# r4dl/LAENeRF

Hardware: AMD Instinct MI355X
Metric: Mrays/s, lego 800x800 train-step (4096 rays/step) (higher is better)
Workload: dtype f16 (table, MLP) / f32 (march, composite); 1 GPU; configs[1]: lego-like 800x800 pinhole rays, 4096 random pixels of one view per step, L=16 T=2^19 F=2 hash grid + 2x64 / 3x64 ffmlp, cascade 1, analytic occupancy (13% occupied), steady-state train step incl. backward + Adam; hip_graph_replay=True, march_pipelined_on_side_stream=True, steps_per_graph_replay=4, parallelism=1 independent ray-batch replicas (no data-path collective)

## Files before the change

### include/laenerf.h

```cpp
#ifndef LAENERF_H
#define LAENERF_H

#include <stdint.h>

#ifdef __cplusplus
extern "C" {
#endif

#if defined(__GNUC__) || defined(__clang__)
#define LAE_API __attribute__((visibility("default")))
#else
#define LAE_API
#endif

#define LAE_OK 0
#define LAE_EINVAL (-1)
#define LAE_ELAUNCH (-2)
#define LAE_ENULL (-3)

#define LAE_F32 0
#define LAE_F16 1

#define LAE_GRID_HASH 0
#define LAE_GRID_TILED 1
#define LAE_INTERP_LINEAR 0
#define LAE_INTERP_SMOOTHSTEP 1

#define LAE_ACT_RELU 0
#define LAE_ACT_EXPONENTIAL 1
#define LAE_ACT_SINE 2
#define LAE_ACT_SIGMOID 3
#define LAE_ACT_SQUAREPLUS 4
#define LAE_ACT_SOFTPLUS 5
#define LAE_ACT_NONE 6

#define LAE_ABI_TAG "abi14"
LAE_API const char* lae_version(void);
LAE_API const char* lae_last_error(void);


LAE_API int lae_near_far_from_aabb(const float* rays_o, const float* rays_d, const float* aabb,
                           uint32_t N, float min_near, float* nears, float* fars, void* stream);

LAE_API int lae_get_rays(const float* poses, uint32_t B, float fx, float fy, float cx, float cy, uint32_t H, uint32_t W,
                 const int64_t* inds, uint64_t inds_batch_stride, uint32_t N, int perturb, float off_x, float off_y,
                 float* rays_o, float* rays_d, const float* aabb, float min_near, float* nears, float* fars, void* stream);

#define LAE_IMG_U8 0
#define LAE_IMG_F16 1
#define LAE_IMG_F32 2
#define LAE_BATCH_IMAGE 0
#define LAE_BATCH_ALL 1
#define LAE_BG_WHITE 0
#define LAE_BG_RANDOM 1
LAE_API int lae_sample_train_batch(const void* images, int dtype, uint32_t n_img, uint32_t H, uint32_t W, uint32_t C,
                           const float* poses, float fx, float fy, float cx, float cy, uint32_t N,
                           const float* aabb, float min_near, uint64_t seed, int64_t* step_counter, int mode, int bg_mode,
                           int srgb_to_linear, float* rays_o, float* rays_d, float* nears, float* fars, float* gt,
                           float* bg_out, int64_t* inds, void* stream);

LAE_API int lae_sample_train_batch_weighted(const void* images, int dtype, uint32_t n_img, uint32_t H, uint32_t W, uint32_t C,
                                    const float* poses, float fx, float fy, float cx, float cy, uint32_t N,
                                    const float* aabb, float min_near, uint64_t seed, int64_t* step_counter, int bg_mode,
                                    int srgb_to_linear, const float* error_map, int32_t* cells_out, float* rays_o, float* rays_d,
                                    float* nears, float* fars, float* gt, float* bg_out, int64_t* inds, void* stream);

LAE_API int lae_error_map_update(float* error_map, uint32_t n_img, uint32_t H, uint32_t W, const int64_t* inds, const int32_t* cells,
                                 const float* pred, const float* gt, uint32_t N, void* stream);

// ... 94 lines not shown
                     uint32_t C, uint32_t H, const void* table_f16, const int32_t* offsets, const int32_t* offsets_host,
                     uint32_t L, float S,
                     uint32_t base_resolution, uint32_t gridtype, int align_corners, uint32_t interp,
                     const void* sigma_weights, const void* color_weights, float density_scale, float T_thresh,
                     uint32_t max_n_step, uint64_t row_budget, const float* noises, const float* bg_rays, float bg_r, float bg_g,
                     float bg_b, int blend_bg, int scale_depth, float* weights_sum, float* depth, float* image,
                     float* weights_edit, float* depth_edit, void* workspace, uint64_t workspace_bytes, uint32_t* stats_out,
                     void* stream);

LAE_API uint64_t lae_compact_scratch_bytes(uint32_t n_alive);
LAE_API int lae_compact_rays_alive(const int32_t* rays_alive, uint32_t n_alive, int32_t* out_alive,
                           int32_t* n_out_dev, void* scratch, void* stream);


LAE_API int lae_grid_encode_forward(const float* inputs, const void* embeddings, const int32_t* offsets,
                            void* outputs, uint32_t B, uint32_t D, uint32_t C, uint32_t L,
                            float S, uint32_t H, void* dy_dx, uint32_t gridtype,
                            int align_corners, uint32_t interp, int dtype, void* stream);

LAE_API int lae_grid_encode_backward(const void* grad, const float* inputs, const void* embeddings,
                             const int32_t* offsets, void* grad_embeddings, uint32_t B,
                             uint32_t D, uint32_t C, uint32_t L, float S, uint32_t H,
                             const void* dy_dx, void* grad_inputs, uint32_t gridtype,
                             int align_corners, uint32_t interp, int dtype, void* stream);

LAE_API int lae_grid_encode_forward_ex(const float* inputs, const void* embeddings, const int32_t* offsets, void* outputs,
                               uint32_t B, uint32_t D, uint32_t C, uint32_t L, float S, uint32_t H, void* dy_dx,
                               uint32_t gridtype, int align_corners, uint32_t interp, int dtype, int blc, float in_shift,
                               float in_scale, const int32_t* offsets_host, void* stream);
LAE_API int lae_grid_encode_backward_ex(const void* grad, const float* inputs, const void* embeddings, const int32_t* offsets,
                                void* grad_embeddings, uint32_t B, uint32_t D, uint32_t C, uint32_t L, float S,
                                uint32_t H, const void* dy_dx, void* grad_inputs, uint32_t gridtype,
                                int align_corners, uint32_t interp, int dtype, int blc, float in_shift, float in_scale,
                                const int32_t* offsets_host, int32_t* nonfinite_flag, uint32_t* touched_lines, void* stream);

LAE_API uint64_t lae_grid_backward_plan_bytes(uint32_t B, uint32_t L);
LAE_API uint64_t lae_grid_touched_lines_words(uint64_t n_entries);
LAE_API int lae_grid_encode_backward_plan(const float* inputs, const int32_t* offsets, uint32_t B, uint32_t D, uint32_t C, uint32_t L,
                                  float S, uint32_t H, uint32_t gridtype, int align_corners, uint32_t interp, int dtype,
                                  float in_shift, float in_scale, const int32_t* offsets_host, void* plan,
                                  uint32_t* touched_lines, void* stream);
LAE_API int lae_grid_encode_backward_planned(const void* grad, const float* inputs, const int32_t* offsets, void* grad_embeddings,
                                     uint32_t B, uint32_t D, uint32_t C, uint32_t L, float S, uint32_t H, uint32_t gridtype,
                                     int align_corners, uint32_t interp, int dtype, float in_shift, float in_scale,
                                     const int32_t* offsets_host, const void* plan, int32_t* nonfinite_flag, void* stream);

LAE_API uint64_t lae_grid_backward_workspace_bytes(uint32_t B, uint32_t L, int dtype);

LAE_API int lae_grid_forward_schedule(const int32_t* offsets_host, uint32_t L, float S, uint32_t H, uint32_t n_chunks,
                              uint32_t* nseg_out, uint32_t* segs_out);

LAE_API int lae_grid_set_forward_mode(int mode);

LAE_API int lae_grid_set_backward_mode(int mode);

LAE_API int lae_grad_total_variation(const void* inputs, const void* embeddings, void* grad,
                             const int32_t* offsets, float weight, uint32_t B, uint32_t D,
                             uint32_t C, uint32_t L, float S, uint32_t H, uint32_t gridtype,
                             int align_corners, int dtype, void* stream);


LAE_API int lae_sh_encode_forward(const float* inputs, float* outputs, uint32_t B, uint32_t D,
                          uint32_t C, float* dy_dx, void* stream);

LAE_API int lae_sh_encode_backward(const float* grad, const float* inputs, uint32_t B, uint32_t D,
                           uint32_t C, const float* dy_dx, float* grad_inputs, void* stream);


LAE_API int lae_ffmlp_forward(const void* inputs, const void* weights, uint32_t B, uint32_t input_dim,
                      uint32_t output_dim, uint32_t hidden_dim, uint32_t num_layers,
                      uint32_t activation, uint32_t output_activation, void* forward_buffer,
                      void* outputs, void* stream);

LAE_API int lae_ffmlp_inference(const void* inputs, const void* weights, uint32_t B, uint32_t input_dim,
                        uint32_t output_dim, uint32_t hidden_dim, uint32_t num_layers,
                        uint32_t activation, uint32_t output_activation, void* inference_buffer,
                        void* outputs, void* stream);

LAE_API int lae_ffmlp_backward(const void* grad, const void* inputs, const void* weights,
                       const void* forward_buffer, uint32_t B, uint32_t input_dim,
                       uint32_t output_dim, uint32_t hidden_dim, uint32_t num_layers,
                       uint32_t activation, uint32_t output_activation, int calc_grad_inputs,
                       void* backward_buffer, void* grad_inputs, void* grad_weights,
                       void* stream);
LAE_API int lae_ffmlp_backward_ex(const void* grad, const void* inputs, const void* weights,
                          const void* forward_buffer, uint32_t B, uint32_t input_dim,
                          uint32_t output_dim, uint32_t hidden_dim, uint32_t num_layers,
                          uint32_t activation, uint32_t output_activation, int calc_grad_inputs,
                          void* backward_buffer, void* grad_inputs, void* grad_weights,
                          int accumulate, int32_t* nonfinite_flag, void* stream);

LAE_API int lae_nerf_head_forward(const void* enc, const float* dirs, const void* sigma_weights, const void* color_weights,
                          uint32_t M, float density_scale, void* h_out, float* sigmas, float* rgbs, int enc_level_major,
                          void* stream);

LAE_API int lae_nerf_density_forward(const void* enc, const void* sigma_weights, uint32_t M, float density_scale, void* h_out,
                             float* sigmas, int enc_level_major, void* stream);

LAE_API int lae_nerf_head_backward(const float* grad_sigmas, const float* grad_rgbs, const void* enc, const float* dirs, const void* h,
                           const float* rgbs, const void* sigma_weights, const void* color_weights, uint32_t M,
                           float density_scale, void* grad_h, void* grad_enc, void* grad_sigma_weights,
                           void* grad_color_weights, int accumulate_weight_grads, int enc_level_major,
                           int32_t* nonfinite_flag, const float* loss_partials, uint32_t loss_n_part, uint32_t loss_n_elem,
                           const float* loss_scale, float* loss_out, void* stream);

LAE_API int lae_freq_encode_forward(const float* inputs, uint32_t B, uint32_t D, uint32_t deg, uint32_t C, float* outputs,
                            void* stream);
LAE_API int lae_freq_encode_backward(const float* grad, const float* outputs, uint32_t B, uint32_t D, uint32_t deg, uint32_t C,
                             float* grad_inputs, void* stream);

LAE_API int lae_palette_forward(const void* w_logits, const void* o_raw, const float* palette, uint32_t P, uint32_t active_mask,
                        uint32_t M, void* pred, float* w_hat, void* o_hat, void* stream);
LAE_API uint64_t lae_palette_backward_scratch_bytes(uint32_t M);
LAE_API int lae_palette_backward(const void* w_logits, const void* o_raw, const float* palette, uint32_t P, uint32_t active_mask,
                         uint32_t M, const void* g_pred, const float* g_w, const void* g_o, void* g_w_logits, void* g_o_raw,
                         float* g_palette, void* scratch, void* stream);

#define LAE_RECOLOR_PREVIEW 0
#define LAE_RECOLOR_WEIGHTS 1
#define LAE_RECOLOR_OFFSETS 2
#define LAE_RECOLOR_EVAL 3
#define LAE_RECOLOR_NO_OFFSETS 1
#define LAE_RECOLOR_TANH 2
LAE_API uint64_t lae_recolor_compact_scratch_bytes(uint32_t N);
LAE_API int lae_recolor_compact(const float* depth, const float* weights_sum, const float* rays_o, const float* rays_d, uint32_t N,
                                int32_t* indices, int32_t* slot_map, float* x_term, float* dirs, float* alpha, int32_t* count,
                                void* scratch, void* stream);
LAE_API int lae_recolor_compose(const int32_t* slot_map, uint32_t N, const void* w_logits, uint32_t w_stride, const void* o_raw,
                                uint32_t o_stride, uint32_t P, uint32_t active_mask, const float* palette, const float* p_weights,
                                const float* p_bias, const float* alpha, const float* base, const float* bg, int mode, uint32_t k,
                                int flags, float* out, uint8_t* out_u8, void* stream);

#define LAE_DISTILL_NO_BG 1
LAE_API int lae_distill_compose(uint32_t R, const int32_t* img_idx, const int32_t* pix, const float* w, const float* pred,
                                const float* dist, const void* w_logits, uint32_t w_stride, const void* o_raw, uint32_t o_stride,
                                uint32_t P, uint32_t active_mask, const float* palette_mod, const float* palette_og,
                                const float* p_weights, const float* p_bias, float blend_thresh, int flags, void* images, int dtype,
// ... 58 lines not shown
LAE_API int lae_min_dist_to_points(const float* pts, uint32_t n, const float* set, uint32_t m, float max_dist, float* out,
                           float* out_max, void* scratch, void* stream);

LAE_API int lae_density_grid_positions(const int32_t* coords, uint32_t n, uint32_t H, float bound_c, const float* noise,
                               float* xyzs, int32_t* indices, void* stream);
LAE_API uint64_t lae_density_grid_partial_scratch_bytes(uint32_t cells, uint32_t n);
LAE_API int lae_density_grid_partial_positions(const float* grid_c, uint32_t cells, const int32_t* coords_rand, const float* u, const float* rnd,
                                       uint32_t n, uint32_t H, float bound_c, const float* noise, float* xyzs, int32_t* indices,
                                       void* scratch, void* stream);
LAE_API int lae_density_grid_update(const float* sigmas, const int32_t* indices, uint32_t n, float density_scale, float decay,
                            uint32_t cells, float* grid, uint32_t* tmp, void* stream);
LAE_API int lae_mark_untrained_grid(const float* poses, uint32_t B, float fx, float fy, float cx, float cy, uint32_t C, uint32_t H,
                            float bound, float min_near, int filter_close_point, float* grid, void* stream);

LAE_API uint64_t lae_marching_cubes_scratch_bytes(uint32_t nx, uint32_t ny, uint32_t nz);
LAE_API int lae_marching_cubes_count(const float* u, uint32_t nx, uint32_t ny, uint32_t nz, float threshold, void* scratch,
                             int32_t* counts, void* stream);
LAE_API int lae_marching_cubes_emit(const float* u, uint32_t nx, uint32_t ny, uint32_t nz, float threshold, void* scratch, float* verts,
                            int32_t* tris, void* stream);

LAE_API int lae_adam_check(const void* grad, int grad_is_half, uint64_t n, void* state, void* stream);
LAE_API int lae_adam_begin(void* state, float beta1, float beta2, int growth_interval, float growth_factor, float backoff_factor,
                   int use_scaler, void* stream);
LAE_API int lae_adam_apply(float* param, float* exp_avg, float* exp_avg_sq, void* grad, int grad_is_half, void* shadow_half, uint64_t n,
                   const void* state, const float* lr, float beta1, float beta2, float eps, float weight_decay, void* stream);

LAE_API int lae_mse_loss_forward(const float* pred, const float* target, uint32_t n, const float* scale, float* loss_out, float* grad,
                         void* stream);

LAE_API int lae_adam_check_multi(uint32_t n_tensors, const void* const* grads, const int* grad_is_half, const uint64_t* sizes, void* state,
                         void* stream);
LAE_API int lae_adam_apply_multi(uint32_t n_tensors, float* const* params, float* const* exp_avgs, float* const* exp_avg_sqs, void* const* grads,
                         const int* grad_is_half, void* const* shadows_half, const uint64_t* sizes, const float* const* lrs, const void* const* touched_lines,
                         const void* state, float beta1, float beta2, float eps, float weight_decay, void* stream);

LAE_API int lae_ema_update_multi(uint32_t n_tensors, float* const* shadows, const float* const* params, const uint64_t* sizes,
                         float one_minus_decay, void* stream);
LAE_API int lae_ema_update_gated(uint32_t n_tensors, float* const* shadows, const float* const* params, const uint64_t* sizes,
                         const int64_t* step, int64_t epoch_len, int32_t* count, double decay, int use_num_updates, void* stream);

#define LAE_EVAL_VIEW_SCRATCH_DOUBLES 2048
LAE_API int lae_eval_view(const float* pred, const float* depth, const void* gt, int gt_dtype, uint32_t gt_channels, uint32_t n_pixels,
                          float bg, const uint8_t* mask, double* scratch, double* sse_out, double* masked_sse_out, float* gt_out,
                          uint8_t* rgb_u8, uint8_t* depth_u8, float* lpips_in, void* stream);
LAE_API int lae_lpips_head(uint32_t n_layers, const float* const* feats, const float* const* weights, const uint32_t* channels,
                           const uint32_t* hw, uint32_t n_pairs, double* scratch, double* out, void* stream);

LAE_API int lae_ffmlp_set_mode(int mode);

LAE_API int lae_allocate_splitk(uint64_t size);
LAE_API int lae_free_splitk(void);

LAE_API int lae_free_workspaces(void);
LAE_API uint64_t lae_workspace_bytes(int retired);

#ifdef __cplusplus
}
#endif
#endif
```

### laenerf_amd/_lib.py

```python
import ctypes
import os

import torch

_HERE = os.path.dirname(os.path.abspath(__file__))
SO_PATH = os.environ.get("LAE_HIP_LIB") or os.path.join(_HERE, "lib", "liblaenerf_hip.so")

u32, u64, f32, i32, vp = ctypes.c_uint32, ctypes.c_uint64, ctypes.c_float, ctypes.c_int, ctypes.c_void_p
i64, f64 = ctypes.c_int64, ctypes.c_double

SIGNATURES = {
    "lae_near_far_from_aabb": [vp, vp, vp, u32, f32, vp, vp, vp],
    "lae_sph_from_ray": [vp, vp, f32, u32, vp, vp],
    "lae_get_rays": [vp, u32, f32, f32, f32, f32, u32, u32, vp, u64, u32, i32, f32, f32, vp, vp, vp, f32, vp, vp, vp],
    "lae_morton3D": [vp, u32, vp, vp],
    "lae_morton3D_invert": [vp, u32, vp, vp],
    "lae_packbits": [vp, u32, f32, vp, vp],
    "lae_march_rays_train_scratch_bytes": [u32],
    "lae_march_rays_train": [vp, vp, vp, f32, f32, u32, u32, u32, u32, u32, vp, vp, vp, vp, vp, vp, vp, vp, vp, vp, vp],
    "lae_march_rays_train_limit": [vp, vp, vp, f32, f32, u32, u32, u32, u32, u32, vp, vp, vp, vp, vp, vp, vp, vp, vp, vp, vp, vp],
    "lae_sample_train_batch": [vp, i32, u32, u32, u32, u32, vp, f32, f32, f32, f32, u32, vp, f32, u64, vp, i32, i32, i32, vp, vp, vp, vp, vp,
                               vp, vp, vp],
    "lae_sample_train_batch_weighted": [vp, i32, u32, u32, u32, u32, vp, f32, f32, f32, f32, u32, vp, f32, u64, vp, i32, i32, vp, vp,
                                        vp, vp, vp, vp, vp, vp, vp, vp],
    "lae_error_map_update": [vp, u32, u32, u32, vp, vp, vp, vp, u32, vp],
    "lae_composite_rays_train_forward": [vp, vp, vp, vp, u32, u32, f32, vp, vp, vp, vp],
    "lae_composite_rays_train_backward": [vp, vp, vp, vp, vp, vp, vp, vp, u32, u32, f32, vp, vp, vp],
    "lae_composite_rays_train_forward_blend": [vp, vp, vp, vp, u32, u32, f32, vp, vp, vp, f32, f32, f32, vp, vp, vp, vp, vp, vp],
    "lae_composite_rays_train_step": [vp, vp, vp, vp, u32, u32, f32, vp, vp, vp, f32, f32, f32, vp, vp, vp, vp, vp, vp, vp, vp, vp, vp, vp, vp, vp, i32, vp],
    "lae_loss_finish": [vp, u32, u32, vp, vp, vp],
    "lae_composite_rays_train_backward_blend": [vp, vp, vp, vp, vp, vp, vp, vp, u32, u32, f32, vp, f32, f32, f32, vp, vp, vp, vp],
    "lae_composite_rays_train_backward_blend_ex": [vp, vp, vp, vp, vp, vp, vp, vp, u32, u32, f32, vp, f32, f32, f32, vp, vp, vp, vp, vp],
    "lae_march_rays": [u32, u32, vp, vp, vp, vp, f32, f32, u32, u32, u32, vp, vp, vp, vp, vp, vp, vp, vp],
    "lae_march_rays_distill": [u32, u32, vp, vp, vp, vp, f32, f32, u32, u32, u32, vp, vp, vp, vp, vp, vp, vp, vp, vp, vp],
    "lae_composite_rays": [u32, u32, f32, vp, vp, vp, vp, vp, vp, vp, vp, vp],
    "lae_composite_rays_distill": [u32, u32, f32, vp, vp, vp, vp, vp, vp, vp, vp, vp, vp, vp, vp],
    "lae_render_frame_workspace_bytes": [u32, u32, u64],
    "lae_render_frame_set_overlap": [i32],
    "lae_render_frame_mode": [],
    "lae_render_frame_last_status": [],
    "lae_render_frame_probe_us": [vp, u32],
    "lae_render_frame": [vp, vp, u32, vp, f32, vp, vp, f32, f32, u32, u32, u32, vp, vp, vp, u32, f32, u32, u32, i32, u32, vp, vp, f32, f32,
                         u32, u64, vp, vp, f32, f32, f32, i32, i32, vp, vp, vp, vp, vp, vp, u64, vp, vp],
    "lae_compact_scratch_bytes": [u32],
    "lae_compact_rays_alive": [vp, u32, vp, vp, vp, vp],
    "lae_grid_encode_forward": [vp, vp, vp, vp, u32, u32, u32, u32, f32, u32, vp, u32, i32, u32, i32, vp],
    "lae_grid_encode_backward": [vp, vp, vp, vp, vp, u32, u32, u32, u32, f32, u32, vp, vp, u32, i32, u32, i32, vp],
    "lae_grid_encode_forward_ex": [vp, vp, vp, vp, u32, u32, u32, u32, f32, u32, vp, u32, i32, u32, i32, i32, f32, f32, vp, vp],
    "lae_grid_encode_backward_ex": [vp, vp, vp, vp, vp, u32, u32, u32, u32, f32, u32, vp, vp, u32, i32, u32, i32, i32, f32, f32, vp, vp, vp, vp],
    "lae_grid_backward_workspace_bytes": [u32, u32, i32],
    "lae_grid_backward_plan_bytes": [u32, u32],
    "lae_grid_touched_lines_words": [u64],
    "lae_grid_encode_backward_plan": [vp, vp, u32, u32, u32, u32, f32, u32, u32, i32, u32, i32, f32, f32, vp, vp, vp, vp],
    "lae_grid_encode_backward_planned": [vp, vp, vp, vp, u32, u32, u32, u32, f32, u32, u32, i32, u32, i32, f32, f32, vp, vp, vp, vp],
    "lae_grid_set_backward_mode": [i32],
    "lae_grid_set_forward_mode": [i32],
    "lae_grid_forward_schedule": [vp, u32, f32, u32, u32, vp, vp],
    "lae_grad_total_variation": [vp, vp, vp, vp, f32, u32, u32, u32, u32, f32, u32, u32, i32, i32, vp],
    "lae_sh_encode_forward": [vp, vp, u32, u32, u32, vp, vp],
    "lae_sh_encode_backward": [vp, vp, u32, u32, u32, vp, vp, vp],
    "lae_freq_encode_forward": [vp, u32, u32, u32, u32, vp, vp],
    "lae_freq_encode_backward": [vp, vp, u32, u32, u32, u32, vp, vp],
    "lae_ffmlp_forward": [vp, vp, u32, u32, u32, u32, u32, u32, u32, vp, vp, vp],
    "lae_ffmlp_inference": [vp, vp, u32, u32, u32, u32, u32, u32, u32, vp, vp, vp],
    "lae_ffmlp_backward": [vp, vp, vp, vp, u32, u32, u32, u32, u32, u32, u32, i32, vp, vp, vp, vp],
    "lae_ffmlp_backward_ex": [vp, vp, vp, vp, u32, u32, u32, u32, u32, u32, u32, i32, vp, vp, vp, i32, vp, vp],
    "lae_nerf_head_forward": [vp, vp, vp, vp, u32, f32, vp, vp, vp, i32, vp],
    "lae_nerf_density_forward": [vp, vp, u32, f32, vp, vp, i32, vp],
    "lae_density_grid_positions": [vp, u32, u32, f32, vp, vp, vp, vp],
    "lae_density_grid_partial_scratch_bytes": [u32, u32],
    "lae_density_grid_partial_positions": [vp, u32, vp, vp, vp, u32, u32, f32, vp, vp, vp, vp, vp],
    "lae_density_grid_update": [vp, vp, u32, f32, f32, u32, vp, vp, vp],
    "lae_mark_untrained_grid": [vp, u32, f32, f32, f32, f32, u32, u32, f32, f32, i32, vp, vp],
    "lae_nerf_head_backward": [vp, vp, vp, vp, vp, vp, vp, vp, u32, f32, vp, vp, vp, vp, i32, i32, vp, vp, u32, u32, vp, vp, vp],
    "lae_palette_forward": [vp, vp, vp, u32, u32, u32, vp, vp, vp, vp],
    "lae_palette_backward_scratch_bytes": [u32],
    "lae_palette_backward": [vp, vp, vp, u32, u32, u32, vp, vp, vp, vp, vp, vp, vp, vp],
    "lae_recolor_compact_scratch_bytes": [u32],
    "lae_recolor_compact": [vp, vp, vp, vp, u32, vp, vp, vp, vp, vp, vp, vp, vp],
    "lae_recolor_compose": [vp, u32, vp, u32, vp, u32, u32, u32, vp, vp, vp, vp, vp, vp, i32, u32, i32, vp, vp, vp],
    "lae_distill_compose": [u32, vp, vp, vp, vp, vp, vp, u32, vp, u32, u32, u32, vp, vp, vp, vp, f32, i32, vp, i32, u32, u32, u32, vp],
    "lae_error_map_seed": [u32, vp, vp, vp, vp, u32, u32, u32, u32, vp, vp, vp],
    "lae_marching_cubes_scratch_bytes": [u32, u32, u32],
    "lae_marching_cubes_count": [vp, u32, u32, u32, f32, vp, vp, vp],
    "lae_marching_cubes_emit": [vp, u32, u32, u32, f32, vp, vp, vp, vp],
    "lae_style_loss_scratch_bytes": [u32],
    "lae_style_loss_forward": [vp, vp, vp, vp, u32, u32, f32, f32, f32, vp, vp, vp, vp, u32, f32, f32, vp],
    "lae_style_loss_backward": [vp, vp, vp, u32, u32, u32, vp, vp, vp, f32, f32, f32, vp, vp, vp, vp, i32, f32, f32, vp],
    "lae_style_loss_forward_dev": [vp, vp, vp, vp, u32, vp, u32, f32, f32, f32, vp, vp, vp, vp, u32, f32, f32, vp],
    "lae_style_loss_backward_dev": [vp, vp, vp, u32, u32, u32, vp, vp, vp, vp, f32, f32, f32, vp, vp, vp, vp, i32, f32, f32, vp],
    "lae_sample_edit_view": [vp, vp, vp, vp, vp, vp, u32, vp, u32, u32, u64, vp, vp, vp, vp, vp, vp],
    "lae_style_loss_backward_image_dev": [vp, vp, vp, u32, u32, u32, vp, vp, vp, vp, f32, f32, f32, vp, vp, vp, vp, vp, i32, f32, f32, vp],
    "lae_style_image_scratch_bytes": [u32],
    "lae_style_image_forward": [vp, u32, vp, vp, u32, vp, u32, vp, vp, vp, vp, vp, vp, vp, vp, u32, vp, i32, u32, vp, vp, vp],
    "lae_style_image_backward": [vp, u32, vp, vp, u32, vp, u32, vp, vp, vp, vp, vp, vp, vp, vp, vp, vp, u32, vp, vp, i32, vp, vp],
    "lae_grow_region": [vp, vp, u32, u32, f32, vp, u32, vp, u32, u32, vp],
    "lae_style_assemble_forward": [vp, vp, u32, u32, u32, vp, vp, u32, vp],
    "lae_style_assemble_backward": [vp, vp, u32, u32, vp, vp],
    "lae_min_dist_to_points": [vp, u32, vp, u32, f32, vp, vp, vp, vp],
    "lae_mse_loss_forward": [vp, vp, u32, vp, vp, vp, vp],
    "lae_adam_check": [vp, i32, u64, vp, vp],
    "lae_adam_check_multi": [u32, vp, vp, vp, vp, vp],
    "lae_adam_apply_multi": [u32, vp, vp, vp, vp, vp, vp, vp, vp, vp, vp, f32, f32, f32, f32, vp],
    "lae_adam_begin": [vp, f32, f32, i32, f32, f32, i32, vp],
    "lae_ema_update_multi": [u32, vp, vp, vp, f32, vp],
    "lae_ema_update_gated": [u32, vp, vp, vp, vp, i64, vp, f64, i32, vp],
    "lae_eval_view": [vp, vp, vp, i32, u32, u32, f32, vp, vp, vp, vp, vp, vp, vp, vp, vp],
    "lae_lpips_head": [u32, vp, vp, vp, vp, u32, vp, vp, vp],
    "lae_adam_apply": [vp, vp, vp, vp, i32, vp, u64, vp, vp, f32, f32, f32, f32, vp],
    "lae_ffmlp_set_mode": [i32],
    "lae_allocate_splitk": [u64],
    "lae_free_splitk": [],
    "lae_free_workspaces": [],
    "lae_workspace_bytes": [i32],
    "lae_version": [],
    "lae_last_error": [],
}
_RESTYPES = {
    "lae_march_rays_train_scratch_bytes": u64,
    "lae_compact_scratch_bytes": u64,
    "lae_density_grid_partial_scratch_bytes": u64,
    "lae_palette_backward_scratch_bytes": u64,
    "lae_style_loss_scratch_bytes": u64,
    "lae_recolor_compact_scratch_bytes": u64,
    "lae_marching_cubes_scratch_bytes": u64,
    "lae_style_image_scratch_bytes": u64,
    "lae_render_frame_workspace_bytes": u64,
    "lae_workspace_bytes": u64,
    "lae_grid_backward_workspace_bytes": u64,
    "lae_grid_backward_plan_bytes": u64,
    "lae_grid_touched_lines_words": u64,
    "lae_version": ctypes.c_char_p,
    "lae_last_error": ctypes.c_char_p,
}

_lib = None
ABI_TAG = b"abi14"


def _abi_of(path):
    lib = ctypes.CDLL(path)
    fn = lib.lae_version
    fn.argtypes, fn.restype = [], ctypes.c_char_p
    return lib, fn().split()[-1]


def load():
    global _lib
    if _lib is not None:
        return _lib
    if not os.path.exists(SO_PATH):
        raise RuntimeError(
            f"laenerf_amd: HIP library not built ({SO_PATH}); run `python -m laenerf_amd.build` "
            "(there is no CPU fallback)")
    if not os.environ.get("LAE_HIP_LIB"):
        from . import build as _build
        if _build.default_is_packed(SO_PATH):
            _build.build(force=True)
            if _build.default_is_packed(SO_PATH):
                raise RuntimeError(f"laenerf_amd: {SO_PATH} was built with packed-fp32 instructions and could not be rebuilt without them")
    lib, tag = _abi_of(SO_PATH)
    if tag != ABI_TAG:
        if os.environ.get("LAE_HIP_LIB"):
            raise RuntimeError(f"laenerf_amd: {SO_PATH} is ABI {tag.decode()}, this package binds {ABI_TAG.decode()}")
        import fcntl
        import shutil
        from . import build as _build
        with open(SO_PATH + ".lock", "w") as lock:
            fcntl.flock(lock, fcntl.LOCK_EX)
            try:
# ... 60 lines not shown
```

### laenerf_amd/backend.py

```python
import sys
import types

import numpy as np
import torch

from . import _lib
from ._lib import check, need_contig, need_cuda, ptr, stream

_F16 = torch.float16


def _dtype_code(t):
    if t.dtype == torch.float32:
        return 0
    if t.dtype == torch.float16:
        return 1
    raise RuntimeError(f"laenerf_amd: unsupported dtype {t.dtype} (float32 / float16 only)")


def _host_i32(a, n):
    if a is None:
        return None
    if not (isinstance(a, np.ndarray) and a.dtype == np.int32 and a.flags.c_contiguous and a.size == n):
        raise RuntimeError("laenerf_amd: offsets_host must be a contiguous int32 numpy array with L + 1 entries")
# ... 341 lines not shown
    @staticmethod
    def grid_encode_forward(inputs, embeddings, offsets, outputs, B, D, C, L, S, H, dy_dx, gridtype, align_corners,
                            interp, blc=False, in_map=(0.0, 1.0), offsets_host=None):
        need_cuda(inputs, embeddings, offsets, outputs, dy_dx); need_contig(inputs, embeddings, offsets, outputs, dy_dx)
        if inputs.dtype != torch.float32 or offsets.dtype != torch.int32:
            raise RuntimeError("grid_encode_forward: inputs must be float32, offsets int32")
        if outputs.dtype != embeddings.dtype or (dy_dx is not None and dy_dx.dtype != embeddings.dtype):
            raise RuntimeError("grid_encode_forward: outputs/dy_dx must have the embeddings dtype")
        lib = _lib.load()
        args = (ptr(inputs), ptr(embeddings), ptr(offsets), ptr(outputs), B, D, C, L, float(S), H, ptr(dy_dx), gridtype,
                int(bool(align_corners)), interp, _dtype_code(embeddings))
        if blc or tuple(in_map) != (0.0, 1.0) or offsets_host is not None:
            check(lib.lae_grid_encode_forward_ex(*args, int(bool(blc)), float(in_map[0]), float(in_map[1]), _host_i32(offsets_host, L + 1),
                                                 stream()), "grid_encode_forward")
        else:
            check(lib.lae_grid_encode_forward(*args, stream()), "grid_encode_forward")

    @staticmethod
    def grid_backward_plan(inputs, offsets, B, D, C, L, S, H, gridtype, align_corners, interp, half, in_map=(0.0, 1.0),
                           offsets_host=None, touched_lines=None):
        need_cuda(inputs, offsets); need_contig(inputs, offsets)
        lib = _lib.load()
        plan = torch.empty(int(lib.lae_grid_backward_plan_bytes(B, L)), dtype=torch.uint8, device=inputs.device)
        check(lib.lae_grid_encode_backward_plan(ptr(inputs), ptr(offsets), B, D, C, L, float(S), H, gridtype, int(bool(align_corners)),
                                                interp, 1 if half else 0, float(in_map[0]), float(in_map[1]),
                                                _host_i32(offsets_host, L + 1), ptr(plan), touched_lines, stream()),
              "grid_backward_plan")
        plan.marks_touched = touched_lines is not None
        return plan

    @staticmethod
    def grid_encode_backward(grad, inputs, embeddings, offsets, grad_embeddings, B, D, C, L, S, H, dy_dx, grad_inputs,
                             gridtype, align_corners, interp, blc=False, in_map=(0.0, 1.0), offsets_host=None, plan=None,
                             nonfinite_flag=None, touched_lines=None):
        ts = (grad, inputs, embeddings, offsets, grad_embeddings, dy_dx, grad_inputs, plan)
        need_cuda(*ts); need_contig(*ts)
        if grad.dtype != grad_embeddings.dtype:
            raise RuntimeError("grid_encode_backward: grad and grad_embeddings dtypes differ")
        lib = _lib.load()
        if plan is not None:
            if blc or dy_dx is not None:
                raise RuntimeError("grid_encode_backward: a plan needs level-major gradients and no input gradient")
            if touched_lines is not None and not getattr(plan, "marks_touched", False):
                raise RuntimeError("grid_encode_backward: the plan was made without the touched-lines bitmap (pass it to grid_backward_plan)")
            check(lib.lae_grid_encode_backward_planned(ptr(grad), ptr(inputs), ptr(offsets), ptr(grad_embeddings), B, D, C, L, float(S), H,
                                                       gridtype, int(bool(align_corners)), interp, _dtype_code(grad), float(in_map[0]),
                                                       float(in_map[1]), _host_i32(offsets_host, L + 1), ptr(plan), nonfinite_flag, stream()),
                  "grid_encode_backward")
            return
        args = (ptr(grad), ptr(inputs), ptr(embeddings), ptr(offsets), ptr(grad_embeddings), B, D, C, L, float(S), H,
                ptr(dy_dx), ptr(grad_inputs), gridtype, int(bool(align_corners)), interp, _dtype_code(grad))
        if blc or tuple(in_map) != (0.0, 1.0) or offsets_host is not None or nonfinite_flag is not None or touched_lines is not None:
            check(lib.lae_grid_encode_backward_ex(*args, int(bool(blc)), float(in_map[0]), float(in_map[1]), _host_i32(offsets_host, L + 1),
                                                  nonfinite_flag, touched_lines, stream()), "grid_encode_backward")
        else:
            check(lib.lae_grid_encode_backward(*args, stream()), "grid_encode_backward")

    @staticmethod
    def grid_backward_workspace_bytes(B, L, half=True):
        return int(_lib.load().lae_grid_backward_workspace_bytes(B, L, 1 if half else 0))

    @staticmethod
    def set_backward_mode(mode):
        check(_lib.load().lae_grid_set_backward_mode(int(mode)), "grid_set_backward_mode")

    @staticmethod
    def grad_total_variation(inputs, embeddings, grad, offsets, weight, B, D, C, L, S, H, gridtype, align_corners):
        need_cuda(inputs, embeddings, grad, offsets); need_contig(inputs, embeddings, grad, offsets)
        check(_lib.load().lae_grad_total_variation(ptr(inputs), ptr(embeddings), ptr(grad), ptr(offsets), float(weight), B, D,
                                                   C, L, float(S), H, gridtype, int(bool(align_corners)),
                                                   _dtype_code(embeddings), stream()), "grad_total_variation")


class _SHEncoder:
    @staticmethod
    def sh_encode_forward(inputs, outputs, B, D, C, dy_dx):
        need_cuda(inputs, outputs, dy_dx); need_contig(inputs, outputs, dy_dx)
        if inputs.dtype != torch.float32 or outputs.dtype != torch.float32:
            raise RuntimeError("sh_encode_forward: float32 required (sphere_harmonics.py:16 casts to fp32)")
        check(_lib.load().lae_sh_encode_forward(ptr(inputs), ptr(outputs), B, D, C, ptr(dy_dx), stream()), "sh_encode_forward")

    @staticmethod
    def sh_encode_backward(grad, inputs, B, D, C, dy_dx, grad_inputs):
        need_cuda(grad, inputs, dy_dx, grad_inputs); need_contig(grad, inputs, dy_dx, grad_inputs)
        if grad.dtype != torch.float32:
            raise RuntimeError("sh_encode_backward: float32 required")
        check(_lib.load().lae_sh_encode_backward(ptr(grad), ptr(inputs), B, D, C, ptr(dy_dx), ptr(grad_inputs), stream()),
# ... 49 lines not shown
            check(_lib.load().lae_ffmlp_backward_ex(ptr(grad), ptr(inputs), ptr(weights), ptr(forward_buffer), B, input_dim,
                                                    output_dim, hidden_dim, num_layers, activation, output_activation,
                                                    int(bool(calc_grad_inputs)), ptr(backward_buffer), ptr(grad_inputs),
                                                    ptr(grad_weights), int(bool(accumulate)), nonfinite_flag, stream()), "ffmlp_backward")
            return
        check(_lib.load().lae_ffmlp_backward(ptr(grad), ptr(inputs), ptr(weights), ptr(forward_buffer), B, input_dim,
                                             output_dim, hidden_dim, num_layers, activation, output_activation,
                                             int(bool(calc_grad_inputs)), ptr(backward_buffer), ptr(grad_inputs),
                                             ptr(grad_weights), stream()), "ffmlp_backward")

    @staticmethod
    def nerf_head_forward(enc, dirs, sigma_weights, color_weights, M, density_scale, h_out, sigmas, rgbs, level_major=False):
        ts = (enc, dirs, sigma_weights, color_weights, h_out, sigmas, rgbs)
        need_cuda(*ts); need_contig(*ts); _FFMLP._half(enc, sigma_weights, color_weights, h_out)
        check(_lib.load().lae_nerf_head_forward(ptr(enc), ptr(dirs), ptr(sigma_weights), ptr(color_weights), M,
                                                float(density_scale), ptr(h_out), ptr(sigmas), ptr(rgbs),
                                                int(bool(level_major)), stream()), "nerf_head_forward")

    @staticmethod
    def nerf_density_forward(enc, sigma_weights, M, density_scale, h_out, sigmas, level_major=False):
        need_cuda(enc, sigma_weights, h_out, sigmas); need_contig(enc, sigma_weights, h_out, sigmas)
        _FFMLP._half(enc, sigma_weights, h_out)
        check(_lib.load().lae_nerf_density_forward(ptr(enc), ptr(sigma_weights), M, float(density_scale), ptr(h_out),
                                                   ptr(sigmas), int(bool(level_major)), stream()), "nerf_density_forward")

    @staticmethod
    def nerf_head_backward(grad_sigmas, grad_rgbs, enc, dirs, h, rgbs, sigma_weights, color_weights, M, density_scale,
                           grad_h, grad_enc, grad_sigma_weights, grad_color_weights, accumulate=False, level_major=False,
                           nonfinite_flag=None):
        ts = (grad_sigmas, grad_rgbs, enc, dirs, h, rgbs, sigma_weights, color_weights, grad_h, grad_enc,
              grad_sigma_weights, grad_color_weights)
        need_cuda(*ts); need_contig(*ts)
        _FFMLP._half(enc, h, sigma_weights, color_weights, grad_h, grad_enc, grad_sigma_weights, grad_color_weights)
        key = _loss_key(grad_sigmas)
        pend = _pending_loss.get(key)
        if pend is not None and pend[5] != stream():
            pend = None
        if pend is not None:
            del _pending_loss[key]
        lp, ln, le, lsc, lo = pend[:5] if pend is not None else (None, 0, 0, None, None)
        try:
            check(_lib.load().lae_nerf_head_backward(ptr(grad_sigmas), ptr(grad_rgbs), ptr(enc), ptr(dirs), ptr(h), ptr(rgbs),
                                                     ptr(sigma_weights), ptr(color_weights), M, float(density_scale),
                                                     ptr(grad_h), ptr(grad_enc), ptr(grad_sigma_weights),
                                                     ptr(grad_color_weights), int(bool(accumulate)), int(bool(level_major)),
                                                     nonfinite_flag, ptr(lp), ln, le, ptr(lsc), ptr(lo), stream()), "nerf_head_backward")
        except RuntimeError:
            if pend is not None:
                _pending_loss[key] = pend
            raise
        if pend is not None:
            deferred_loss_stats["carried"] += 1

    @staticmethod
    def ffmlp_set_mode(mode):
        check(_lib.load().lae_ffmlp_set_mode(int(mode)), "ffmlp_set_mode")

    @staticmethod
    def fused_backward_available(input_dim, hidden_dim, num_layers, activation):
        return hidden_dim == 64 and activation == 0 and num_layers in (2, 3) and input_dim in (32, 48, 64)

    @staticmethod
    def allocate_splitk(size):
        check(_lib.load().lae_allocate_splitk(int(size)), "allocate_splitk")

    @staticmethod
    def free_splitk():
        check(_lib.load().lae_free_splitk(), "free_splitk")


_timing = {"on": False, "only": None, "events": []}
_UNITS = {"grid_encode_forward": 4, "grid_encode_backward": 5, "grid_backward_plan": 2, "ffmlp_forward": 2, "ffmlp_inference": 2,
          "ffmlp_backward": 4, "nerf_head_forward": 4, "nerf_head_backward": 8, "nerf_density_forward": 2, "sh_encode_forward": 2, "march_rays_train": 6, "composite_rays_train_forward": 5,
          "composite_rays_train_backward": 9,
          "composite_rays_train_forward_blend": 5, "composite_rays_train_backward_blend": 9}


def enable_kernel_timing(on, only=("grid_encode_forward",)):
    import gc
    if on and not _timing["on"]:
        _timing["gc_was_enabled"] = gc.isenabled()
        gc.collect()
        gc.disable()
    elif not on and _timing["on"]:
        if _timing.pop("gc_was_enabled", True):
# ... 239 lines not shown
```

### laenerf_amd/csrc/ffmlp.hip

```cpp
#include <string>
#include <algorithm>
#include <type_traits>
#include <stdlib.h>
#include "lae_common.h"

namespace {

typedef _Float16 half_t;
typedef _Float16 h4 __attribute__((ext_vector_type(4)));
typedef float f4 __attribute__((ext_vector_type(4)));

__device__ __forceinline__ f4 mfma16(h4 a, h4 b, f4 c) { return __builtin_amdgcn_mfma_f32_16x16x16f16(a, b, c, 0, 0, 0); }

typedef _Float16 h8 __attribute__((ext_vector_type(8)));
__device__ __forceinline__ f4 mfma32(h4 a_lo, h4 a_hi, h4 b_lo, h4 b_hi, f4 c) {
    const h8 a = __builtin_shufflevector(a_lo, a_hi, 0, 1, 2, 3, 4, 5, 6, 7);
    const h8 b = __builtin_shufflevector(b_lo, b_hi, 0, 1, 2, 3, 4, 5, 6, 7);
    return __builtin_amdgcn_mfma_f32_16x16x32_f16(a, b, c, 0, 0, 0);
}
template <int KT, typename LoadA>
__device__ __forceinline__ f4 mfma_ksteps(LoadA&& a_of, const h4* b, f4 acc) {
#pragma unroll
    for (int kt = 0; kt + 1 < KT; kt += 2) acc = mfma32(a_of(kt), a_of(kt + 1), b[kt], b[kt + 1], acc);
    if constexpr (KT & 1) {
        const h4 z = h4{(half_t)0.0f, (half_t)0.0f, (half_t)0.0f, (half_t)0.0f};
        acc = mfma32(a_of(KT - 1), z, b[KT - 1], z, acc);
    }
    return acc;
}

#define K_ACT 10.0f
__device__ __forceinline__ float act_fwd(uint32_t a, float v) {
    switch (a) {
        case LAE_ACT_RELU: return v > 0.0f ? v : 0.0f;
        case LAE_ACT_EXPONENTIAL: return expf(v);
        case LAE_ACT_SINE: return sinf(v);
        case LAE_ACT_SIGMOID: return 1.0f / (1.0f + expf(-v));
// ... 244 lines not shown
            if ((uint32_t)i < nt_n) {
                const half_t* q = A + (b0 + 4 * g) * IN + (nt0 + i) * 16 + c;
                bf[i][0] = q[0]; bf[i][1] = q[IN]; bf[i][2] = q[2 * (size_t)IN]; bf[i][3] = q[3 * (size_t)IN];
            }
        }
#pragma unroll
        for (int i = 0; i < 4; i++)
#pragma unroll
            for (int j = 0; j < 4; j++)
                if ((uint32_t)i < mt_n && (uint32_t)j < nt_n) acc[i][j] = mfma16(a[i], bf[j], acc[i][j]);
    }
    __shared__ float red[16 * 256];
    for (int ww = 0; ww < MLP_BLOCK / 64; ww++) {
        if (w == ww) {
#pragma unroll
            for (int i = 0; i < 4; i++)
#pragma unroll
                for (int j = 0; j < 4; j++)
#pragma unroll
                    for (int r = 0; r < 4; r++) {
                        float* p = &red[(i * 4 + j) * 256 + (4 * g + r) * 16 + c];
                        *p = (ww == 0) ? acc[i][j][r] : (*p + acc[i][j][r]);
                    }
        }
        __syncthreads();
    }
    float* slab = slabs + (size_t)blockIdx.x * nW + w_off;
    for (uint32_t e = threadIdx.x; e < 16 * 256; e += MLP_BLOCK) {
        const uint32_t t = e >> 8, i = t >> 2, j = t & 3, rr = (e >> 4) & 15, cc = e & 15;
        if (i < mt_n && j < nt_n) slab[(size_t)((mt0 + i) * 16 + rr) * IN + (nt0 + j) * 16 + cc] = red[e];
    }
}

constexpr int DWR_GROUPS = 16;
__device__ __forceinline__ void dw_reduce_body(const float* __restrict__ slabs, uint32_t n_slices, uint32_t nW, half_t* __restrict__ gw,
                                               int accumulate, uint32_t block, int32_t* __restrict__ nf_flag = nullptr) {
    __shared__ float part[DWR_GROUPS][64];
    const uint32_t e = threadIdx.x & 63, sg = threadIdx.x >> 6;
    const uint32_t i = block * 64 + e;
    float s[8] = {0, 0, 0, 0, 0, 0, 0, 0};
    if (i < nW) {
        uint32_t k = sg;
        for (; k + 7 * DWR_GROUPS < n_slices; k += 8 * DWR_GROUPS) {
#pragma unroll
            for (int u = 0; u < 8; u++) s[u] += slabs[(size_t)(k + u * DWR_GROUPS) * nW + i];
        }
        for (; k < n_slices; k += DWR_GROUPS) s[0] += slabs[(size_t)k * nW + i];
    }
    part[sg][e] = ((s[0] + s[1]) + (s[2] + s[3])) + ((s[4] + s[5]) + (s[6] + s[7]));
    __syncthreads();
    if (sg == 0 && i < nW) {
        float t[DWR_GROUPS];
#pragma unroll
        for (int u = 0; u < DWR_GROUPS; u++) t[u] = part[u][e];
#pragma unroll
        for (int w = DWR_GROUPS / 2; w > 0; w >>= 1)
#pragma unroll
            for (int u = 0; u < w; u++) t[u] = t[u] + t[u + w];
        const half_t r = accumulate ? (half_t)((float)gw[i] + t[0]) : (half_t)t[0];
        gw[i] = r;
        if (nf_flag && (__builtin_bit_cast(uint16_t, r) & 0x7c00u) == 0x7c00u) atomicOr(nf_flag, 1);
    }
}
__global__ __launch_bounds__(64 * DWR_GROUPS) void k_dw_reduce(const float* __restrict__ slabs, uint32_t n_slices, uint32_t nW,
                                                               half_t* __restrict__ gw, int accumulate = 0, int32_t* __restrict__ nf_flag = nullptr) {
    dw_reduce_body(slabs, n_slices, nW, gw, accumulate, blockIdx.x, nf_flag);
}
struct LossFinish { const float* partials; uint32_t n_part, n_elem; const float* scale; float* out; };
__global__ __launch_bounds__(64 * DWR_GROUPS) void k_dw_reduce2(const float* __restrict__ slabs_a, uint32_t n_a, uint32_t nW_a,
                                                                half_t* __restrict__ gw_a, const float* __restrict__ slabs_b,
                                                                uint32_t n_b, uint32_t nW_b, half_t* __restrict__ gw_b,
                                                                uint32_t nb_a, uint32_t nb_b, int accumulate, int32_t* __restrict__ nf_flag,
                                                                LossFinish lf) {
    if (blockIdx.x < nb_a) dw_reduce_body(slabs_a, n_a, nW_a, gw_a, accumulate, blockIdx.x, nf_flag);
    else if (blockIdx.x < nb_a + nb_b) dw_reduce_body(slabs_b, n_b, nW_b, gw_b, accumulate, blockIdx.x - nb_a, nf_flag);
    else {
        static_assert(64 * DWR_GROUPS == 1024, "the loss sum is written for 16 waves, like k_loss_finish");
        __shared__ float part[16];
        float acc = 0.0f;
        for (uint32_t i = threadIdx.x; i < lf.n_part; i += 1024) acc += lf.partials[i];
        {
            auto dpp = [](float v, auto ctrl, auto mask) {
                return __builtin_bit_cast(float, __builtin_amdgcn_update_dpp(0, __builtin_bit_cast(int, v), decltype(ctrl)::value, decltype(mask)::value, 0xf, false));
            };
            using std::integral_constant;
            acc += dpp(acc, integral_constant<int, 0x111>{}, integral_constant<int, 0xf>{});
            acc += dpp(acc, integral_constant<int, 0x112>{}, integral_constant<int, 0xf>{});
            acc += dpp(acc, integral_constant<int, 0x114>{}, integral_constant<int, 0xf>{});
            acc += dpp(acc, integral_constant<int, 0x118>{}, integral_constant<int, 0xf>{});
            acc += dpp(acc, integral_constant<int, 0x142>{}, integral_constant<int, 0xa>{});
            acc += dpp(acc, integral_constant<int, 0x143>{}, integral_constant<int, 0xc>{});
            acc = __builtin_bit_cast(float, __builtin_amdgcn_readlane(__builtin_bit_cast(int, acc), 63));
        }
        if ((threadIdx.x & 63) == 0) part[threadIdx.x >> 6] = acc;
        __syncthreads();
        if (threadIdx.x == 0) {
            float t = 0.0f;
#pragma unroll
            for (int w = 0; w < 16; w++) t += part[w];
            const float loss = t / (float)lf.n_elem;
            lf.out[0] = loss * (lf.scale ? lf.scale[0] : 1.0f);
            lf.out[1] = loss;
        }
    }
}

#include "sh_table.inc"

__device__ __forceinline__ void stage_rows(half_t* dst, int ld, const half_t* __restrict__ src, int rows, int cols) {
    for (uint32_t e = threadIdx.x; e < (uint32_t)rows * cols / 4; e += blockDim.x) {
        const uint32_t r = (e * 4) / cols, k = (e * 4) % cols;
        *reinterpret_cast<h4*>(dst + r * ld + k) = *reinterpret_cast<const h4*>(src + (size_t)r * cols + k);
    }
}

template <int KT>
__device__ __forceinline__ void layer64(const half_t* Wl, int ld, const h4 (&in)[KT], int c, int g, f4 (&acc)[4]) {
#pragma unroll
    for (int mt = 0; mt < 4; mt++) acc[mt] = f4{0, 0, 0, 0};
#pragma unroll
    for (int kt = 0; kt + 1 < KT; kt += 2)
#pragma unroll
        for (int mt = 0; mt < 4; mt++) {
            const half_t* wr = Wl + (mt * 16 + c) * ld + kt * 16 + 4 * g;
            acc[mt] = mfma32(*reinterpret_cast<const h4*>(wr), *reinterpret_cast<const h4*>(wr + 16), in[kt], in[kt + 1], acc[mt]);
        }
    if constexpr (KT & 1) {
        const h4 z = h4{(half_t)0.0f, (half_t)0.0f, (half_t)0.0f, (half_t)0.0f};
#pragma unroll
        for (int mt = 0; mt < 4; mt++)
            acc[mt] = mfma32(*reinterpret_cast<const h4*>(Wl + (mt * 16 + c) * ld + (KT - 1) * 16 + 4 * g), z, in[KT - 1], z, acc[mt]);
    }
}
typedef _Float16 h2 __attribute__((ext_vector_type(2)));
__device__ __forceinline__ void relu4(const f4 (&acc)[4], h4 (&out)[4]) {
#pragma unroll
    for (int mt = 0; mt < 4; mt++) {
// ... 1328 lines not shown
    return lae::check_launch("ffmlp_backward");
}

int lae_nerf_head_forward(const void* enc, const float* dirs, const void* sigma_weights, const void* color_weights,
                          uint32_t M, float density_scale, void* h_out, float* sigmas, float* rgbs, int enc_level_major,
                          void* stream) {
    if (M == 0) return LAE_OK;
    if (!enc || !dirs || !sigma_weights || !color_weights || !h_out || !sigmas || !rgbs) return LAE_ENULL;
    if (M % 16 != 0) return LAE_EINVAL;
    if (const int rc = head_args_ok(sigma_weights, color_weights, M, "nerf_head_forward")) return rc;
    const int rc = launch_head_fwd5<true>((const half_t*)enc, dirs, (const half_t*)sigma_weights, (const half_t*)color_weights, M / 16, M / 16,
                                          density_scale, (half_t*)h_out, sigmas, rgbs, enc_level_major, nullptr, M,
                                          reinterpret_cast<hipStream_t>(stream));
    return rc != LAE_OK ? rc : lae::check_launch("nerf_head_forward");
}

int lae_nerf_density_forward(const void* enc, const void* sigma_weights, uint32_t M, float density_scale, void* h_out,
                             float* sigmas, int enc_level_major, void* stream) {
    if (M == 0) return LAE_OK;
    if (!enc || !sigma_weights || !sigmas) return LAE_ENULL;
    if (M % 16 != 0) return LAE_EINVAL;
    if (const int rc = head_args_ok(sigma_weights, sigma_weights, M, "nerf_density_forward")) return rc;
    const int rc = launch_head_fwd5<false>((const half_t*)enc, nullptr, (const half_t*)sigma_weights, nullptr, M / 16, M / 16, density_scale,
                                           (half_t*)h_out, sigmas, nullptr, enc_level_major, nullptr, M, reinterpret_cast<hipStream_t>(stream));
    return rc != LAE_OK ? rc : lae::check_launch("nerf_density_forward");
}

int lae_nerf_head_backward(const float* grad_sigmas, const float* grad_rgbs, const void* enc, const float* dirs, const void* h,
                           const float* rgbs, const void* sigma_weights, const void* color_weights, uint32_t M,
                           float density_scale, void* grad_h, void* grad_enc, void* grad_sigma_weights,
                           void* grad_color_weights, int accumulate_weight_grads, int enc_level_major, int32_t* nonfinite_flag,
                           const float* loss_partials, uint32_t loss_n_part, uint32_t loss_n_elem, const float* loss_scale,
                           float* loss_out, void* stream) {
    if (!grad_sigma_weights || !grad_color_weights) return LAE_ENULL;
    if (loss_out && (!loss_partials || loss_n_elem == 0)) return LAE_EINVAL;
    hipStream_t s = reinterpret_cast<hipStream_t>(stream);
    if (M == 0) {
        if (loss_out) {
            const int rc = lae_loss_finish(loss_partials, loss_n_part, loss_n_elem, loss_scale, loss_out, stream);
            if (rc != LAE_OK) return rc;
        }
        if (accumulate_weight_grads) return LAE_OK;
        if (hipMemsetAsync(grad_sigma_weights, 0, 64 * (32 + 64 + 16) * 2, s) != hipSuccess) return LAE_ELAUNCH;
        if (hipMemsetAsync(grad_color_weights, 0, 64 * (32 + 128 + 16) * 2, s) != hipSuccess) return LAE_ELAUNCH;
        return LAE_OK;
    }
    if (!grad_sigmas || !grad_rgbs || !enc || !dirs || !h || !rgbs || !sigma_weights || !color_weights || !grad_h) return LAE_ENULL;
    if (M % 16 != 0) return LAE_EINVAL;
    HeadBwdArgs ha{dirs, rgbs, grad_rgbs, grad_sigmas, density_scale, 0};
    HeadBwdArgs hs{};
    hs.level_major = enc_level_major;
    const uint32_t nW_c = 64 * (32 + 128 + 16), nW_s = 64 * (32 + 64 + 16);
    const size_t cap = (size_t)lae::num_cus() * 2;
    float* ws = reinterpret_cast<float*>(lae::workspace(lae::WS_FFMLP_SLABS, cap * (nW_c + nW_s) * sizeof(float), s));
    if (!ws) return LAE_ELAUNCH;
    float* ws_s = ws + cap * nW_c;
    uint32_t n_c = 0, n_s = 0;
    int rc = launch_bwd_fused<32, 2, 1>(nullptr, (const half_t*)h, (const half_t*)color_weights, M, (half_t*)grad_h,
                                        (half_t*)grad_color_weights, s, ha, accumulate_weight_grads, ws, &n_c);
    if (rc != LAE_OK) return rc;
    rc = launch_bwd_fused<32, 1, 0>((const half_t*)grad_h, (const half_t*)enc, (const half_t*)sigma_weights, M, (half_t*)grad_enc,
                                    (half_t*)grad_sigma_weights, s, hs, accumulate_weight_grads, ws_s, &n_s);
    if (rc != LAE_OK) return rc;
    const uint32_t nb_c = lae::cdiv(nW_c, 64u), nb_s = lae::cdiv(nW_s, 64u);
    const LossFinish lf{loss_partials, loss_n_part, loss_n_elem, loss_scale, loss_out};
    k_dw_reduce2<<<nb_c + nb_s + (loss_out ? 1u : 0u), 64 * DWR_GROUPS, 0, s>>>(ws, n_c, nW_c, (half_t*)grad_color_weights, ws_s, n_s, nW_s,
                                                                               (half_t*)grad_sigma_weights, nb_c, nb_s,
                                                                               accumulate_weight_grads, nonfinite_flag, lf);
    return lae::check_launch("nerf_head_backward");
}

int lae_ffmlp_set_mode(int mode) {
    if (mode != 0 && mode != 1 && mode != 3) return LAE_EINVAL;
    g_ffmlp_mode = mode == 1 ? 1 : 0;
    g_bwd_fused_variant = mode == 3 ? 0 : 2;
    return LAE_OK;
}

int lae_allocate_splitk(uint64_t size) {
    (void)size;
    return LAE_OK;
}

int lae_free_splitk(void) {
    lae::free_workspaces();
    return LAE_OK;
}

}
```

### laenerf_amd/csrc/gridencoder.hip

```cpp
#include <math.h>
#include <stdio.h>
#include <stdlib.h>
#include <algorithm>
#include <type_traits>
#include "lae_common.h"
#include <vector>
#include <mutex>
#include <utility>

namespace {

constexpr int MAX_LEVELS = 32;
struct LevelScales { float scale[MAX_LEVELS]; float in_shift, in_scale; };

typedef _Float16 half_t;
typedef _Float16 half2_t __attribute__((ext_vector_type(2)));

__constant__ uint32_t k_primes[7] = {1u, 2654435761u, 805459861u, 3674653429u, 2097192037u, 1434869437u, 2165219737u};

#ifdef LAE_GRID_STAMPS
__device__ unsigned long long g_grid_stamps[32768 * 32];
#define GRID_STAMP(slot, i) do { if (threadIdx.x == 0 && (uint32_t)(i) < 32u) g_grid_stamps[(size_t)(slot) * 32 + (i)] = wall_clock64(); } while (0)
#define GRID_NOTE(slot, i, v) do { if (threadIdx.x == 0 && (uint32_t)(i) < 32u) g_grid_stamps[(size_t)(slot) * 32 + (i)] = (v); } while (0)
#else
#define GRID_STAMP(slot, i) do { } while (0)
#define GRID_NOTE(slot, i, v) do { } while (0)
#endif


template <int D>
struct LevelInfo {
    float scale;
    uint32_t resolution, hashmap_size, table_off;
    uint32_t stride[D];
    uint32_t ndense;
    bool use_hash, pow2;
    bool nowrap;
};
// ... 259 lines not shown
#endif
}


__global__ __launch_bounds__(GRID_BLOCK) void k_grid_fwd_lean_tail(
    const float* __restrict__ inputs, const half_t* __restrict__ grid, const int32_t* __restrict__ offsets,
    half_t* __restrict__ outputs, uint32_t B, LevelScales sc, uint32_t L, uint64_t os_b, uint64_t os_l,
    const uint32_t* __restrict__ B_dev, uint32_t b0) {
    const uint32_t b = b0 + blockIdx.x * GRID_BLOCK + threadIdx.x;
    B = min(B, *B_dev);
    if (b >= B) return;
#pragma unroll
    for (uint32_t level = 0; level < 16u; level++)
        if (level < L) grid_fwd_lean_row(inputs, grid, offsets, outputs, sc, os_b, os_l, level, b);
}
constexpr uint32_t PART_SHIFT = 12, PART = 1u << PART_SHIFT;
constexpr uint32_t BK_MAX = 512;
constexpr uint32_t BK_TARGET = 32;

struct LevelBins { uint32_t P, SUB; };
__host__ __device__ __forceinline__ LevelBins level_bins_of(uint32_t hashmap_size, uint32_t bk_target = BK_TARGET) {
    LevelBins lb;
    lb.P = (hashmap_size + PART - 1) >> PART_SHIFT;
    lb.SUB = lb.P >= bk_target ? 1u : (bk_target + lb.P - 1) / lb.P;
    return lb;
}
__host__ __device__ __forceinline__ bool level_is_binned(uint32_t hashmap_size) { return level_bins_of(hashmap_size).P <= BK_MAX; }


template <typename T, int D, int C>
__global__ __launch_bounds__(GRID_BLOCK) void k_grid_bwd(
    const T* __restrict__ grad, const float* __restrict__ inputs, const int32_t* __restrict__ offsets,
    T* __restrict__ grad_grid, uint32_t B, uint32_t L, LevelScales sc, uint32_t gridtype, bool align_corners,
    uint32_t interp, uint32_t nb, bool xcd_mode, uint64_t gs_b, uint64_t gs_l, bool only_unbinned) {
    uint32_t level, chunk;
    block_to_level_chunk(nb, xcd_mode, level, chunk);
    if (level >= L) return;
    const uint32_t b = chunk * GRID_BLOCK + threadIdx.x;
    if (b >= B) return;
    const LevelInfo<D> li = level_info<D>(sc, offsets, level, gridtype, align_corners);
    if (only_unbinned) {
        if constexpr (D == 3) { if (level_is_binned(li.hashmap_size)) return; }
    }
    T* __restrict__ tab = grad_grid + (size_t)li.table_off * C;

    float frac[D];
    uint32_t pg[D];
#pragma unroll
    for (int d = 0; d < D; d++) {
        const float xv = (inputs[(size_t)b * D + d] + sc.in_shift) * sc.in_scale;
        if (xv < 0.0f || xv > 1.0f) return;
        float p = fmaf(xv, li.scale, align_corners ? 0.0f : 0.5f);
        const float fl = floorf(p);
        pg[d] = (uint32_t)fl;
        p -= (float)pg[d];
        if (interp == 1) p = p * p * (3.0f - 2.0f * p);
        frac[d] = p;
    }
    const T* g = grad + (size_t)b * gs_b + (size_t)level * gs_l;
    float gc[C];
#pragma unroll
    for (int ch = 0; ch < C; ch++) gc[ch] = (float)g[ch];

#pragma unroll
    for (int idx = 0; idx < (1 << D); idx++) {
        float w = 1.0f;
        uint32_t pgl[D];
// ... 14 lines not shown
        } else {
#pragma unroll
            for (int ch = 0; ch < C; ch++) atomicAdd(tab + gi + ch, w * gc[ch]);
        }
    }
}

template <typename T> struct BVal;
template <> struct BVal<half_t> { using type = uint2; };
template <> struct BVal<float> { using type = float4; };
constexpr int FILL_THREADS = 256;
constexpr int SPT = 4;
constexpr int SEGS = 1;
constexpr uint32_t UNIT_SAMPLES = FILL_THREADS * SPT;
constexpr uint32_t STAGE_CAP = 4096 + 256;
constexpr uint32_t KEY_SINGLE = 15u;
constexpr int ACC_THREADS = 1024;
constexpr uint32_t BWD_MAX_SAMPLES = 1u << 24;
constexpr uint32_t COARSE_RES = 64;
constexpr bool WIDE_COARSE_UNITS = false;
constexpr uint32_t SUB_RECS = 64;
constexpr uint32_t TICKET_ARRIVALS = 2;
constexpr uint32_t TICKET_WORDS = TICKET_ARRIVALS + MAX_LEVELS * SUB_RECS;
template <typename T> constexpr uint32_t sub_rec_words() { return (sizeof(T) == 2 ? 2 * PART : PART) + PART / 64; }

struct BwdPlan {
    uint16_t* cnt;
    uint32_t* part_cnt;
    uint32_t* totals;
    uint32_t* offs;
    uint32_t* tickets;
};

__device__ __forceinline__ uint32_t pack_half2(float a, float b) {
    const half2_t h = {(half_t)a, (half_t)b};
    return __builtin_bit_cast(uint32_t, h);
}

template <typename T, bool FILL, bool PLAIN>
__global__ __launch_bounds__(FILL_THREADS) void k_bwd_walk(
    const T* __restrict__ gradT, const float* __restrict__ inputs, const int32_t* __restrict__ offsets, uint32_t B,
    uint32_t L, LevelScales sc, uint32_t gridtype_, bool align_corners_, uint32_t interp_, uint32_t U, BwdPlan plan,
    typename BVal<T>::type* __restrict__ qvals, uint16_t* __restrict__ qkeys, uint32_t* __restrict__ touched_,
    uint32_t* __restrict__ level_full) {
    const uint32_t gridtype = PLAIN ? 0u : gridtype_, interp = PLAIN ? 0u : interp_;
    const bool align_corners = PLAIN ? false : align_corners_;
    using V = typename BVal<T>::type;
    if constexpr (FILL) GRID_STAMP(blockIdx.x, 0);
    const uint32_t NBLK = U / SEGS;
    const uint32_t level = blockIdx.x / NBLK, chunk = blockIdx.x % NBLK;
    if (FILL && blockIdx.x == 0) for (uint32_t k = threadIdx.x; k < TICKET_WORDS; k += FILL_THREADS) plan.tickets[k] = 0;
    const LevelInfo<3> li = level_info<3>(sc, offsets, level, gridtype, align_corners);
    const uint32_t P = (li.hashmap_size + PART - 1) >> PART_SHIFT;
    if (P > BK_MAX) return;
    __shared__ uint32_t hist[BK_MAX], start[BK_MAX + 1], gbase[FILL ? BK_MAX : 1];
    __shared__ __attribute__((aligned(16))) V s_vals[FILL ? STAGE_CAP : 1];
    __shared__ __attribute__((aligned(16))) uint16_t s_keys[FILL ? STAGE_CAP : 8];
    extern __shared__ uint32_t s_lines[];
    const uint32_t tid = threadIdx.x, lane = tid & 63u;
    const uint32_t line_shift = (li.table_off >> 3) & 31u;
    const uint32_t line_words = (line_shift + ((li.hashmap_size + 7u) >> 3) + 31u) >> 5;
    __shared__ uint32_t s_mark;
    if (!FILL) {
        if (tid == 0) s_mark = (touched_ && !level_full[level]) ? 1u : 0u;
        __syncthreads();
    }
    uint32_t* __restrict__ touched = (!FILL && s_mark) ? touched_ : nullptr;
    if (!FILL && touched) { for (uint32_t k = tid; k < line_words; k += FILL_THREADS) s_lines[k] = 0u; }
    const bool wide = li.resolution < COARSE_RES && WIDE_COARSE_UNITS;
    const uint32_t NSUB = wide ? 4u : 1u;
    if (wide && (chunk & 3u)) {
        if constexpr (!FILL) {
            const uint32_t u_e = chunk * SEGS, unit_e = level * U + u_e;
            for (uint32_t k = tid; k < BK_MAX / 2; k += FILL_THREADS) reinterpret_cast<uint32_t*>(plan.cnt + (size_t)unit_e * BK_MAX)[k] = 0u;
            for (uint32_t k = tid; k < P; k += FILL_THREADS) plan.part_cnt[((size_t)level * BK_MAX + k) * U + u_e] = 0u;
        }
        return;
    }
    const uint32_t b0 = wide ? ((chunk >> 2) * (UNIT_SAMPLES * 4u) + tid * (SPT * 4u)) : (chunk * FILL_THREADS + tid) * (SPT * SEGS);
    const uint32_t NC = (P <= BK_MAX / 8 && li.resolution >= COARSE_RES) ? 8u : 1u;
    const T* __restrict__ g_lvl = gradT + (size_t)level * B * 2;

    uint32_t cpg[3] = {0, 0, 0};
    bool have = false;
// ... 373 lines not shown
            const uint32_t w0 = v.x, w1 = v.y;
            const uint32_t carry = (((w0 & 0x7c007c00u) + 0x28002800u) | ((w1 & 0x7c007c00u) + 0x28002800u)) & 0x80008000u;
            if (carry == 0) {
                long long a, b;
                half2_to_fix24_small(w0, a, b);
                atomicAdd(&acc64[e0], (unsigned long long)a);
                atomicAdd(&acc64[PART + e0], (unsigned long long)b);
                const uint32_t e1s = code != KEY_SINGLE ? e1 : e0;
                half2_to_fix24_small(w1, a, b);
                atomicAdd(&acc64[e1s], (unsigned long long)a);
                atomicAdd(&acc64[PART + e1s], (unsigned long long)b);
            } else {
                if (half_nonfinite(w0) || half_nonfinite(w0 >> 16)) atomicOr(&poison[e0 >> 5], 1u << (e0 & 31));
                else {
                    atomicAdd(&acc64[e0], (unsigned long long)half_to_fix24(w0 & 0xffffu));
                    atomicAdd(&acc64[PART + e0], (unsigned long long)half_to_fix24(w0 >> 16));
                }
                if (code != KEY_SINGLE) {
                    if (half_nonfinite(w1) || half_nonfinite(w1 >> 16)) atomicOr(&poison[e1 >> 5], 1u << (e1 & 31));
                    else {
                        atomicAdd(&acc64[e1], (unsigned long long)half_to_fix24(w1 & 0xffffu));
                        atomicAdd(&acc64[PART + e1], (unsigned long long)half_to_fix24(w1 >> 16));
                    }
                }
            }
        } else {
            float* af = reinterpret_cast<float*>(acc64);
            atomicAdd(af + e0, v.x); atomicAdd(af + PART + e0, v.y);
            if (code != KEY_SINGLE) { atomicAdd(af + e1, v.z); atomicAdd(af + PART + e1, v.w); }
        }
    };

    bool first_task = true;
    [[maybe_unused]] uint32_t stamp_task = 0;
    GRID_STAMP(4096 + blockIdx.x, 0);
    for (;;) {
        if (tid == 0) s_ticket = first_task ? blockIdx.x : atomicAdd(&plan.tickets[0], 1u) + gridDim.x;
        first_task = false;
        __syncthreads();
        const uint32_t t = __builtin_amdgcn_readfirstlane(s_ticket);
        GRID_STAMP(4096 + blockIdx.x, 1 + stamp_task * 6);
        if (t >= total_buckets) break;
        GRID_NOTE(4096 + blockIdx.x, 2 + stamp_task * 6, t);
        const uint32_t item = t;
        uint32_t level = 0;
        while (level + 1 < L && item >= s_first[level + 1]) level++;
        level = __builtin_amdgcn_readfirstlane(level);
        const uint32_t bk = item - __builtin_amdgcn_readfirstlane(s_first[level]);
        const uint32_t SUB = __builtin_amdgcn_readfirstlane(s_sub[level]), p = bk / SUB, sub = bk % SUB;
        const uint32_t table_off = (uint32_t)offsets[level], hashmap_size = (uint32_t)offsets[level + 1] - table_off;
        const uint32_t n = __builtin_amdgcn_readfirstlane(plan.totals[level * BK_MAX + p]), q0 = __builtin_amdgcn_readfirstlane(plan.offs[level * BK_MAX + p]);
        const uint32_t lo = (uint32_t)(((uint64_t)n * sub) / SUB), hi = (uint32_t)(((uint64_t)n * (sub + 1)) / SUB);
        if (n == 0) { __syncthreads(); continue; }
        const uint32_t part_lo = p << PART_SHIFT;
        const uint32_t n_ent = min(PART, hashmap_size - part_lo);
        T* __restrict__ dst = grad_grid + ((size_t)table_off + part_lo) * 2;
        uint32_t oldv[HALF ? PART / ACC_THREADS : 1];
        if constexpr (HALF) {
#pragma unroll
            for (int it = 0; it < (int)(PART / ACC_THREADS); it++) { const uint32_t e = tid + it * ACC_THREADS; oldv[it] = e < n_ent ? reinterpret_cast<const uint32_t*>(dst)[e] : 0u; }
        }
        for (uint32_t i = tid; i < ACCW; i += ACC_THREADS) acc64[i] = 0ull;
        if (tid < PART / 32) poison[tid] = 0u;
        __syncthreads();
        GRID_STAMP(4096 + blockIdx.x, 3 + stamp_task * 6);
        const uint32_t scale_res = (uint32_t)ceilf(sc.scale[level]) + 1;
        const V* __restrict__ pv = qvals + q0;
        const uint16_t* __restrict__ pk = qkeys + q0;
        if (!HALF && scale_res >= COARSE_RES) {
            uint32_t i = lo + tid;
            for (; i + 3 * ACC_THREADS < hi; i += 4 * ACC_THREADS) {
                V v[4]; uint32_t k[4];
#pragma unroll
                for (int j = 0; j < 4; j++) { v[j] = pv[i + j * ACC_THREADS]; k[j] = pk[i + j * ACC_THREADS]; }
#pragma unroll
                for (int j = 0; j < 4; j++) apply(k[j], v[j]);
            }
            for (; i < hi; i += ACC_THREADS) { const V v = pv[i]; const uint32_t k = pk[i]; apply(k, v); }
        } else {
            if constexpr (HALF) {
                using u4 = __attribute__((__vector_size__(16))) uint32_t;
                const uint32_t abs_lo = q0 + lo, abs_hi = q0 + hi, A0 = abs_lo & ~7u;
                const uint32_t n_groups = (abs_hi - A0 + 7u) >> 3;
                const __amdgpu_buffer_rsrc_t rs_v = __builtin_amdgcn_make_buffer_rsrc(const_cast<V*>(qvals + A0), 0, (int)(n_groups * 64u), 0x00020000);
                const __amdgpu_buffer_rsrc_t rs_k = __builtin_amdgcn_make_buffer_rsrc(const_cast<uint16_t*>(qkeys + A0), 0, (int)(n_groups * 16u), 0x00020000);
                const bool coarse = scale_res < COARSE_RES;
                for (uint32_t gq = coarse ? (tid & 63u) * (ACC_THREADS / 64) + (tid >> 6) : tid; gq < n_groups; gq += ACC_THREADS) {
                    const u4 va = __builtin_amdgcn_raw_buffer_load_b128(rs_v, (int)(gq * 64u), 0, 0);
                    const u4 vb = __builtin_amdgcn_raw_buffer_load_b128(rs_v, (int)(gq * 64u + 16u), 0, 0);
                    const u4 vc = __builtin_amdgcn_raw_buffer_load_b128(rs_v, (int)(gq * 64u + 32u), 0, 0);
                    const u4 vd = __builtin_amdgcn_raw_buffer_load_b128(rs_v, (int)(gq * 64u + 48u), 0, 0);
                    const u4 kk = __builtin_amdgcn_raw_buffer_load_b128(rs_k, (int)(gq * 16u), 0, 0);
                    const uint32_t w[16] = {va[0], va[1], va[2], va[3], vb[0], vb[1], vb[2], vb[3], vc[0], vc[1], vc[2], vc[3], vd[0], vd[1], vd[2], vd[3]};
// ... 54 lines not shown
            }
        }
        GRID_STAMP(4096 + blockIdx.x, 4 + stamp_task * 6);
        __syncthreads();
        GRID_STAMP(4096 + blockIdx.x, 5 + stamp_task * 6);
        if (SUB > 1) {
            unsigned long long* __restrict__ rec = partials + (size_t)(level * SUB_RECS + p) * sub_rec_words<T>();
            uint32_t* __restrict__ rec_poison = reinterpret_cast<uint32_t*>(rec + ACCW);
            if constexpr (HALF) {
                for (uint32_t i = tid; i < ACCW; i += ACC_THREADS) { const unsigned long long v = acc64[i]; if (v) atomicAdd(rec + i, v); }
            } else {
                const float* af = reinterpret_cast<const float*>(acc64);
                float* rf = reinterpret_cast<float*>(rec);
                for (uint32_t i = tid; i < 2 * PART; i += ACC_THREADS) { const float v = af[i]; if (v != 0.0f) atomicAdd(rf + i, v); }
            }
            if (tid < PART / 32 && poison[tid]) atomicOr(rec_poison + tid, poison[tid]);
            asm volatile("s_waitcnt vmcnt(0)" ::: "memory");
            __syncthreads();
            if (tid == 0) s_arr = atomicAdd(&plan.tickets[TICKET_ARRIVALS + level * SUB_RECS + p], 1u);
            __syncthreads();
            if (s_arr != SUB - 1) { GRID_STAMP(4096 + blockIdx.x, 6 + stamp_task * 6); stamp_task++; __syncthreads(); continue; }
            for (uint32_t i = tid; i < ACCW; i += ACC_THREADS) acc64[i] = atomicExch(rec + i, 0ull);
            if (tid < PART / 32) poison[tid] = atomicExch(rec_poison + tid, 0u);
            __syncthreads();
        }
        if constexpr (HALF) {
            uint32_t* d2 = reinterpret_cast<uint32_t*>(dst);
            bool wrote_nonfinite = false;
#pragma unroll
            for (int it = 0; it < (int)(PART / ACC_THREADS); it++) {
                const uint32_t e = tid + it * ACC_THREADS;
                if (e >= n_ent) break;
                const long long i0 = (long long)acc64[e], i1 = (long long)acc64[PART + e];
                const bool bad = (poison[e >> 5] >> (e & 31)) & 1u;
                if (i0 == 0 && i1 == 0 && !bad) continue;
                const uint32_t o = oldv[it];
                uint32_t r0, r1;
                if (bad) { r0 = 0x7e00u; r1 = 0x7e00u; }
                else {
                    r0 = half_nonfinite(o) ? (o & 0xffffu) : fix24_to_half(i0 + half_to_fix24(o & 0xffffu));
                    r1 = half_nonfinite(o >> 16) ? (o >> 16) : fix24_to_half(i1 + half_to_fix24(o >> 16));
                }
                d2[e] = r0 | (r1 << 16);
                wrote_nonfinite |= half_nonfinite(r0) || half_nonfinite(r1);
            }
            if (nf_flag && wrote_nonfinite) atomicOr(nf_flag, 1);
        } else {
            const float* af = reinterpret_cast<const float*>(acc64);
            float2* d2 = reinterpret_cast<float2*>(dst);
            for (uint32_t e = tid; e < n_ent; e += ACC_THREADS) {
                const float v0 = af[e], v1 = af[PART + e];
                if (v0 == 0.0f && v1 == 0.0f) continue;
                float2 o = d2[e]; o.x += v0; o.y += v1; d2[e] = o;
                if (nf_flag && !(isfinite(o.x) && isfinite(o.y))) atomicOr(nf_flag, 1);
            }
        }
        GRID_STAMP(4096 + blockIdx.x, 6 + stamp_task * 6);
        stamp_task++;
        __syncthreads();
    }
}

template <typename T>
__global__ __launch_bounds__(256) void k_out_transpose(const T* __restrict__ in, T* __restrict__ out, uint32_t B, uint32_t L) {
    using V = typename std::conditional<sizeof(T) == 2, uint32_t, uint2>::type;
    __shared__ V tile[256 * 33];
    const uint32_t b0 = blockIdx.x * 256;
    const uint32_t nb = min(256u, B - b0);
    const V* src = reinterpret_cast<const V*>(in);
    for (uint32_t e = threadIdx.x; e < nb * L; e += 256) {
        const uint32_t l = e / nb, b = e % nb;
        tile[b * (L + 1) + l] = src[(size_t)l * B + b0 + b];
    }
    __syncthreads();
    V* dstv = reinterpret_cast<V*>(out) + (size_t)b0 * L;
    for (uint32_t e = threadIdx.x; e < nb * L; e += 256) dstv[e] = tile[(e / L) * (L + 1) + (e % L)];
}

template <typename T>
__global__ __launch_bounds__(256) void k_grad_transpose(const T* __restrict__ in, T* __restrict__ out, uint32_t B, uint32_t L) {
    using V = typename std::conditional<sizeof(T) == 2, uint32_t, uint2>::type;
    __shared__ V tile[256 * 33];
    const uint32_t b0 = blockIdx.x * 256;
    const uint32_t nb = min(256u, B - b0);
    const V* src = reinterpret_cast<const V*>(in) + (size_t)b0 * L;
    for (uint32_t e = threadIdx.x; e < nb * L; e += 256) tile[(e / L) * (L + 1) + (e % L)] = src[e];
    __syncthreads();
    V* dstv = reinterpret_cast<V*>(out);
    for (uint32_t e = threadIdx.x; e < nb * L; e += 256) {
        const uint32_t l = e / nb, b = e % nb;
        dstv[(size_t)l * B + b0 + b] = tile[b * (L + 1) + l];
    }
// ... 209 lines not shown
    const bool xcd = (a.L % 8) == 0;
    k_grid_fwd<T, D, C><<<nb_safe * a.L, GRID_BLOCK, 0, a.stream>>>(a.inputs, (const T*)a.emb, a.offsets, (T*)a.out, a.B, a.L,
                                                                a.sc, (T*)a.dy_dx, a.gridtype, a.align, a.interp, nb_safe,
                                                                xcd, a.os_b, a.os_l, a.B_dev);
}
template <typename T, int D>
static int dispatch_fwd_c(const FwdArgs& a, uint32_t C) {
    switch (C) {
        case 1: launch_fwd<T, D, 1>(a); return LAE_OK;
        case 2: launch_fwd<T, D, 2>(a); return LAE_OK;
        case 4: launch_fwd<T, D, 4>(a); return LAE_OK;
        case 8: launch_fwd<T, D, 8>(a); return LAE_OK;
        default: return LAE_EINVAL;
    }
}
template <typename T>
static int dispatch_fwd_d(const FwdArgs& a, uint32_t D, uint32_t C) {
    switch (D) {
        case 2: return dispatch_fwd_c<T, 2>(a, C);
        case 3: return dispatch_fwd_c<T, 3>(a, C);
        case 4: return dispatch_fwd_c<T, 4>(a, C);
        case 5: return dispatch_fwd_c<T, 5>(a, C);
        default: return LAE_EINVAL;
    }
}

struct BwdArgs {
    const void* grad; const float* inputs; const int32_t* offsets; void* gemb; uint32_t B, L; LevelScales sc;
    uint32_t gridtype; bool align; uint32_t interp; uint64_t gs_b, gs_l; hipStream_t stream;
    const int32_t* offsets_host = nullptr;
    int32_t* nf_flag = nullptr;
    uint32_t* touched = nullptr;
    uint32_t* touched_full = nullptr;
};
template <typename T, int D, int C>
static void launch_bwd(const BwdArgs& a) {
    const uint32_t nb = lae::cdiv(a.B, GRID_BLOCK);
    const bool xcd = (a.L % 8) == 0;
    k_grid_bwd<T, D, C><<<nb * a.L, GRID_BLOCK, 0, a.stream>>>(a.grad ? (const T*)a.grad : nullptr, a.inputs, a.offsets,
                                                                (T*)a.gemb, a.B, a.L, a.sc, a.gridtype, a.align,
                                                                a.interp, nb, xcd, a.gs_b, a.gs_l, false);
}
template <typename T, int D>
static int dispatch_bwd_c(const BwdArgs& a, uint32_t C) {
    if constexpr (sizeof(T) == 2) {
        switch (C) {
            case 2: launch_bwd<T, D, 2>(a); return LAE_OK;
            case 4: launch_bwd<T, D, 4>(a); return LAE_OK;
            case 8: launch_bwd<T, D, 8>(a); return LAE_OK;
            default: return LAE_EINVAL;
        }
    } else {
        switch (C) {
            case 1: launch_bwd<T, D, 1>(a); return LAE_OK;
            case 2: launch_bwd<T, D, 2>(a); return LAE_OK;
            case 4: launch_bwd<T, D, 4>(a); return LAE_OK;
            case 8: launch_bwd<T, D, 8>(a); return LAE_OK;
            default: return LAE_EINVAL;
        }
    }
}
template <typename T>
static int dispatch_bwd_d(const BwdArgs& a, uint32_t D, uint32_t C) {
    switch (D) {
        case 2: return dispatch_bwd_c<T, 2>(a, C);
        case 3: return dispatch_bwd_c<T, 3>(a, C);
        case 4: return dispatch_bwd_c<T, 4>(a, C);
        case 5: return dispatch_bwd_c<T, 5>(a, C);
        default: return LAE_EINVAL;
    }
}

static int grid_forward(const float* inputs, const void* embeddings, const int32_t* offsets, void* outputs, uint32_t B,
                        uint32_t D, uint32_t C, uint32_t L, float S, uint32_t H, void* dy_dx, uint32_t gridtype,
// ... 7 lines not shown
    a.inputs = inputs; a.emb = embeddings; a.offsets = offsets; a.out = outputs; a.B = B; a.L = L;
    int rc = fill_scales(a.sc, L, S, H);
    if (rc) return rc;
    a.sc.in_shift = in_shift; a.sc.in_scale = in_scale;
    a.dy_dx = dy_dx; a.gridtype = gridtype; a.align = align_corners != 0; a.interp = interp;
    a.stream = reinterpret_cast<hipStream_t>(stream);
    if (dtype != LAE_F32 && dtype != LAE_F16) return LAE_EINVAL;
    const bool staged = blc && C == 2 && L <= 32;
    void* lbc = nullptr;
    if (staged) {
        lbc = lae::workspace(lae::WS_GRID_OUT_T, (size_t)B * L * C * (dtype == LAE_F16 ? 2 : 4), a.stream);
        if (!lbc) return LAE_ELAUNCH;
        a.out = lbc;
    }
    const bool level_major = !blc || staged;
    a.os_b = level_major ? C : (uint64_t)L * C;
    a.os_l = level_major ? (uint64_t)B * C : C;
    if (dtype == LAE_F32) rc = dispatch_fwd_d<float>(a, D, C);
    else rc = dispatch_fwd_d<half_t>(a, D, C);
    if (rc) return rc;
    if (staged) {
        if (dtype == LAE_F16) k_out_transpose<half_t><<<lae::cdiv(B, 256), 256, 0, a.stream>>>((const half_t*)lbc, (half_t*)outputs, B, L);
        else k_out_transpose<float><<<lae::cdiv(B, 256), 256, 0, a.stream>>>((const float*)lbc, (float*)outputs, B, L);
    }
    return lae::check_launch("grid_encode_forward");
}

struct PlanLayout { size_t totals_off, offs_off, cnt_off, part_off, bytes; };
static inline uint32_t bwd_units(uint32_t B) { return lae::cdiv(B, UNIT_SAMPLES * SEGS) * SEGS; }
static inline PlanLayout plan_layout(uint32_t B, uint32_t L) {
    const size_t U = bwd_units(B);
    auto up = [](size_t v) { return (v + 255) / 256 * 256; };
    PlanLayout w;
    w.totals_off = up((size_t)TICKET_WORDS * 4);
    w.offs_off = w.totals_off + up((size_t)L * BK_MAX * 4);
    w.cnt_off = w.offs_off + up((size_t)L * BK_MAX * 4);
    w.part_off = w.cnt_off + up((size_t)L * U * BK_MAX * 2);
    w.bytes = w.part_off + up((size_t)L * BK_MAX * U * 4);
    return w;
}
static inline BwdPlan plan_at(void* buf, uint32_t B, uint32_t L) {
    const PlanLayout lay = plan_layout(B, L);
    uint8_t* p = reinterpret_cast<uint8_t*>(buf);
    BwdPlan plan;
    plan.tickets = reinterpret_cast<uint32_t*>(p);
    plan.totals = reinterpret_cast<uint32_t*>(p + lay.totals_off);
    plan.offs = reinterpret_cast<uint32_t*>(p + lay.offs_off);
    plan.cnt = reinterpret_cast<uint16_t*>(p + lay.cnt_off);
    plan.part_cnt = reinterpret_cast<uint32_t*>(p + lay.part_off);
    return plan;
}
static inline size_t merge_bytes() { return ((size_t)MAX_LEVELS * SUB_RECS * sub_rec_words<half_t>() * 8 + 255) / 256 * 256; }
template <typename T>
static inline size_t bwd_exec_ws_bytes(uint32_t B, uint32_t L) {
    auto up = [](size_t v) { return (v + 255) / 256 * 256; };
    const size_t cap = (size_t)L * bwd_units(B) * UNIT_SAMPLES * 8;
    return merge_bytes() + up(cap * sizeof(typename BVal<T>::type)) + up(cap * 2);
}

template <typename T>
static void bwd_plan(const float* inputs, const int32_t* offsets, uint32_t B, uint32_t L, const BwdArgs& a, const BwdPlan& plan) {
    const uint32_t U = bwd_units(B);
    size_t line_lds = 0;
    if (a.touched) {
        uint32_t words = ((1u << 21) >> 3 >> 5) + 2;
        if (a.offsets_host) {
            words = 1;
// ... 16 lines not shown
static int launch_bwd_fast(const void* gT, const float* inputs, const int32_t* offsets, void* gemb, uint32_t B, uint32_t L,
                           const BwdArgs& a, const void* caller_plan = nullptr) {
    using V = typename BVal<T>::type;
    auto up = [](size_t v) { return (v + 255) / 256 * 256; };
    const uint32_t U = bwd_units(B);
    const size_t plan_bytes = caller_plan ? 0 : plan_layout(B, L).bytes;
    uint8_t* ws = reinterpret_cast<uint8_t*>(lae::workspace(lae::WS_GRID_BINS, plan_bytes + bwd_exec_ws_bytes<T>(B, L), a.stream));
    if (!ws) return LAE_ELAUNCH;
    unsigned long long* partials = reinterpret_cast<unsigned long long*>(ws);
    {
        static std::mutex mtx;
        static std::vector<void*> zeroed;
        static uint64_t epoch = 0;
        std::lock_guard<std::mutex> lk(mtx);
        if (epoch != lae::workspace_epoch()) { zeroed.clear(); epoch = lae::workspace_epoch(); }
        if (std::find(zeroed.begin(), zeroed.end(), (void*)ws) == zeroed.end()) {
            if (hipMemsetAsync(ws, 0, merge_bytes(), a.stream) != hipSuccess) {
                (void)hipGetLastError();
                lae::set_last_error_str("grid backward: could not zero the merge records (first call inside a capture? warm up eagerly)");
                return LAE_ELAUNCH;
            }
            if (zeroed.size() > 64) zeroed.clear();
            zeroed.push_back((void*)ws);
        }
    }
    const BwdPlan plan = plan_at(caller_plan ? const_cast<void*>(caller_plan) : ws + merge_bytes(), B, L);
    uint8_t* ex = ws + merge_bytes() + plan_bytes;
    const size_t cap = (size_t)L * U * UNIT_SAMPLES * 8;
    V* qvals = reinterpret_cast<V*>(ex);
    uint16_t* qkeys = reinterpret_cast<uint16_t*>(ex + up(cap * sizeof(V)));
    const T* g = (const T*)gT;
    T* ge = (T*)gemb;
    if (!caller_plan) bwd_plan<T>(inputs, offsets, B, L, a, plan);
#ifdef LAE_GRID_BWD_PHASE_PROBE
    const char* phase_env = getenv("LAE_GRID_BWD_PHASE");
    const int phase_probe = phase_env ? atoi(phase_env) : 0;
    if (phase_probe != 2)
#endif
    if (a.gridtype == 0 && !a.align && a.interp == 0)
        k_bwd_walk<T, true, true><<<U / SEGS * L, FILL_THREADS, 0, a.stream>>>(g, inputs, offsets, B, L, a.sc, a.gridtype, a.align, a.interp, U, plan, qvals, qkeys, nullptr, nullptr);
    else
        k_bwd_walk<T, true, false><<<U / SEGS * L, FILL_THREADS, 0, a.stream>>>(g, inputs, offsets, B, L, a.sc, a.gridtype, a.align, a.interp, U, plan, qvals, qkeys, nullptr, nullptr);
#ifdef LAE_GRID_BWD_PHASE_PROBE
    if (phase_probe == 1) return lae::check_launch("grid backward (fill-only probe)");
#endif
    static const uint32_t bk_env = [] { const char* e = getenv("LAE_GRID_BWD_BK_TARGET"); return e ? (uint32_t)std::min(std::max(atoi(e), 1), (int)SUB_RECS) : 0u; }();
    static_assert(BK_TARGET <= SUB_RECS && 64u <= SUB_RECS, "bk_target choices must fit the merge records");
    const uint32_t bk_target = std::min(bk_env ? bk_env : (B >= 400000u ? 64u : BK_TARGET), SUB_RECS);
    k_bwd_acc<T><<<(uint32_t)lae::num_cus() * 2, ACC_THREADS, 0, a.stream>>>(offsets, ge, L, a.sc, a.gridtype, a.align, plan, qvals, qkeys, partials, a.nf_flag, bk_target);
    bool need_generic = true;
    if (a.offsets_host) {
        need_generic = false;
        for (uint32_t l = 0; l < L; l++)
            if (!level_is_binned((uint32_t)(a.offsets_host[l + 1] - a.offsets_host[l]))) need_generic = true;
    }
    if (need_generic) {
        const uint32_t nbg = lae::cdiv(B, GRID_BLOCK);
        k_grid_bwd<T, 3, 2><<<nbg * L, GRID_BLOCK, 0, a.stream>>>(g, inputs, offsets, ge, B, L, a.sc, a.gridtype, a.align, a.interp, nbg,
                                                                  (L % 8) == 0, 2, (uint64_t)B * 2, true);
    }
    return LAE_OK;
}

static inline size_t touched_words(const int32_t* offsets_host, uint32_t L) { return ((size_t)offsets_host[L] >> 3 >> 5) + 2; }

static int g_force_atomic_bwd = 0;

static int grid_backward(const void* grad, const float* inputs, const void* embeddings, const int32_t* offsets,
                         void* grad_embeddings, uint32_t B, uint32_t D, uint32_t C, uint32_t L, float S, uint32_t H,
                         const void* dy_dx, void* grad_inputs, uint32_t gridtype, int align_corners, uint32_t interp,
                         int dtype, bool blc, void* stream, float in_shift = 0.0f, float in_scale = 1.0f,
                         const int32_t* offsets_host = nullptr, const void* plan = nullptr, int32_t* nf_flag = nullptr,
                         uint32_t* touched = nullptr) {
    (void)embeddings;
    if (B == 0) return LAE_OK;
    if (!grad || !inputs || !offsets || !grad_embeddings) return LAE_ENULL;
    if (plan && !(D == 3 && C == 2 && L <= 32 && B <= BWD_MAX_SAMPLES && !blc && !g_force_atomic_bwd)) return LAE_EINVAL;
    if (gridtype > 1 || interp > 1) return LAE_EINVAL;
    if (touched && dtype != LAE_F16) return LAE_EINVAL;
    if (nf_flag || touched) {
        if (!(D == 3 && C == 2 && L <= 32 && B <= BWD_MAX_SAMPLES && !g_force_atomic_bwd) || !offsets_host) return LAE_EINVAL;
        for (uint32_t l = 0; l < L; l++)
            if (!level_is_binned((uint32_t)(offsets_host[l + 1] - offsets_host[l]))) return LAE_EINVAL;
    }
    BwdArgs a;
    a.offsets_host = offsets_host;
    a.nf_flag = nf_flag;
    a.touched = touched;
    if (touched) a.touched_full = touched + touched_words(offsets_host, L);
    a.grad = grad; a.inputs = inputs; a.offsets = offsets; a.gemb = grad_embeddings; a.B = B; a.L = L;
    int rc = fill_scales(a.sc, L, S, H);
    if (rc) return rc;
    a.sc.in_shift = in_shift; a.sc.in_scale = in_scale;
    a.gridtype = gridtype; a.align = align_corners != 0; a.interp = interp;
    a.gs_b = blc ? (uint64_t)L * C : C;
    a.gs_l = blc ? C : (uint64_t)B * C;
    a.stream = reinterpret_cast<hipStream_t>(stream);
    if (dtype != LAE_F32 && dtype != LAE_F16) return LAE_EINVAL;
    if (D == 3 && C == 2 && L <= 32 && B <= BWD_MAX_SAMPLES && !g_force_atomic_bwd) {
        const size_t esz = dtype == LAE_F16 ? 2 : 4;
        const void* gT = grad;
        if (blc) {
            void* ws = lae::workspace(lae::WS_GRID_GRAD_T, (size_t)B * L * 2 * esz, a.stream);
            if (!ws) return LAE_ELAUNCH;
            if (dtype == LAE_F16) k_grad_transpose<half_t><<<lae::cdiv(B, 256), 256, 0, a.stream>>>((const half_t*)grad, (half_t*)ws, B, L);
            else k_grad_transpose<float><<<lae::cdiv(B, 256), 256, 0, a.stream>>>((const float*)grad, (float*)ws, B, L);
            gT = ws;
        }
        rc = (dtype == LAE_F16) ? launch_bwd_fast<half_t>(gT, inputs, offsets, grad_embeddings, B, L, a, plan)
                                : launch_bwd_fast<float>(gT, inputs, offsets, grad_embeddings, B, L, a, plan);
        if (rc) return rc;
        rc = LAE_OK;
    } else if (dtype == LAE_F32) rc = dispatch_bwd_d<float>(a, D, C);
    else rc = dispatch_bwd_d<half_t>(a, D, C);
    if (rc) return rc;
    if (dy_dx && grad_inputs) {
        const uint32_t n = B * D;
        if (dtype == LAE_F32)
            k_grid_input_bwd<float><<<lae::cdiv(n, 256), 256, 0, a.stream>>>((const float*)grad, (const float*)dy_dx,
                                                                            (float*)grad_inputs, B, D, C, L, a.gs_b, a.gs_l);
        else
            k_grid_input_bwd<half_t><<<lae::cdiv(n, 256), 256, 0, a.stream>>>((const half_t*)grad, (const half_t*)dy_dx,
// ... 33 lines not shown
    a.stream = stream; a.os_b = 2; a.os_l = (uint64_t)B_cap * 2;
    a.B_dev = B_dev; a.B_launch = std::min(B_launch, B_cap); a.B_likely = std::min(B_likely, a.B_launch);
    launch_fwd<half_t, 3, 2>(a);
    return LAE_OK;
}

extern "C" {

int lae_grid_encode_forward(const float* inputs, const void* embeddings, const int32_t* offsets, void* outputs,
                            uint32_t B, uint32_t D, uint32_t C, uint32_t L, float S, uint32_t H, void* dy_dx,
                            uint32_t gridtype, int align_corners, uint32_t interp, int dtype, void* stream) {
    return grid_forward(inputs, embeddings, offsets, outputs, B, D, C, L, S, H, dy_dx, gridtype, align_corners, interp,
                        dtype, false, stream);
}
int lae_grid_encode_backward(const void* grad, const float* inputs, const void* embeddings, const int32_t* offsets,
                             void* grad_embeddings, uint32_t B, uint32_t D, uint32_t C, uint32_t L, float S, uint32_t H,
                             const void* dy_dx, void* grad_inputs, uint32_t gridtype, int align_corners,
                             uint32_t interp, int dtype, void* stream) {
    return grid_backward(grad, inputs, embeddings, offsets, grad_embeddings, B, D, C, L, S, H, dy_dx, grad_inputs,
                         gridtype, align_corners, interp, dtype, false, stream);
}

int lae_grid_encode_forward_ex(const float* inputs, const void* embeddings, const int32_t* offsets, void* outputs,
                               uint32_t B, uint32_t D, uint32_t C, uint32_t L, float S, uint32_t H, void* dy_dx,
                               uint32_t gridtype, int align_corners, uint32_t interp, int dtype, int blc, float in_shift,
                               float in_scale, const int32_t* offsets_host, void* stream) {
    return grid_forward(inputs, embeddings, offsets, outputs, B, D, C, L, S, H, dy_dx, gridtype, align_corners, interp,
                        dtype, blc != 0, stream, in_shift, in_scale, offsets_host);
}
int lae_grid_encode_backward_ex(const void* grad, const float* inputs, const void* embeddings, const int32_t* offsets,
                                void* grad_embeddings, uint32_t B, uint32_t D, uint32_t C, uint32_t L, float S,
                                uint32_t H, const void* dy_dx, void* grad_inputs, uint32_t gridtype,
                                int align_corners, uint32_t interp, int dtype, int blc, float in_shift, float in_scale,
                                const int32_t* offsets_host, int32_t* nonfinite_flag, uint32_t* touched_lines, void* stream) {
    return grid_backward(grad, inputs, embeddings, offsets, grad_embeddings, B, D, C, L, S, H, dy_dx, grad_inputs,
                         gridtype, align_corners, interp, dtype, blc != 0, stream, in_shift, in_scale, offsets_host, nullptr,
                         nonfinite_flag, touched_lines);
}

uint64_t lae_grid_backward_workspace_bytes(uint32_t B, uint32_t L, int dtype) {
    return plan_layout(B, L).bytes + (dtype == LAE_F16 ? bwd_exec_ws_bytes<half_t>(B, L) : bwd_exec_ws_bytes<float>(B, L));
}

uint64_t lae_grid_backward_plan_bytes(uint32_t B, uint32_t L) { return plan_layout(B, L).bytes; }

uint64_t lae_grid_touched_lines_words(uint64_t n_entries) { return (n_entries >> 3 >> 5) + 2 + MAX_LEVELS; }

int lae_grid_encode_backward_plan(const float* inputs, const int32_t* offsets, uint32_t B, uint32_t D, uint32_t C, uint32_t L, float S,
                                  uint32_t H, uint32_t gridtype, int align_corners, uint32_t interp, int dtype, float in_shift,
                                  float in_scale, const int32_t* offsets_host, void* plan, uint32_t* touched_lines, void* stream) {
    if (B == 0) return LAE_OK;
    if (!inputs || !offsets || !plan) return LAE_ENULL;
    if (D != 3 || C != 2 || L > 32 || B > BWD_MAX_SAMPLES || gridtype > 1 || interp > 1 || (dtype != LAE_F32 && dtype != LAE_F16)) return LAE_EINVAL;
    if (touched_lines) {
        if (!offsets_host || dtype != LAE_F16 || g_force_atomic_bwd) return LAE_EINVAL;
        for (uint32_t l = 0; l < L; l++)
            if (!level_is_binned((uint32_t)(offsets_host[l + 1] - offsets_host[l]))) return LAE_EINVAL;
    }
    BwdArgs a;
    a.offsets_host = offsets_host;
    a.touched = touched_lines;
    if (touched_lines) a.touched_full = touched_lines + touched_words(offsets_host, L);
    a.grad = nullptr; a.inputs = inputs; a.offsets = offsets; a.gemb = nullptr; a.B = B; a.L = L;
    int rc = fill_scales(a.sc, L, S, H);
    if (rc) return rc;
    a.sc.in_shift = in_shift; a.sc.in_scale = in_scale;
    a.gridtype = gridtype; a.align = align_corners != 0; a.interp = interp;
    a.gs_b = C; a.gs_l = (uint64_t)B * C;
    a.stream = reinterpret_cast<hipStream_t>(stream);
    if (dtype == LAE_F16) bwd_plan<half_t>(inputs, offsets, B, L, a, plan_at(plan, B, L));
    else bwd_plan<float>(inputs, offsets, B, L, a, plan_at(plan, B, L));
    return lae::check_launch("grid_encode_backward_plan");
}

int lae_grid_encode_backward_planned(const void* grad, const float* inputs, const int32_t* offsets, void* grad_embeddings, uint32_t B,
                                     uint32_t D, uint32_t C, uint32_t L, float S, uint32_t H, uint32_t gridtype, int align_corners,
                                     uint32_t interp, int dtype, float in_shift, float in_scale, const int32_t* offsets_host,
                                     const void* plan, int32_t* nonfinite_flag, void* stream) {
    if (!plan) return LAE_ENULL;
    return grid_backward(grad, inputs, nullptr, offsets, grad_embeddings, B, D, C, L, S, H, nullptr, nullptr, gridtype, align_corners,
                         interp, dtype, false, stream, in_shift, in_scale, offsets_host, plan, nonfinite_flag, nullptr);
}

int lae_grid_forward_schedule(const int32_t* offsets_host, uint32_t L, float S, uint32_t H, uint32_t n_chunks, uint32_t* nseg_out,
                              uint32_t* segs_out) {
    if (!offsets_host || !nseg_out || !segs_out) return LAE_ENULL;
    LevelScales sc;
    if (fill_scales(sc, L, S, H) != LAE_OK || L > 8 * FWD_MAX_SEG) return LAE_EINVAL;
    FwdSched fs;
    const uint32_t per_xcd = fwd_sched_build(fs, L, n_chunks, sc, offsets_host);
    for (int x = 0; x < 8; x++) {
        nseg_out[x] = fs.nseg[x];
        for (uint32_t q = 0; q < fs.nseg[x]; q++) {
            uint32_t* o = segs_out + ((size_t)x * FWD_MAX_SEG + q) * 3;
            o[0] = fs.seg[x][q].level; o[1] = fs.seg[x][q].c0; o[2] = fs.seg[x][q].n;
        }
    }
    return (int)per_xcd;
}

int lae_grid_set_forward_mode(int mode) {
    if (mode < 0 || mode > 2) return LAE_EINVAL;
    g_fwd_mode = mode;
    return LAE_OK;
}

int lae_grid_set_backward_mode(int mode) {
    if (mode != 0 && mode != 1) return LAE_EINVAL;
    g_force_atomic_bwd = mode;
    return LAE_OK;
}

int lae_grad_total_variation(const void* inputs, const void* embeddings, void* grad, const int32_t* offsets,
                             float weight, uint32_t B, uint32_t D, uint32_t C, uint32_t L, float S, uint32_t H,
// ... 30 lines not shown
```

### laenerf_amd/csrc/lae_common.h

```cpp
#pragma once
#include <hip/hip_runtime.h>
#include <stdint.h>
#include "../../include/laenerf.h"

#define LAE_WAVE 64

namespace lae {

void set_last_error(const char* what, hipError_t e);

enum WsSlot { WS_FFMLP_SLABS = 0, WS_GRID_GRAD_T = 1, WS_GRID_OUT_T = 2, WS_GRID_BINS = 3, WS_SLOTS = 4 };
void* workspace(WsSlot slot, size_t bytes, hipStream_t stream);
size_t workspace_bytes(bool retired);
uint64_t workspace_epoch();
void free_workspaces();
int num_cus();
void set_last_error_str(const char* what);

int grid_forward_frame(const float* inputs, const void* embeddings, const int32_t* offsets, void* outputs, uint32_t B_cap,
                       uint32_t B_launch, const uint32_t* B_dev, uint32_t L, float S, uint32_t H, uint32_t gridtype,
                       int align_corners, uint32_t interp, float in_shift, float in_scale, hipStream_t stream,
                       const int32_t* offsets_host, uint32_t B_likely = 0);
struct FrameCtrl { uint32_t n_alive, n_step, n_rows, step, iter, done, total_rows, pad; };
static_assert(sizeof(FrameCtrl) == 32, "FrameCtrl layout");
__host__ __device__ __forceinline__ uint32_t frame_rays_per_group(uint32_t n_step) { return 64u / n_step; }
struct __attribute__((aligned(16))) RayAcc { float ws, depth, r, g, b, t, wse, de; };
static_assert(sizeof(RayAcc) == 32, "RayAcc layout");
struct FrameHeadArgs {
    const FrameCtrl* cur;
    const int32_t* alive;
    const float* deltas;
    const uint8_t* edit_occ;
    RayAcc* acc;
    int32_t* seg_next;
    uint32_t* seg_counts_next;
    uint32_t* blk_counts_next;
    uint32_t R;
    float T_thresh;
};
constexpr int FRAME_HEAD_WAVES = 8;
int nerf_head_composite_frame(const void* enc, const float* dirs, const void* sigma_weights, const void* color_weights,
                              uint32_t M_cap, float density_scale, const FrameHeadArgs& fa, bool edit, uint32_t n_blocks,
                              hipStream_t stream);
uint32_t frame_head_max_blocks();

static inline int check_launch(const char* what) {
    hipError_t e = hipGetLastError();
    if (e != hipSuccess) { set_last_error(what, e); return LAE_ELAUNCH; }
    return LAE_OK;
}

static inline uint32_t cdiv(uint64_t a, uint64_t b) { return (uint32_t)((a + b - 1) / b); }

__device__ __forceinline__ float clampf(float x, float lo, float hi) { return fminf(hi, fmaxf(lo, x)); }

template <int CTRL, int ROW_MASK>
__device__ __forceinline__ uint32_t dpp_u32(uint32_t v) {
    return (uint32_t)__builtin_amdgcn_update_dpp(0, (int)v, CTRL, ROW_MASK, 0xf, false);
}
__device__ __forceinline__ uint32_t wave_incl_scan(uint32_t v) {
    v += dpp_u32<0x111, 0xf>(v); v += dpp_u32<0x112, 0xf>(v); v += dpp_u32<0x114, 0xf>(v); v += dpp_u32<0x118, 0xf>(v);
    v += dpp_u32<0x142, 0xa>(v);
    v += dpp_u32<0x143, 0xc>(v);
    return v;
}

template <int NW>
__device__ __forceinline__ uint32_t block_excl_scan(uint32_t v, uint32_t* total, uint32_t* lds ) {
    const int lane = threadIdx.x & 63, w = threadIdx.x >> 6;
    uint32_t inc = wave_incl_scan(v);
    if (lane == 63) lds[w] = inc;
    __syncthreads();
    if (threadIdx.x == 0) {
        uint32_t s = 0;
#pragma unroll
        for (int i = 0; i < NW; i++) { uint32_t t = lds[i]; lds[i] = s; s += t; }
        lds[NW] = s;
    }
// ... 9 lines not shown
```

### laenerf_amd/csrc/optimizer.hip

```cpp
#include "lae_common.h"
#include <hip/hip_fp16.h>

#define STREAM(s) reinterpret_cast<hipStream_t>(s)

namespace {

typedef _Float16 half_t;

struct OptState {
    float scale;
    int32_t growth_tracker;
    int32_t found_inf;
    int32_t skip;
    int32_t step;
    float inv_bc1;
    float bc2_sqrt;
    float inv_scale;
    int32_t skipped_total;
    float next_inv_bc1;
    float next_bc2_sqrt;
    int32_t next_for;
    float next_beta1;
    float next_beta2;
    int32_t pad[2];
// ... 100 lines not shown
            float4 pp = *reinterpret_cast<const float4*>(p + i), mm = *reinterpret_cast<const float4*>(m + i),
                   vv = *reinterpret_cast<const float4*>(v + i);
            adam1(pp.x, mm.x, vv.x, g[0] * inv_scale, lr_over_bc1, bc2_sqrt, h);
            adam1(pp.y, mm.y, vv.y, g[1] * inv_scale, lr_over_bc1, bc2_sqrt, h);
            adam1(pp.z, mm.z, vv.z, g[2] * inv_scale, lr_over_bc1, bc2_sqrt, h);
            adam1(pp.w, mm.w, vv.w, g[3] * inv_scale, lr_over_bc1, bc2_sqrt, h);
            *reinterpret_cast<float4*>(p + i) = pp;
            *reinterpret_cast<float4*>(m + i) = mm;
            *reinterpret_cast<float4*>(v + i) = vv;
            if (shadow) {
                half_t s[4] = {(half_t)pp.x, (half_t)pp.y, (half_t)pp.z, (half_t)pp.w};
                *reinterpret_cast<uint2*>(shadow + i) = *reinterpret_cast<const uint2*>(s);
            }
        } else {
            for (size_t j = i; j < n; j++) {
                const float gj = ldg(grad, j) * inv_scale;
                grad[j] = (G)0.0f;
                if (skip) continue;
                float pj = p[j], mj = m[j], vj = v[j];
                adam1(pj, mj, vj, gj, lr_over_bc1, bc2_sqrt, h);
                p[j] = pj; m[j] = mj; v[j] = vj;
                if (shadow) shadow[j] = (half_t)pj;
            }
        }
    }
}

constexpr int MAX_SEGS = 8;
struct CheckSegs { const void* grad[MAX_SEGS]; size_t n[MAX_SEGS]; int is_half[MAX_SEGS]; int count; };
struct ApplySegs {
    float* p[MAX_SEGS]; float* m[MAX_SEGS]; float* v[MAX_SEGS]; void* grad[MAX_SEGS]; half_t* shadow[MAX_SEGS];
    const float* lr[MAX_SEGS]; size_t n[MAX_SEGS]; int is_half[MAX_SEGS]; int count;
    const uint32_t* touched[MAX_SEGS];
};

template <typename G>
__device__ __forceinline__ bool seg_has_nonfinite(const G* __restrict__ grad, size_t n) {
    bool bad = false;
    const size_t stride = (size_t)gridDim.x * blockDim.x * 8;
    for (size_t i = ((size_t)blockIdx.x * blockDim.x + threadIdx.x) * 8; i < n; i += stride) {
        if (i + 8 <= n) {
            if constexpr (sizeof(G) == 2) {
                const uint4 v = *reinterpret_cast<const uint4*>(grad + i);
                const uint32_t w[4] = {v.x, v.y, v.z, v.w};
#pragma unroll
                for (int k = 0; k < 4; k++) bad |= ((w[k] & 0x7c00u) == 0x7c00u) || ((w[k] & 0x7c000000u) == 0x7c000000u);
            } else {
                const float4 a = *reinterpret_cast<const float4*>(grad + i), b = *reinterpret_cast<const float4*>(grad + i + 4);
                bad |= !isfinite(a.x) || !isfinite(a.y) || !isfinite(a.z) || !isfinite(a.w) || !isfinite(b.x) || !isfinite(b.y) ||
                       !isfinite(b.z) || !isfinite(b.w);
            }
        } else {
            for (size_t j = i; j < n; j++) bad |= !isfinite(ldg(grad, j));
        }
    }
    return bad;
}

__global__ __launch_bounds__(256) void k_check_multi(CheckSegs sg, OptState* __restrict__ st) {
    bool bad = false;
    for (int s = 0; s < sg.count; s++)
        bad |= sg.is_half[s] ? seg_has_nonfinite((const half_t*)sg.grad[s], sg.n[s]) : seg_has_nonfinite((const float*)sg.grad[s], sg.n[s]);
    if (__any(bad) && (threadIdx.x & 63) == 0) atomicOr(&st->found_inf, 1);
}

template <typename G>
// ... 21 lines not shown
            }
            if (skip) continue;
            float4 pp = *reinterpret_cast<const float4*>(p + i), mm = *reinterpret_cast<const float4*>(m + i),
                   vv = *reinterpret_cast<const float4*>(v + i);
            adam1(pp.x, mm.x, vv.x, g[0] * inv_scale, lr_over_bc1, bc2_sqrt, h);
            adam1(pp.y, mm.y, vv.y, g[1] * inv_scale, lr_over_bc1, bc2_sqrt, h);
            adam1(pp.z, mm.z, vv.z, g[2] * inv_scale, lr_over_bc1, bc2_sqrt, h);
            adam1(pp.w, mm.w, vv.w, g[3] * inv_scale, lr_over_bc1, bc2_sqrt, h);
            *reinterpret_cast<float4*>(p + i) = pp;
            *reinterpret_cast<float4*>(m + i) = mm;
            *reinterpret_cast<float4*>(v + i) = vv;
            if (shadow) {
                half_t s[4] = {(half_t)pp.x, (half_t)pp.y, (half_t)pp.z, (half_t)pp.w};
                *reinterpret_cast<uint2*>(shadow + i) = *reinterpret_cast<const uint2*>(s);
            }
        } else {
            for (size_t j = i; j < n; j++) {
                const float gj = ldg(grad, j) * inv_scale;
                grad[j] = (G)0.0f;
                if (skip) continue;
                float pj = p[j], mj = m[j], vj = v[j];
                adam1(pj, mj, vj, gj, lr_over_bc1, bc2_sqrt, h);
                p[j] = pj; m[j] = mj; v[j] = vj;
                if (shadow) shadow[j] = (half_t)pj;
            }
        }
    }
}

__global__ __launch_bounds__(256) void k_apply_multi(ApplySegs sg, OptState* __restrict__ st, AdamHyper h) {
    const bool skip = st->skip != 0;
    const float inv_scale = st->inv_scale, bc2_sqrt = st->bc2_sqrt;
    if (blockIdx.x == gridDim.x - 1 && threadIdx.x == 0) prepare_next_step(st, h.beta1, h.beta2);
    for (int s = 0; s < sg.count; s++) {
        const float lr_over_bc1 = (float)((double)sg.lr[s][0] * (double)st->inv_bc1);
        if (sg.is_half[s]) seg_apply(sg.p[s], sg.m[s], sg.v[s], (half_t*)sg.grad[s], sg.shadow[s], sg.n[s], skip, inv_scale, bc2_sqrt, lr_over_bc1, h, sg.touched[s]);
        else seg_apply(sg.p[s], sg.m[s], sg.v[s], (float*)sg.grad[s], sg.shadow[s], sg.n[s], skip, inv_scale, bc2_sqrt, lr_over_bc1, h, sg.touched[s]);
    }
}

struct EmaSegs { float* shadow[MAX_SEGS]; const float* param[MAX_SEGS]; size_t n[MAX_SEGS]; int count; };
__device__ __forceinline__ void ema_segs(const EmaSegs& sg, float one_minus_decay) {
    const size_t stride = (size_t)gridDim.x * 256 * 4;
    for (int s = 0; s < sg.count; s++) {
        float* __restrict__ sh = sg.shadow[s];
        const float* __restrict__ p = sg.param[s];
        const size_t n = sg.n[s], n4 = n & ~(size_t)3;
        for (size_t i = ((size_t)blockIdx.x * 256 + threadIdx.x) * 4; i < n4; i += stride) {
            float4 a = *reinterpret_cast<const float4*>(sh + i);
            const float4 b = *reinterpret_cast<const float4*>(p + i);
            a.x -= (a.x - b.x) * one_minus_decay; a.y -= (a.y - b.y) * one_minus_decay;
            a.z -= (a.z - b.z) * one_minus_decay; a.w -= (a.w - b.w) * one_minus_decay;
            *reinterpret_cast<float4*>(sh + i) = a;
        }
        if (blockIdx.x == 0 && threadIdx.x < n - n4) { const size_t j = n4 + threadIdx.x; sh[j] -= (sh[j] - p[j]) * one_minus_decay; }
    }
}
__global__ __launch_bounds__(256) void k_ema_multi(EmaSegs sg, float one_minus_decay) { ema_segs(sg, one_minus_decay); }

__global__ __launch_bounds__(256) void k_ema_gated(EmaSegs sg, const int64_t* __restrict__ step, int64_t epoch_len, int32_t* count,
                                                   double decay, int use_num_updates) {
    __shared__ float s_omd;
    __shared__ int s_go;
    if (threadIdx.x == 0) {
        const int64_t s = __hip_atomic_load(step, __ATOMIC_RELAXED, __HIP_MEMORY_SCOPE_AGENT);
        const int go = s > 0 && s % epoch_len == 0;
// ... 62 lines not shown
    EmaSegs sg{};
    size_t biggest = 0;
    for (uint32_t i = 0; i < n_tensors; i++) {
        if (sizes[i] && (!shadows[i] || !params[i])) return LAE_ENULL;
        if ((reinterpret_cast<uintptr_t>(shadows[i]) | reinterpret_cast<uintptr_t>(params[i])) & 15) return LAE_EINVAL;
        sg.shadow[i] = shadows[i]; sg.param[i] = params[i]; sg.n[i] = sizes[i];
        biggest = std::max(biggest, (size_t)sizes[i]);
    }
    sg.count = (int)n_tensors;
    k_ema_multi<<<stream_blocks(biggest, 4), 256, 0, STREAM(stream)>>>(sg, one_minus_decay);
    return lae::check_launch("ema_update_multi");
}

int lae_ema_update_gated(uint32_t n_tensors, float* const* shadows, const float* const* params, const uint64_t* sizes, const int64_t* step,
                         int64_t epoch_len, int32_t* count, double decay, int use_num_updates, void* stream) {
    if (n_tensors == 0) return LAE_OK;
    if (!shadows || !params || !sizes || !step || !count) return LAE_ENULL;
    if (n_tensors > (uint32_t)MAX_SEGS || epoch_len < 1) return LAE_EINVAL;
    EmaSegs sg{};
    size_t biggest = 0;
    for (uint32_t i = 0; i < n_tensors; i++) {
        if (sizes[i] && (!shadows[i] || !params[i])) return LAE_ENULL;
        if ((reinterpret_cast<uintptr_t>(shadows[i]) | reinterpret_cast<uintptr_t>(params[i])) & 15) return LAE_EINVAL;
        sg.shadow[i] = shadows[i]; sg.param[i] = params[i]; sg.n[i] = sizes[i];
        biggest = std::max(biggest, (size_t)sizes[i]);
    }
    sg.count = (int)n_tensors;
    k_ema_gated<<<stream_blocks(biggest, 4), 256, 0, STREAM(stream)>>>(sg, step, epoch_len, count, decay, use_num_updates);
    return lae::check_launch("ema_update_gated");
}

int lae_adam_apply_multi(uint32_t n_tensors, float* const* params, float* const* exp_avgs, float* const* exp_avg_sqs, void* const* grads,
                         const int* grad_is_half, void* const* shadows_half, const uint64_t* sizes, const float* const* lrs,
                         const void* const* touched_lines, const void* state, float beta1, float beta2, float eps, float weight_decay,
                         void* stream) {
    if (n_tensors == 0) return LAE_OK;
    if (!params || !exp_avgs || !exp_avg_sqs || !grads || !grad_is_half || !shadows_half || !sizes || !lrs || !state) return LAE_ENULL;
    if (n_tensors > (uint32_t)MAX_SEGS) return LAE_EINVAL;
    ApplySegs sg{};
    size_t biggest = 0;
    for (uint32_t i = 0; i < n_tensors; i++) {
        if (sizes[i] && (!params[i] || !exp_avgs[i] || !exp_avg_sqs[i] || !grads[i] || !lrs[i])) return LAE_ENULL;
        const uintptr_t al = reinterpret_cast<uintptr_t>(params[i]) | reinterpret_cast<uintptr_t>(exp_avgs[i]) |
                             reinterpret_cast<uintptr_t>(exp_avg_sqs[i]) | reinterpret_cast<uintptr_t>(grads[i]) |
                             reinterpret_cast<uintptr_t>(shadows_half[i]);
        if (al & 15) return LAE_EINVAL;
        sg.p[i] = params[i]; sg.m[i] = exp_avgs[i]; sg.v[i] = exp_avg_sqs[i]; sg.grad[i] = grads[i];
        sg.shadow[i] = (half_t*)shadows_half[i]; sg.lr[i] = lrs[i]; sg.n[i] = sizes[i]; sg.is_half[i] = grad_is_half[i];
        sg.touched[i] = (touched_lines && weight_decay == 0.0f) ? (const uint32_t*)touched_lines[i] : nullptr;
        biggest = std::max(biggest, (size_t)sizes[i]);
    }
    sg.count = (int)n_tensors;
    k_apply_multi<<<stream_blocks(biggest, 4), 256, 0, STREAM(stream)>>>(sg, reinterpret_cast<OptState*>(const_cast<void*>(state)),
                                                                        AdamHyper{beta1, beta2, eps, weight_decay});
    return lae::check_launch("adam_apply_multi");
}

int lae_adam_begin(void* state, float beta1, float beta2, int growth_interval, float growth_factor, float backoff_factor,
                   int use_scaler, void* stream) {
    if (!state) return LAE_ENULL;
    k_begin<<<1, 64, 0, STREAM(stream)>>>(reinterpret_cast<OptState*>(state), beta1, beta2, growth_interval, growth_factor,
                                          backoff_factor, use_scaler);
    return lae::check_launch("adam_begin");
}

int lae_adam_apply(float* param, float* exp_avg, float* exp_avg_sq, void* grad, int grad_is_half, void* shadow_half, uint64_t n,
                   const void* state, const float* lr, float beta1, float beta2, float eps, float weight_decay, void* stream) {
    if (n == 0) return LAE_OK;
    if (!param || !exp_avg || !exp_avg_sq || !grad || !state || !lr) return LAE_ENULL;
    const uintptr_t al = reinterpret_cast<uintptr_t>(param) | reinterpret_cast<uintptr_t>(exp_avg) | reinterpret_cast<uintptr_t>(exp_avg_sq) |
                         reinterpret_cast<uintptr_t>(grad) | reinterpret_cast<uintptr_t>(shadow_half);
    if (al & 15) return LAE_EINVAL;
    const AdamHyper h{beta1, beta2, eps, weight_decay};
    OptState* st = reinterpret_cast<OptState*>(const_cast<void*>(state));
    if (grad_is_half)
        k_apply<half_t><<<stream_blocks(n, 4), 256, 0, STREAM(stream)>>>(param, exp_avg, exp_avg_sq, (half_t*)grad, (half_t*)shadow_half, n, st, lr, h);
    else
        k_apply<float><<<stream_blocks(n, 4), 256, 0, STREAM(stream)>>>(param, exp_avg, exp_avg_sq, (float*)grad, (half_t*)shadow_half, n, st, lr, h);
    return lae::check_launch("adam_apply");
}

}
// ... 1 lines not shown
```

### laenerf_amd/editing/style_encoder.py

```python
import torch
import torch.nn as nn
from torch.autograd import Function
from torch.amp import custom_bwd, custom_fwd

from ..backend import style_backend as _backend
from ..encoding import get_encoder
from ..ffmlp import FFMLP


class _palette_recompose(Function):
    @staticmethod
    @custom_fwd(device_type="cuda")
    def forward(ctx, w_logits, o_raw, palette, active_mask):
        M = w_logits.shape[0]
        w_logits, o_raw = w_logits.half().contiguous(), o_raw.half().contiguous()
        palette = palette.float().contiguous()
        P = palette.shape[0]
        n_active = bin(active_mask & ((1 << P) - 1)).count("1")
        dev = w_logits.device
        pred = torch.empty(M, 3, dtype=torch.half, device=dev)
        w_hat = torch.empty(M, n_active, dtype=torch.float32, device=dev)
        o_hat = torch.empty(M, 3, dtype=torch.half, device=dev)
        _backend.palette_forward(w_logits, o_raw, palette, P, active_mask, M, pred, w_hat, o_hat)
        ctx.save_for_backward(w_logits, o_raw, palette)
# ... 95 lines not shown
        _grid.grid_encode_forward(x, table, enc.offsets, feats, M, 3, 2, L, S, H, None, enc.gridtype_id, enc.align_corners,
                                  enc.interp_id, blc=False, in_map=in_map, offsets_host=enc.offsets_host)
        feat = torch.empty(Mp, 32, device=x.device, dtype=torch.half)
        off_in = torch.empty(Mp, off_cols, device=x.device, dtype=torch.half) if degree else None
        _backend.style_assemble_forward(feats, d.float().contiguous() if degree else None, M, Mp, degree, feat, off_in, off_cols)
        ctx.save_for_backward(x, table)
        ctx.enc, ctx.in_map, ctx.geom, ctx.off_cols, ctx.plan = enc, in_map, (M, L, S, H), off_cols, plan
        return (feat, off_in) if degree else (feat, feat)

    @staticmethod
    @custom_bwd(device_type="cuda")
    def backward(ctx, g_feat, g_off):
        from ..backend import gridencoder_backend as _grid
        x, table = ctx.saved_tensors
        enc = ctx.enc
        M, L, S, H = ctx.geom
        if g_feat is None and g_off is None:
            return (None,) * 8
        g_feat = None if g_feat is None else g_feat.to(torch.half).contiguous()
        g_off = None if g_off is None else g_off.to(torch.half).contiguous()
        off_cols = ctx.off_cols if g_off is not None and g_off.shape[1] != 32 else 32
        grad_feats = torch.empty(L, M, 2, device=x.device, dtype=torch.half)
        _backend.style_assemble_backward(g_feat, g_off, M, off_cols, grad_feats)
        grad_table = enc.shadow.grad_half if enc.shadow is not None else torch.zeros_like(table)
        flag = enc.shadow.flag_for_backward(M) if enc.shadow is not None else None
        touched = enc.shadow.touched_for_backward(M) if flag is not None else None
        if ctx.plan is not None and touched is not None and not getattr(ctx.plan, "marks_touched", False):
            touched = None
        if enc.shadow is not None and touched is None:
            enc.shadow.unreported = enc.shadow.unreported or flag is None
            enc.shadow.mark_all_touched()
        _grid.grid_encode_backward(grad_feats, x, table, enc.offsets, grad_table, M, 3, 2, L, S, H, None, None, enc.gridtype_id,
                                   enc.align_corners, enc.interp_id, blc=False, in_map=ctx.in_map, offsets_host=enc.offsets_host,
                                   plan=ctx.plan, nonfinite_flag=flag, touched_lines=touched)
        return None, None, (None if enc.shadow is not None else grad_table), None, None, None, None, None


class LAENeRF(nn.Module):

    def __init__(self, params, encoding="hashgrid", dir_encoding=None, num_layers=3, hidden_dim=64, color_palette=None, size=256,
                 style_img=None, vgg=None, style_generator=None):
        super().__init__()
        self.opt = params
        self.bound = params.bound
        self.encoder, self.in_dim = get_encoder(encoding, desired_resolution=2048 * self.bound, num_levels=16, log2_hashmap_size=19)
        self.num_layers = num_layers
        self.hidden_dim = hidden_dim
        self.num_color_bases = params.num_palette_bases
        if not 0 < self.num_color_bases <= 16:
            raise ValueError("LAENeRF: 1..16 palette bases (the MLP output tile is 16 wide)")
        self.register_buffer("active_palets", torch.ones(self.num_color_bases, dtype=torch.bool))
        self._active_mask = (1 << self.num_color_bases) - 1
        pal = color_palette if color_palette is not None else torch.rand(self.num_color_bases, 3, dtype=torch.float32)
        self.color_palette = nn.Parameter(pal.detach().clone().float())
        self.original_color_palette = None
        self.size = size
        self.dir_encoding, self.in_dim_dir = None, 0
        if dir_encoding is not None:
            self.dir_encoding, self.in_dim_dir = get_encoder(dir_encoding, degree=3)
        self.offset_in_dim = (self.in_dim + self.in_dim_dir + 15) // 16 * 16
        self.offset_net = FFMLP(self.offset_in_dim, 3, hidden_dim, num_layers - 1)
        self.weight_net = FFMLP(self.in_dim, self.num_color_bases, hidden_dim, num_layers - 1)
        self.style_transfer_net = None
        if float(getattr(params, "style_weight", 0) or 0) > 0:
            from . import style_network as sn
            style_img = style_img if style_img is not None else getattr(params, "style_image", None)
            vgg = vgg if vgg is not None else getattr(params, "vgg_weights", None)
# ... 156 lines not shown
```

### laenerf_amd/field.py

```python
import numpy as np
import torch
from torch.autograd import Function
from torch.amp import custom_bwd, custom_fwd

from .backend import ffmlp_backend as _mlp
from .backend import gridencoder_backend as _grid
from .ffmlp.head import COLOR_NET_PARAMS, SIGMA_NET_PARAMS


class _nerf_field(Function):
    calls = 0

    @staticmethod
    @custom_fwd(device_type="cuda")
    def forward(ctx, x, dirs, embeddings, sigma_weights, color_weights, enc, sigma_shadow, color_shadow, bound, density_scale, plan=None):
        _nerf_field.calls += 1
        M = x.shape[0]
        L = enc.num_levels
        x = x.float().contiguous()
        dirs = dirs.float().contiguous()
        table = enc.shadow.table_half(embeddings) if enc.shadow is not None else embeddings.to(torch.half)
        shadows = (sigma_shadow, color_shadow) if sigma_shadow is not None and color_shadow is not None else None
        if shadows is not None:
            ws, wc = sigma_shadow.table_half(sigma_weights), color_shadow.table_half(color_weights)
# ... 1 lines not shown
            ws, wc = sigma_weights.half().contiguous(), color_weights.half().contiguous()
        in_map = (float(bound), float(np.float32(1.0) / np.float32(2 * bound)))
        S, H = np.log2(enc.per_level_scale), enc.base_resolution
        feats = torch.empty(L, M, 2, device=x.device, dtype=torch.half)
        _grid.grid_encode_forward(x, table, enc.offsets, feats, M, 3, 2, L, S, H, None, enc.gridtype_id, enc.align_corners,
                                  enc.interp_id, blc=False, in_map=in_map, offsets_host=enc.offsets_host)
        h = torch.empty(M, 16, device=x.device, dtype=torch.half)
        sigmas = torch.empty(M, device=x.device, dtype=torch.float32)
        rgbs = torch.empty(M, 3, device=x.device, dtype=torch.float32)
        _mlp.nerf_head_forward(feats, dirs, ws, wc, M, density_scale, h, sigmas, rgbs, level_major=True)
        ctx.save_for_backward(x, dirs, table, ws, wc, feats, h, rgbs)
        ctx.enc, ctx.shadows, ctx.in_map, ctx.geom = enc, shadows, in_map, (M, L, S, H)
        ctx.density_scale = density_scale
        ctx.plan = plan
        ctx.wdtypes = (sigma_weights.dtype, color_weights.dtype)
        return sigmas, rgbs

    @staticmethod
    @custom_bwd(device_type="cuda")
    def backward(ctx, grad_sigmas, grad_rgbs):
        x, dirs, table, ws, wc, feats, h, rgbs = ctx.saved_tensors
        enc = ctx.enc
        M, L, S, H = ctx.geom
        grad_sigmas = grad_sigmas.float().contiguous()
        grad_rgbs = grad_rgbs.float().contiguous()
        grad_h = torch.empty_like(h)
        grad_feats = torch.empty_like(feats)
        wflag = None
        if ctx.shadows is not None:
            gws, gwc = ctx.shadows[0].grad_half, ctx.shadows[1].grad_half
            wflag = _weights_flag(ctx.shadows)
        else:
            gws, gwc = torch.empty_like(ws), torch.empty_like(wc)
        _mlp.nerf_head_backward(grad_sigmas, grad_rgbs, feats, dirs, h, rgbs, ws, wc, M, ctx.density_scale, grad_h, grad_feats,
                                gws, gwc, accumulate=ctx.shadows is not None, level_major=True, nonfinite_flag=wflag)
        grad_table = enc.shadow.grad_half if enc.shadow is not None else torch.zeros_like(table)
        flag = enc.shadow.flag_for_backward(M) if enc.shadow is not None else None
        touched = enc.shadow.touched_for_backward(M) if flag is not None else None
        if ctx.plan is not None and touched is not None and not getattr(ctx.plan, "marks_touched", False):
            touched = None
        if enc.shadow is not None and touched is None:
            enc.shadow.mark_all_touched()
        _grid.grid_encode_backward(grad_feats, x, table, enc.offsets, grad_table, M, 3, 2, L, S, H, None, None, enc.gridtype_id,
                                   enc.align_corners, enc.interp_id, blc=False, in_map=ctx.in_map, offsets_host=enc.offsets_host, plan=ctx.plan,
                                   nonfinite_flag=flag, touched_lines=touched)
        return (None, None, None if enc.shadow is not None else grad_table,
                None if ctx.shadows is not None else gws.to(ctx.wdtypes[0]),
                None if ctx.shadows is not None else gwc.to(ctx.wdtypes[1]), None, None, None, None, None, None)


def _weights_flag(shadows):
    a, b = shadows[0].flag_for_backward(), shadows[1].flag_for_backward()
    if a is not None and a == b:
        return a
    shadows[0].unreported = shadows[1].unreported = True
    return None


def field_supported(enc, sigma_net, color_net):
    return (enc.input_dim == 3 and enc.level_dim == 2 and enc.num_levels == 16
            and sigma_net.weights.numel() == SIGMA_NET_PARAMS and color_net.weights.numel() == COLOR_NET_PARAMS)


def nerf_field(x, dirs, enc, sigma_net, color_net, bound=1, density_scale=1.0, plan=None):
    if x.shape[0] % 16 != 0:
        raise RuntimeError("nerf_field: the number of samples must be a multiple of 16")
    return _nerf_field.apply(x, dirs, enc.embeddings, sigma_net.weights, color_net.weights, enc, sigma_net.shadow,
                             color_net.shadow, float(bound), float(density_scale), plan)


@torch.no_grad()
def field_backward_plan(x, enc, bound=1):
    x = x.float().contiguous()
    if x.shape[0] > (1 << 24):
        return None
    in_map = (float(bound), float(np.float32(1.0) / np.float32(2 * bound)))
    touched = enc.shadow.touched_for_backward(x.shape[0]) if enc.shadow is not None else None
    return _grid.grid_backward_plan(x, enc.offsets, x.shape[0], 3, 2, enc.num_levels, np.log2(enc.per_level_scale), enc.base_resolution,
# ... 22 lines not shown
```

### laenerf_amd/gridencoder/grid.py

```python
import numpy as np
import torch
import torch.nn as nn
from torch.autograd import Function
from torch.amp import custom_bwd, custom_fwd

from ..backend import gridencoder_backend as _backend

_gridtype_to_id = {"hash": 0, "tiled": 1}
_interp_to_id = {"linear": 0, "smoothstep": 1}


class _grid_encode(Function):

    @staticmethod
    @custom_fwd(device_type="cuda")
    def forward(ctx, inputs, embeddings, offsets, per_level_scale, base_resolution, calc_grad_inputs=False, gridtype=0,
                align_corners=False, interpolation=0, shadow=None, in_map=(0.0, 1.0), offsets_host=None):
        inputs = inputs.contiguous()
        B, D = inputs.shape
        L = offsets.shape[0] - 1
        C = embeddings.shape[1]
        S = np.log2(per_level_scale)
        H = base_resolution
        ctx.shadow = None
# ... 1 lines not shown
            if shadow is not None:
                embeddings = shadow.table_half(embeddings)
                ctx.shadow = shadow
            else:
                embeddings = embeddings.to(torch.half)
        outputs = torch.empty(B, L * C, device=inputs.device, dtype=embeddings.dtype)
        dy_dx = torch.empty(B, L * D * C, device=inputs.device, dtype=embeddings.dtype) if calc_grad_inputs else None
        _backend.grid_encode_forward(inputs, embeddings, offsets, outputs, B, D, C, L, S, H, dy_dx, gridtype,
                                     align_corners, interpolation, blc=True, in_map=in_map, offsets_host=offsets_host)
        ctx.offsets_host = offsets_host
        ctx.save_for_backward(inputs, embeddings, offsets, dy_dx)
        ctx.dims = [B, D, C, L, S, H, gridtype, interpolation]
        ctx.in_map = in_map
        ctx.align_corners = align_corners
        return outputs

    @staticmethod
    @custom_bwd(device_type="cuda")
    def backward(ctx, grad):
        inputs, embeddings, offsets, dy_dx = ctx.saved_tensors
        B, D, C, L, S, H, gridtype, interpolation = ctx.dims
        grad = grad.contiguous()
        if grad.dtype != embeddings.dtype:
            grad = grad.to(embeddings.dtype)
        grad_embeddings = ctx.shadow.grad_half if ctx.shadow is not None else torch.zeros_like(embeddings)
        grad_inputs = torch.zeros_like(inputs, dtype=embeddings.dtype) if dy_dx is not None else None
        flag = ctx.shadow.flag_for_backward(B) if ctx.shadow is not None and D == 3 and C == 2 else None
        touched = ctx.shadow.touched_for_backward(B) if flag is not None and grad.dtype == torch.half else None
        if ctx.shadow is not None and (flag is None or touched is None):
            ctx.shadow.unreported = ctx.shadow.unreported or flag is None
            ctx.shadow.mark_all_touched()
        _backend.grid_encode_backward(grad, inputs, embeddings, offsets, grad_embeddings, B, D, C, L, S, H, dy_dx,
                                      grad_inputs, gridtype, ctx.align_corners, interpolation, blc=True, in_map=ctx.in_map,
                                      offsets_host=ctx.offsets_host, nonfinite_flag=flag, touched_lines=touched)
        if dy_dx is not None:
            grad_inputs = grad_inputs.to(inputs.dtype)
            if ctx.in_map[1] != 1.0:
                grad_inputs = grad_inputs * ctx.in_map[1]
        return (grad_inputs, (None if ctx.shadow is not None else grad_embeddings), None, None, None, None, None, None, None,
                None, None, None)


class TableShadow:

    def __init__(self, embeddings):
        self.half = embeddings.detach().to(torch.half).contiguous()
        n = self.half.numel()
        self.grad_store = torch.zeros((n + 839) // 840 * 840, dtype=torch.half, device=self.half.device)
        self.grad_half = self.grad_store[:n].view_as(self.half)
        self.version = embeddings._version
        self.nonfinite_flag = None
        self.unreported = False
        self.touched_lines = None

    def mark_all_touched(self):
        if self.touched_lines is not None:
            self.touched_lines.fill_(-1)

    def flag_for_backward(self, n_samples=0):
        if self.nonfinite_flag is None or n_samples > (1 << 24):
            self.unreported = True
            self.mark_all_touched()
            return None
        return self.nonfinite_flag

    def touched_for_backward(self, n_samples=0):
        if self.touched_lines is None or self.nonfinite_flag is None or n_samples > (1 << 24):
            return None
        return self.touched_lines.data_ptr()

    def table_half(self, embeddings):
        if embeddings._version != self.version:
            self.half.copy_(embeddings.detach())
            self.version = embeddings._version
        return self.half


grid_encode = _grid_encode.apply


def level_offsets(input_dim, num_levels, per_level_scale, base_resolution, log2_hashmap_size, align_corners):
    offsets, offset = [], 0
    max_params = 2 ** log2_hashmap_size
    for i in range(num_levels):
        resolution = int(np.ceil(base_resolution * per_level_scale ** i))
        n = min(max_params, (resolution if align_corners else resolution + 1) ** input_dim)
# ... 79 lines not shown
```

### laenerf_amd/optim.py

```python
import ctypes
import os

import numpy as np
import torch

from . import _lib
from .ffmlp import FFMLP
from .gridencoder import GridEncoder


_direct_grad = {"depth": 0}


class FusedAdam(torch.optim.Optimizer):
    def __init__(self, model, lr=1e-2, betas=(0.9, 0.99), eps=1e-15, weight_decay=0.0, param_groups=None,
                 grad_scaler=True, init_scale=2.0 ** 16, growth_factor=2.0, backoff_factor=0.5, growth_interval=2000, device_lr=False):
        groups = param_groups if param_groups is not None else [{"params": [p for p in model.parameters() if p.requires_grad], "lr": lr}]
        groups = [{**g, "params": [p for p in g["params"] if p.requires_grad]} for g in groups]
        super().__init__(groups, dict(lr=lr, betas=tuple(betas), eps=eps, weight_decay=weight_decay))
        self.betas, self.eps, self.weight_decay = betas, eps, weight_decay
        self.use_scaler = bool(grad_scaler)
        self.growth_factor, self.backoff_factor, self.growth_interval = growth_factor, backoff_factor, growth_interval
        tables = {id(m.embeddings): m for m in model.modules() if isinstance(m, GridEncoder) and m.level_dim % 2 == 0}
        tables.update({id(m.weights): m for m in model.modules() if isinstance(m, FFMLP)})
        self.items = []
        dev = None
        for gi, g in enumerate(self.param_groups):
            for p in g["params"]:
                if not p.is_cuda or p.dtype != torch.float32 or not p.is_contiguous():
                    raise RuntimeError("FusedAdam: parameters must be contiguous fp32 tensors on the GPU (no CPU fallback)")
                dev = p.device
                shadow = None
                owner = tables.get(id(p))
                if owner is not None:
                    shadow = owner.attach_shadow()
                else:
                    p.grad = torch.zeros_like(p)
                    p._lae_persistent_grad = True
                m, v = torch.zeros_like(p), torch.zeros_like(p)
                self.state[p] = {"step": torch.tensor(0.0), "exp_avg": m, "exp_avg_sq": v}
                self.items.append((p, m, v, shadow, gi))
        if dev is None:
            raise ValueError("FusedAdam: no parameter to optimise")
        self.dev_state = torch.zeros(16, dtype=torch.int32, device=dev)
        if self.use_scaler:
            for p, _, _, shadow, _ in self.items:
                owner = tables.get(id(p))
                if shadow is not None and isinstance(owner, GridEncoder) and owner.input_dim == 3 and owner.level_dim == 2 \
                        and owner.num_levels <= 32 and int((owner.offsets_host[1:] - owner.offsets_host[:-1]).max()) <= (1 << 21):
                    shadow.nonfinite_flag = self.dev_state.data_ptr() + 8
                    if weight_decay == 0 and not os.environ.get("LAE_ADAM_NO_TOUCHED_LINES"):
                        n_words = int(_lib.load().lae_grid_touched_lines_words(p.shape[0]))
                        shadow.touched_lines = torch.zeros(n_words, dtype=torch.int32, device=p.device)
                elif shadow is not None and isinstance(owner, FFMLP):
                    shadow.nonfinite_flag = self.dev_state.data_ptr() + 8
        self._scale_view = self.dev_state.view(torch.float32)
        self._scale_view[0] = init_scale if self.use_scaler else 1.0
        self.device_lr = bool(device_lr)
        self._lr_host = [float(g["lr"]) for g in self.param_groups]
        self.lrs = torch.tensor(self._lr_host, dtype=torch.float32, device=dev)
        if len(self.items) > 8:
            raise RuntimeError("FusedAdam: at most 8 parameter tensors (one multi-tensor launch)")
        self._args = None

    def scale(self, loss):
        return loss * self._scale_view[0] if self.use_scaler else loss

    def backward(self, loss):
        key = (tuple(loss.shape), loss.dtype, str(loss.device))
        cache = self.__dict__.setdefault("_root_grads", {})
        one = cache.get(key)
        if one is None:
            one = cache[key] = torch.ones(loss.shape, dtype=loss.dtype, device=loss.device)
            from .raymarching.raymarching import register_unit_root_grad
            register_unit_root_grad(one)
        _direct_grad["depth"] += 1
        try:
            loss.backward(gradient=one)
        finally:
            _direct_grad["depth"] -= 1
        self.finish_loss()

    @staticmethod
    def finish_loss():
        from .backend import flush_pending_loss
        flush_pending_loss()

    def get_scale(self):
# ... 14 lines not shown
        self.sync_lr()

    def sync_lr(self):
        if self.device_lr:
            return
        cur = [float(g["lr"]) for g in self.param_groups]
        if cur != self._lr_host:
            if torch.cuda.is_current_stream_capturing():
                raise RuntimeError("FusedAdam: a learning rate changed inside a stream capture; call sync_lr() outside the capture")
            st = self.__dict__.setdefault("_lr_stage", {"bufs": [torch.empty(len(cur), dtype=torch.float32).pin_memory() for _ in range(2)],
                                                        "evs": [None, None], "k": 0})
            k = st["k"]
            if st["evs"][k] is not None:
                st["evs"][k].synchronize()
            st["bufs"][k].copy_(torch.tensor(cur, dtype=torch.float32))
            self.lrs.copy_(st["bufs"][k], non_blocking=True)
            ev = st["evs"][k] or torch.cuda.Event()
            ev.record()
            st["evs"][k] = ev
            st["k"] = 1 - k
            self._lr_host = cur

    def sync_shadows(self):
        for p, _, _, shadow, _ in self.items:
            if shadow is not None:
                shadow.half.copy_(p.detach())
                shadow.version = p._version

    def zero_grad(self, set_to_none=False):
        self.dev_state[2:3].zero_()
        for p, _, _, shadow, _ in self.items:
            if shadow is not None:
                shadow.grad_half.zero_()
                p.grad = None
            elif p.grad is not None:
                p.grad.zero_()

    def _grad(self, p, shadow):
        if shadow is not None:
            if p.grad is not None:
                shadow.grad_half.add_(p.grad.to(torch.half))
                p.grad = None
                if hasattr(shadow, "unreported"):
                    shadow.unreported = True
                    shadow.mark_all_touched()
            return shadow.grad_half, 1
        if p.grad is None:
            p.grad = torch.zeros_like(p)
        if p.grad.dtype != torch.float32 or not p.grad.is_contiguous():
            raise RuntimeError("FusedAdam: fp32 contiguous .grad expected")
        return p.grad, 0

    def _tables(self):
        grads = [self._grad(p, sh) for p, _, _, sh, _ in self.items]
        key = tuple(g.data_ptr() for g, _ in grads)
        if self._args is None or self._args["key"] != key:
            n = len(self.items)
            arr = lambda vals: (ctypes.c_void_p * n)(*vals)
            self._args = {
                "key": key, "n": n,
                "grads": arr(key), "is_half": (ctypes.c_int * n)(*[h for _, h in grads]),
                "sizes": (ctypes.c_uint64 * n)(*[p.numel() for p, *_ in self.items]),
                "params": arr([p.data_ptr() for p, *_ in self.items]),
                "m": arr([m.data_ptr() for _, m, *_ in self.items]), "v": arr([v.data_ptr() for _, _, v, *_ in self.items]),
                "shadows": arr([None if sh is None else sh.half.data_ptr() for _, _, _, sh, _ in self.items]),
                "lrs": arr([self.lrs.data_ptr() + 4 * gi for *_, gi in self.items]),
                "touched": arr([None if sh is None or getattr(sh, "touched_lines", None) is None else sh.touched_lines.data_ptr()
                                for _, _, _, sh, _ in self.items]),
            }
        return self._args

    @torch.no_grad()
    def step(self, closure=None):
        if closure is not None:
            raise RuntimeError("FusedAdam.step: closures are not supported")
        self.sync_lr()
        self.finish_loss()
        lib, st, s = _lib.load(), self.dev_state.data_ptr(), _lib.stream()
        a = self._tables()
        for *_, shadow, _ in self.items:
            if shadow is not None and getattr(shadow, "unreported", False) and hasattr(shadow, "mark_all_touched"):
                shadow.mark_all_touched()
        if self.use_scaler:
            c = self._check_tables(a)
            if c["n"]:
                _lib.check(lib.lae_adam_check_multi(c["n"], c["grads"], c["is_half"], c["sizes"], st, s), "adam_check")
        _lib.check(lib.lae_adam_begin(st, self.betas[0], self.betas[1], self.growth_interval, self.growth_factor,
                                      self.backoff_factor, int(self.use_scaler), s), "adam_begin")
        _lib.check(lib.lae_adam_apply_multi(a["n"], a["params"], a["m"], a["v"], a["grads"], a["is_half"], a["shadows"],
                                            a["sizes"], a["lrs"], a["touched"], st, self.betas[0], self.betas[1], self.eps,
                                            self.weight_decay, s), "adam_apply")
        for *_, shadow, _ in self.items:
            if shadow is not None and hasattr(shadow, "unreported"):
                shadow.unreported = False

    def _check_tables(self, a):
        keep = tuple(not (sh is not None and getattr(sh, "nonfinite_flag", None) is not None and not sh.unreported)
                     for _, _, _, sh, _ in self.items)
        cached = a.get("check")
        if cached is None or cached["keep"] != keep:
            idx = [i for i, k in enumerate(keep) if k]
            n = len(idx)
            arr = (ctypes.c_void_p * max(n, 1))
            cached = a["check"] = {"keep": keep, "n": n, "grads": arr(*[a["grads"][i] for i in idx]),
                                   "is_half": (ctypes.c_int * max(n, 1))(*[a["is_half"][i] for i in idx]),
                                   "sizes": (ctypes.c_uint64 * max(n, 1))(*[a["sizes"][i] for i in idx])}
        return cached

    def state_dict(self):
        step = float(self.steps_taken)
        for p, *_ in self.items:
            self.state[p]["step"] = torch.tensor(step)
        sd = super().state_dict()
        sd["scaler"] = {"scale": self.get_scale(), "growth_tracker": int(self.dev_state[1].item())}
        return sd

    def load_state_dict(self, sd):
        sd = dict(sd)
        scaler = sd.pop("scaler", None)
        keep = {id(p): (m, v) for p, m, v, _, _ in self.items}
        super().load_state_dict(sd)
        step = 0
        for p, m, v, _, _ in self.items:
# ... 109 lines not shown
```

Baseline: 11.17 Mrays/s.

## Fuse NeRF head backward with grid-encode backward and add grad-dirty word

```diff
diff --git a/include/laenerf.h b/include/laenerf.h
--- a/include/laenerf.h
+++ b/include/laenerf.h
@@ -34,7 +34,7 @@
 #define LAE_ACT_SOFTPLUS 5
 #define LAE_ACT_NONE 6
 
-#define LAE_ABI_TAG "abi14"
+#define LAE_ABI_TAG "abi15"
 LAE_API const char* lae_version(void);
 LAE_API const char* lae_last_error(void);
 
@@ -195,7 +195,8 @@
                                 void* grad_embeddings, uint32_t B, uint32_t D, uint32_t C, uint32_t L, float S,
                                 uint32_t H, const void* dy_dx, void* grad_inputs, uint32_t gridtype,
                                 int align_corners, uint32_t interp, int dtype, int blc, float in_shift, float in_scale,
-                                const int32_t* offsets_host, int32_t* nonfinite_flag, uint32_t* touched_lines, void* stream);
+                                const int32_t* offsets_host, int32_t* nonfinite_flag, uint32_t* touched_lines, uint32_t* grad_dirty,
+                                void* stream);
 
 LAE_API uint64_t lae_grid_backward_plan_bytes(uint32_t B, uint32_t L);
 LAE_API uint64_t lae_grid_touched_lines_words(uint64_t n_entries);
@@ -206,7 +207,8 @@
 LAE_API int lae_grid_encode_backward_planned(const void* grad, const float* inputs, const int32_t* offsets, void* grad_embeddings,
                                      uint32_t B, uint32_t D, uint32_t C, uint32_t L, float S, uint32_t H, uint32_t gridtype,
                                      int align_corners, uint32_t interp, int dtype, float in_shift, float in_scale,
-                                     const int32_t* offsets_host, const void* plan, int32_t* nonfinite_flag, void* stream);
+                                     const int32_t* offsets_host, const void* plan, int32_t* nonfinite_flag, uint32_t* grad_dirty,
+                                     void* stream);
 
 LAE_API uint64_t lae_grid_backward_workspace_bytes(uint32_t B, uint32_t L, int dtype);
 
@@ -266,6 +268,16 @@
                            void* grad_color_weights, int accumulate_weight_grads, int enc_level_major,
                            int32_t* nonfinite_flag, const float* loss_partials, uint32_t loss_n_part, uint32_t loss_n_elem,
                            const float* loss_scale, float* loss_out, void* stream);
+
+LAE_API int lae_nerf_field_backward(const float* grad_sigmas, const float* grad_rgbs, const void* enc, const float* dirs, const void* h,
+                            const float* rgbs, const void* sigma_weights, const void* color_weights, uint32_t M, float density_scale,
+                            void* grad_h, void* grad_enc, void* grad_sigma_weights, void* grad_color_weights,
+                            int accumulate_weight_grads, int32_t* weights_nonfinite_flag, const float* loss_partials,
+                            uint32_t loss_n_part, uint32_t loss_n_elem, const float* loss_scale, float* loss_out,
+                            const float* inputs, const int32_t* offsets, void* grad_embeddings, uint32_t L, float S, uint32_t H,
+                            uint32_t gridtype, int align_corners, uint32_t interp, float in_shift, float in_scale,
+                            const int32_t* offsets_host, const void* plan, int32_t* table_nonfinite_flag, uint32_t* touched_lines,
+                            uint32_t* grad_dirty, void* stream);
 
 LAE_API int lae_freq_encode_forward(const float* inputs, uint32_t B, uint32_t D, uint32_t deg, uint32_t C, float* outputs,
                             void* stream);
@@ -390,7 +402,7 @@
                          void* stream);
 LAE_API int lae_adam_apply_multi(uint32_t n_tensors, float* const* params, float* const* exp_avgs, float* const* exp_avg_sqs, void* const* grads,
                          const int* grad_is_half, void* const* shadows_half, const uint64_t* sizes, const float* const* lrs, const void* const* touched_lines,
-                         const void* state, float beta1, float beta2, float eps, float weight_decay, void* stream);
+                         void* const* grad_dirty, const void* state, float beta1, float beta2, float eps, float weight_decay, void* stream);
 
 LAE_API int lae_ema_update_multi(uint32_t n_tensors, float* const* shadows, const float* const* params, const uint64_t* sizes,
                          float one_minus_decay, void* stream);
diff --git a/laenerf_amd/_lib.py b/laenerf_amd/_lib.py
--- a/laenerf_amd/_lib.py
+++ b/laenerf_amd/_lib.py
@@ -47,12 +47,12 @@
     "lae_grid_encode_forward": [vp, vp, vp, vp, u32, u32, u32, u32, f32, u32, vp, u32, i32, u32, i32, vp],
     "lae_grid_encode_backward": [vp, vp, vp, vp, vp, u32, u32, u32, u32, f32, u32, vp, vp, u32, i32, u32, i32, vp],
     "lae_grid_encode_forward_ex": [vp, vp, vp, vp, u32, u32, u32, u32, f32, u32, vp, u32, i32, u32, i32, i32, f32, f32, vp, vp],
-    "lae_grid_encode_backward_ex": [vp, vp, vp, vp, vp, u32, u32, u32, u32, f32, u32, vp, vp, u32, i32, u32, i32, i32, f32, f32, vp, vp, vp, vp],
+    "lae_grid_encode_backward_ex": [vp, vp, vp, vp, vp, u32, u32, u32, u32, f32, u32, vp, vp, u32, i32, u32, i32, i32, f32, f32, vp, vp, vp, vp, vp],
     "lae_grid_backward_workspace_bytes": [u32, u32, i32],
     "lae_grid_backward_plan_bytes": [u32, u32],
     "lae_grid_touched_lines_words": [u64],
     "lae_grid_encode_backward_plan": [vp, vp, u32, u32, u32, u32, f32, u32, u32, i32, u32, i32, f32, f32, vp, vp, vp, vp],
-    "lae_grid_encode_backward_planned": [vp, vp, vp, vp, u32, u32, u32, u32, f32, u32, u32, i32, u32, i32, f32, f32, vp, vp, vp, vp],
+    "lae_grid_encode_backward_planned": [vp, vp, vp, vp, u32, u32, u32, u32, f32, u32, u32, i32, u32, i32, f32, f32, vp, vp, vp, vp, vp],
     "lae_grid_set_backward_mode": [i32],
     "lae_grid_set_forward_mode": [i32],
     "lae_grid_forward_schedule": [vp, u32, f32, u32, u32, vp, vp],
@@ -73,6 +73,8 @@
     "lae_density_grid_update": [vp, vp, u32, f32, f32, u32, vp, vp, vp],
     "lae_mark_untrained_grid": [vp, u32, f32, f32, f32, f32, u32, u32, f32, f32, i32, vp, vp],
     "lae_nerf_head_backward": [vp, vp, vp, vp, vp, vp, vp, vp, u32, f32, vp, vp, vp, vp, i32, i32, vp, vp, u32, u32, vp, vp, vp],
+    "lae_nerf_field_backward": [vp, vp, vp, vp, vp, vp, vp, vp, u32, f32, vp, vp, vp, vp, i32, vp, vp, u32, u32, vp, vp,
+                                vp, vp, vp, u32, f32, u32, u32, i32, u32, f32, f32, vp, vp, vp, vp, vp, vp],
     "lae_palette_forward": [vp, vp, vp, u32, u32, u32, vp, vp, vp, vp],
     "lae_palette_backward_scratch_bytes": [u32],
     "lae_palette_backward": [vp, vp, vp, u32, u32, u32, vp, vp, vp, vp, vp, vp, vp, vp],
@@ -101,7 +103,7 @@
     "lae_mse_loss_forward": [vp, vp, u32, vp, vp, vp, vp],
     "lae_adam_check": [vp, i32, u64, vp, vp],
     "lae_adam_check_multi": [u32, vp, vp, vp, vp, vp],
-    "lae_adam_apply_multi": [u32, vp, vp, vp, vp, vp, vp, vp, vp, vp, vp, f32, f32, f32, f32, vp],
+    "lae_adam_apply_multi": [u32, vp, vp, vp, vp, vp, vp, vp, vp, vp, vp, vp, f32, f32, f32, f32, vp],
     "lae_adam_begin": [vp, f32, f32, i32, f32, f32, i32, vp],
     "lae_ema_update_multi": [u32, vp, vp, vp, f32, vp],
     "lae_ema_update_gated": [u32, vp, vp, vp, vp, i64, vp, f64, i32, vp],
@@ -135,7 +137,7 @@
 }
 
 _lib = None
-ABI_TAG = b"abi14"
+ABI_TAG = b"abi15"
 
 
 def _abi_of(path):
diff --git a/laenerf_amd/backend.py b/laenerf_amd/backend.py
--- a/laenerf_amd/backend.py
+++ b/laenerf_amd/backend.py
@@ -397,7 +397,7 @@
     @staticmethod
     def grid_encode_backward(grad, inputs, embeddings, offsets, grad_embeddings, B, D, C, L, S, H, dy_dx, grad_inputs,
                              gridtype, align_corners, interp, blc=False, in_map=(0.0, 1.0), offsets_host=None, plan=None,
-                             nonfinite_flag=None, touched_lines=None):
+                             nonfinite_flag=None, touched_lines=None, grad_dirty=None):
         ts = (grad, inputs, embeddings, offsets, grad_embeddings, dy_dx, grad_inputs, plan)
         need_cuda(*ts); need_contig(*ts)
         if grad.dtype != grad_embeddings.dtype:
@@ -410,14 +410,15 @@
                 raise RuntimeError("grid_encode_backward: the plan was made without the touched-lines bitmap (pass it to grid_backward_plan)")
             check(lib.lae_grid_encode_backward_planned(ptr(grad), ptr(inputs), ptr(offsets), ptr(grad_embeddings), B, D, C, L, float(S), H,
                                                        gridtype, int(bool(align_corners)), interp, _dtype_code(grad), float(in_map[0]),
-                                                       float(in_map[1]), _host_i32(offsets_host, L + 1), ptr(plan), nonfinite_flag, stream()),
+                                                       float(in_map[1]), _host_i32(offsets_host, L + 1), ptr(plan), nonfinite_flag, grad_dirty, stream()),
                   "grid_encode_backward")
             return
         args = (ptr(grad), ptr(inputs), ptr(embeddings), ptr(offsets), ptr(grad_embeddings), B, D, C, L, float(S), H,
                 ptr(dy_dx), ptr(grad_inputs), gridtype, int(bool(align_corners)), interp, _dtype_code(grad))
-        if blc or tuple(in_map) != (0.0, 1.0) or offsets_host is not None or nonfinite_flag is not None or touched_lines is not None:
+        if (blc or tuple(in_map) != (0.0, 1.0) or offsets_host is not None or nonfinite_flag is not None or touched_lines is not None
+                or grad_dirty is not None):
             check(lib.lae_grid_encode_backward_ex(*args, int(bool(blc)), float(in_map[0]), float(in_map[1]), _host_i32(offsets_host, L + 1),
-                                                  nonfinite_flag, touched_lines, stream()), "grid_encode_backward")
+                                                  nonfinite_flag, touched_lines, grad_dirty, stream()), "grid_encode_backward")
         else:
             check(lib.lae_grid_encode_backward(*args, stream()), "grid_encode_backward")
 
@@ -533,25 +534,54 @@
               grad_sigma_weights, grad_color_weights)
         need_cuda(*ts); need_contig(*ts)
         _FFMLP._half(enc, h, sigma_weights, color_weights, grad_h, grad_enc, grad_sigma_weights, grad_color_weights)
+        _FFMLP._with_pending_loss(grad_sigmas, lambda lp, ln, le, lsc, lo: check(_lib.load().lae_nerf_head_backward(
+            ptr(grad_sigmas), ptr(grad_rgbs), ptr(enc), ptr(dirs), ptr(h), ptr(rgbs), ptr(sigma_weights), ptr(color_weights), M,
+            float(density_scale), ptr(grad_h), ptr(grad_enc), ptr(grad_sigma_weights), ptr(grad_color_weights), int(bool(accumulate)),
+            int(bool(level_major)), nonfinite_flag, ptr(lp), ln, le, ptr(lsc), ptr(lo), stream()), "nerf_head_backward"))
+
+    @staticmethod
+    def _with_pending_loss(grad_sigmas, call):
         key = _loss_key(grad_sigmas)
         pend = _pending_loss.get(key)
         if pend is not None and pend[5] != stream():
             pend = None
         if pend is not None:
             del _pending_loss[key]
-        lp, ln, le, lsc, lo = pend[:5] if pend is not None else (None, 0, 0, None, None)
         try:
-            check(_lib.load().lae_nerf_head_backward(ptr(grad_sigmas), ptr(grad_rgbs), ptr(enc), ptr(dirs), ptr(h), ptr(rgbs),
-                                                     ptr(sigma_weights), ptr(color_weights), M, float(density_scale),
-                                                     ptr(grad_h), ptr(grad_enc), ptr(grad_sigma_weights),
-                                                     ptr(grad_color_weights), int(bool(accumulate)), int(bool(level_major)),
-                                                     nonfinite_flag, ptr(lp), ln, le, ptr(lsc), ptr(lo), stream()), "nerf_head_backward")
+            call(*(pend[:5] if pend is not None else (None, 0, 0, None, None)))
         except RuntimeError:
             if pend is not None:
                 _pending_loss[key] = pend
             raise
         if pend is not None:
             deferred_loss_stats["carried"] += 1
+
+    @staticmethod
+    def nerf_field_backward(grad_sigmas, grad_rgbs, enc, dirs, h, rgbs, sigma_weights, color_weights, M, density_scale, grad_h, grad_enc,
+                            grad_sigma_weights, grad_color_weights, inputs, offsets, grad_embeddings, L, S, H, gridtype, align_corners,
+                            interp, accumulate=False, weights_nonfinite_flag=None, in_map=(0.0, 1.0), offsets_host=None, plan=None,
+                            table_nonfinite_flag=None, touched_lines=None, grad_dirty=None):
+        ts = (grad_sigmas, grad_rgbs, enc, dirs, h, rgbs, sigma_weights, color_weights, grad_h, grad_enc, grad_sigma_weights,
+              grad_color_weights, inputs, offsets, grad_embeddings, plan)
+        need_cuda(*ts); need_contig(*ts)
+        _FFMLP._half(enc, h, sigma_weights, color_weights, grad_h, grad_enc, grad_sigma_weights, grad_color_weights, grad_embeddings)
+        if plan is not None and touched_lines is not None and not getattr(plan, "marks_touched", False):
+            raise RuntimeError("nerf_field_backward: the plan was made without the touched-lines bitmap (pass it to grid_backward_plan)")
+        if _timing["on"]:
+            _FFMLP.nerf_head_backward(grad_sigmas, grad_rgbs, enc, dirs, h, rgbs, sigma_weights, color_weights, M, density_scale, grad_h,
+                                      grad_enc, grad_sigma_weights, grad_color_weights, accumulate=accumulate, level_major=True,
+                                      nonfinite_flag=weights_nonfinite_flag)
+            _GridEncoder.grid_encode_backward(grad_enc[:L], inputs, grad_embeddings, offsets, grad_embeddings, M, 3, 2, L, S, H, None, None,
+                                              gridtype, align_corners, interp, blc=False, in_map=in_map, offsets_host=offsets_host,
+                                              plan=plan, nonfinite_flag=table_nonfinite_flag, touched_lines=touched_lines,
+                                              grad_dirty=grad_dirty)
+            return
+        _FFMLP._with_pending_loss(grad_sigmas, lambda lp, ln, le, lsc, lo: check(_lib.load().lae_nerf_field_backward(
+            ptr(grad_sigmas), ptr(grad_rgbs), ptr(enc), ptr(dirs), ptr(h), ptr(rgbs), ptr(sigma_weights), ptr(color_weights), M,
+            float(density_scale), ptr(grad_h), ptr(grad_enc), ptr(grad_sigma_weights), ptr(grad_color_weights), int(bool(accumulate)),
+            weights_nonfinite_flag, ptr(lp), ln, le, ptr(lsc), ptr(lo), ptr(inputs), ptr(offsets), ptr(grad_embeddings), L, float(S), H,
+            gridtype, int(bool(align_corners)), interp, float(in_map[0]), float(in_map[1]), _host_i32(offsets_host, L + 1), ptr(plan),
+            table_nonfinite_flag, touched_lines, grad_dirty, stream()), "nerf_field_backward"))
 
     @staticmethod
     def ffmlp_set_mode(mode):
diff --git a/laenerf_amd/csrc/dw_reduce.h b/laenerf_amd/csrc/dw_reduce.h
--- /dev/null
+++ b/laenerf_amd/csrc/dw_reduce.h
@@ -0,0 +1,87 @@
+#pragma once
+#include <hip/hip_runtime.h>
+#include <stdint.h>
+#include <type_traits>
+
+namespace lae_dw {
+
+typedef _Float16 half_t;
+constexpr int DWR_GROUPS = 16;
+constexpr uint32_t DWR_THREADS = 64 * DWR_GROUPS;
+constexpr uint32_t DWR_LDS_FLOATS = DWR_GROUPS * 64;
+
+__device__ __forceinline__ void dw_reduce_body(const float* __restrict__ slabs, uint32_t n_slices, uint32_t nW, half_t* __restrict__ gw,
+                                               int accumulate, uint32_t block, int32_t* __restrict__ nf_flag, float* part) {
+    const uint32_t e = threadIdx.x & 63, sg = threadIdx.x >> 6;
+    const uint32_t i = block * 64 + e;
+    float s[8] = {0, 0, 0, 0, 0, 0, 0, 0};
+    if (i < nW) {
+        uint32_t k = sg;
+        for (; k + 7 * DWR_GROUPS < n_slices; k += 8 * DWR_GROUPS) {
+#pragma unroll
+            for (int u = 0; u < 8; u++) s[u] += slabs[(size_t)(k + u * DWR_GROUPS) * nW + i];
+        }
+        for (; k < n_slices; k += DWR_GROUPS) s[0] += slabs[(size_t)k * nW + i];
+    }
+    part[sg * 64 + e] = ((s[0] + s[1]) + (s[2] + s[3])) + ((s[4] + s[5]) + (s[6] + s[7]));
+    __syncthreads();
+    if (sg == 0 && i < nW) {
+        float t[DWR_GROUPS];
+#pragma unroll
+        for (int u = 0; u < DWR_GROUPS; u++) t[u] = part[u * 64 + e];
+#pragma unroll
+        for (int w = DWR_GROUPS / 2; w > 0; w >>= 1)
+#pragma unroll
+            for (int u = 0; u < w; u++) t[u] = t[u] + t[u + w];
+        const half_t r = accumulate ? (half_t)((float)gw[i] + t[0]) : (half_t)t[0];
+        gw[i] = r;
+        if (nf_flag && (__builtin_bit_cast(uint16_t, r) & 0x7c00u) == 0x7c00u) atomicOr(nf_flag, 1);
+    }
+}
+
+struct LossFinish { const float* partials; uint32_t n_part, n_elem; const float* scale; float* out; };
+__device__ __forceinline__ void loss_finish_block(const LossFinish& lf, float* part) {
+    static_assert(DWR_THREADS == 1024, "the loss sum is written for 16 waves, like k_loss_finish");
+    float acc = 0.0f;
+    for (uint32_t i = threadIdx.x; i < lf.n_part; i += 1024) acc += lf.partials[i];
+    {
+        auto dpp = [](float v, auto ctrl, auto mask) {
+            return __builtin_bit_cast(float, __builtin_amdgcn_update_dpp(0, __builtin_bit_cast(int, v), decltype(ctrl)::value, decltype(mask)::value, 0xf, false));
+        };
+        using std::integral_constant;
+        acc += dpp(acc, integral_constant<int, 0x111>{}, integral_constant<int, 0xf>{});
+        acc += dpp(acc, integral_constant<int, 0x112>{}, integral_constant<int, 0xf>{});
+        acc += dpp(acc, integral_constant<int, 0x114>{}, integral_constant<int, 0xf>{});
+        acc += dpp(acc, integral_constant<int, 0x118>{}, integral_constant<int, 0xf>{});
+        acc += dpp(acc, integral_constant<int, 0x142>{}, integral_constant<int, 0xa>{});
+        acc += dpp(acc, integral_constant<int, 0x143>{}, integral_constant<int, 0xc>{});
+        acc = __builtin_bit_cast(float, __builtin_amdgcn_readlane(__builtin_bit_cast(int, acc), 63));
+    }
+    if ((threadIdx.x & 63) == 0) part[threadIdx.x >> 6] = acc;
+    __syncthreads();
+    if (threadIdx.x == 0) {
+        float t = 0.0f;
+#pragma unroll
+        for (int w = 0; w < 16; w++) t += part[w];
+        const float loss = t / (float)lf.n_elem;
+        lf.out[0] = loss * (lf.scale ? lf.scale[0] : 1.0f);
+        lf.out[1] = loss;
+    }
+}
+
+struct DwTailJob {
+    const float* slabs_a; uint32_t n_a, nW_a; half_t* gw_a;
+    const float* slabs_b; uint32_t n_b, nW_b; half_t* gw_b;
+    uint32_t nb_a, nb_b;
+    int accumulate;
+    int32_t* nf_flag;
+    LossFinish lf;
+    uint32_t n_tasks;
+};
+__device__ __forceinline__ void dw_tail_task(const DwTailJob& j, uint32_t task, float* part) {
+    if (task < j.nb_a) dw_reduce_body(j.slabs_a, j.n_a, j.nW_a, j.gw_a, j.accumulate, task, j.nf_flag, part);
+    else if (task < j.nb_a + j.nb_b) dw_reduce_body(j.slabs_b, j.n_b, j.nW_b, j.gw_b, j.accumulate, task - j.nb_a, j.nf_flag, part);
+    else loss_finish_block(j.lf, part);
+}
+
+}
diff --git a/laenerf_amd/csrc/ffmlp.hip b/laenerf_amd/csrc/ffmlp.hip
--- a/laenerf_amd/csrc/ffmlp.hip
+++ b/laenerf_amd/csrc/ffmlp.hip
@@ -3,6 +3,7 @@
 #include <type_traits>
 #include <stdlib.h>
 #include "lae_common.h"
+#include "dw_reduce.h"
 
 namespace {
 
@@ -313,77 +314,16 @@
     }
 }
 
-constexpr int DWR_GROUPS = 16;
-__device__ __forceinline__ void dw_reduce_body(const float* __restrict__ slabs, uint32_t n_slices, uint32_t nW, half_t* __restrict__ gw,
-                                               int accumulate, uint32_t block, int32_t* __restrict__ nf_flag = nullptr) {
-    __shared__ float part[DWR_GROUPS][64];
-    const uint32_t e = threadIdx.x & 63, sg = threadIdx.x >> 6;
-    const uint32_t i = block * 64 + e;
-    float s[8] = {0, 0, 0, 0, 0, 0, 0, 0};
-    if (i < nW) {
-        uint32_t k = sg;
-        for (; k + 7 * DWR_GROUPS < n_slices; k += 8 * DWR_GROUPS) {
-#pragma unroll
-            for (int u = 0; u < 8; u++) s[u] += slabs[(size_t)(k + u * DWR_GROUPS) * nW + i];
-        }
-        for (; k < n_slices; k += DWR_GROUPS) s[0] += slabs[(size_t)k * nW + i];
-    }
-    part[sg][e] = ((s[0] + s[1]) + (s[2] + s[3])) + ((s[4] + s[5]) + (s[6] + s[7]));
-    __syncthreads();
-    if (sg == 0 && i < nW) {
-        float t[DWR_GROUPS];
-#pragma unroll
-        for (int u = 0; u < DWR_GROUPS; u++) t[u] = part[u][e];
-#pragma unroll
-        for (int w = DWR_GROUPS / 2; w > 0; w >>= 1)
-#pragma unroll
-            for (int u = 0; u < w; u++) t[u] = t[u] + t[u + w];
-        const half_t r = accumulate ? (half_t)((float)gw[i] + t[0]) : (half_t)t[0];
-        gw[i] = r;
-        if (nf_flag && (__builtin_bit_cast(uint16_t, r) & 0x7c00u) == 0x7c00u) atomicOr(nf_flag, 1);
-    }
-}
+using lae_dw::DWR_GROUPS;
+using lae_dw::LossFinish;
 __global__ __launch_bounds__(64 * DWR_GROUPS) void k_dw_reduce(const float* __restrict__ slabs, uint32_t n_slices, uint32_t nW,
                                                                half_t* __restrict__ gw, int accumulate = 0, int32_t* __restrict__ nf_flag = nullptr) {
-    dw_reduce_body(slabs, n_slices, nW, gw, accumulate, blockIdx.x, nf_flag);
-}
-struct LossFinish { const float* partials; uint32_t n_part, n_elem; const float* scale; float* out; };
-__global__ __launch_bounds__(64 * DWR_GROUPS) void k_dw_reduce2(const float* __restrict__ slabs_a, uint32_t n_a, uint32_t nW_a,
-                                                                half_t* __restrict__ gw_a, const float* __restrict__ slabs_b,
-                                                                uint32_t n_b, uint32_t nW_b, half_t* __restrict__ gw_b,
-                                                                uint32_t nb_a, uint32_t nb_b, int accumulate, int32_t* __restrict__ nf_flag,
-                                                                LossFinish lf) {
-    if (blockIdx.x < nb_a) dw_reduce_body(slabs_a, n_a, nW_a, gw_a, accumulate, blockIdx.x, nf_flag);
-    else if (blockIdx.x < nb_a + nb_b) dw_reduce_body(slabs_b, n_b, nW_b, gw_b, accumulate, blockIdx.x - nb_a, nf_flag);
-    else {
-        static_assert(64 * DWR_GROUPS == 1024, "the loss sum is written for 16 waves, like k_loss_finish");
-        __shared__ float part[16];
-        float acc = 0.0f;
-        for (uint32_t i = threadIdx.x; i < lf.n_part; i += 1024) acc += lf.partials[i];
-        {
-            auto dpp = [](float v, auto ctrl, auto mask) {
-                return __builtin_bit_cast(float, __builtin_amdgcn_update_dpp(0, __builtin_bit_cast(int, v), decltype(ctrl)::value, decltype(mask)::value, 0xf, false));
-            };
-            using std::integral_constant;
-            acc += dpp(acc, integral_constant<int, 0x111>{}, integral_constant<int, 0xf>{});
-            acc += dpp(acc, integral_constant<int, 0x112>{}, integral_constant<int, 0xf>{});
-            acc += dpp(acc, integral_constant<int, 0x114>{}, integral_constant<int, 0xf>{});
-            acc += dpp(acc, integral_constant<int, 0x118>{}, integral_constant<int, 0xf>{});
-            acc += dpp(acc, integral_constant<int, 0x142>{}, integral_constant<int, 0xa>{});
-            acc += dpp(acc, integral_constant<int, 0x143>{}, integral_constant<int, 0xc>{});
-            acc = __builtin_bit_cast(float, __builtin_amdgcn_readlane(__builtin_bit_cast(int, acc), 63));
-        }
-        if ((threadIdx.x & 63) == 0) part[threadIdx.x >> 6] = acc;
-        __syncthreads();
-        if (threadIdx.x == 0) {
-            float t = 0.0f;
-#pragma unroll
-            for (int w = 0; w < 16; w++) t += part[w];
-            const float loss = t / (float)lf.n_elem;
-            lf.out[0] = loss * (lf.scale ? lf.scale[0] : 1.0f);
-            lf.out[1] = loss;
-        }
-    }
+    __shared__ float part[lae_dw::DWR_LDS_FLOATS];
+    lae_dw::dw_reduce_body(slabs, n_slices, nW, gw, accumulate, blockIdx.x, nf_flag, part);
+}
+__global__ __launch_bounds__(64 * DWR_GROUPS) void k_dw_reduce2(lae_dw::DwTailJob job) {
+    __shared__ float part[lae_dw::DWR_LDS_FLOATS];
+    lae_dw::dw_tail_task(job, blockIdx.x, part);
 }
 
 #include "sh_table.inc"
@@ -1778,6 +1718,20 @@
                            void* grad_color_weights, int accumulate_weight_grads, int enc_level_major, int32_t* nonfinite_flag,
                            const float* loss_partials, uint32_t loss_n_part, uint32_t loss_n_elem, const float* loss_scale,
                            float* loss_out, void* stream) {
+    return lae::nerf_head_backward(grad_sigmas, grad_rgbs, enc, dirs, h, rgbs, sigma_weights, color_weights, M, density_scale, grad_h,
+                                   grad_enc, grad_sigma_weights, grad_color_weights, accumulate_weight_grads, enc_level_major,
+                                   nonfinite_flag, loss_partials, loss_n_part, loss_n_elem, loss_scale, loss_out, stream, nullptr);
+}
+
+}
+
+int lae::nerf_head_backward(const float* grad_sigmas, const float* grad_rgbs, const void* enc, const float* dirs, const void* h,
+                            const float* rgbs, const void* sigma_weights, const void* color_weights, uint32_t M,
+                            float density_scale, void* grad_h, void* grad_enc, void* grad_sigma_weights,
+                            void* grad_color_weights, int accumulate_weight_grads, int enc_level_major, int32_t* nonfinite_flag,
+                            const float* loss_partials, uint32_t loss_n_part, uint32_t loss_n_elem, const float* loss_scale,
+                            float* loss_out, void* stream, lae_dw::DwTailJob* tail) {
+    if (tail) tail->n_tasks = 0;
     if (!grad_sigma_weights || !grad_color_weights) return LAE_ENULL;
     if (loss_out && (!loss_partials || loss_n_elem == 0)) return LAE_EINVAL;
     hipStream_t s = reinterpret_cast<hipStream_t>(stream);
@@ -1810,11 +1764,14 @@
     if (rc != LAE_OK) return rc;
     const uint32_t nb_c = lae::cdiv(nW_c, 64u), nb_s = lae::cdiv(nW_s, 64u);
     const LossFinish lf{loss_partials, loss_n_part, loss_n_elem, loss_scale, loss_out};
-    k_dw_reduce2<<<nb_c + nb_s + (loss_out ? 1u : 0u), 64 * DWR_GROUPS, 0, s>>>(ws, n_c, nW_c, (half_t*)grad_color_weights, ws_s, n_s, nW_s,
-                                                                               (half_t*)grad_sigma_weights, nb_c, nb_s,
-                                                                               accumulate_weight_grads, nonfinite_flag, lf);
+    const lae_dw::DwTailJob job{ws, n_c, nW_c, (half_t*)grad_color_weights, ws_s, n_s, nW_s, (half_t*)grad_sigma_weights, nb_c, nb_s,
+                                accumulate_weight_grads, nonfinite_flag, lf, nb_c + nb_s + (loss_out ? 1u : 0u)};
+    if (tail) *tail = job;
+    else k_dw_reduce2<<<job.n_tasks, 64 * DWR_GROUPS, 0, s>>>(job);
     return lae::check_launch("nerf_head_backward");
 }
+
+extern "C" {
 
 int lae_ffmlp_set_mode(int mode) {
     if (mode != 0 && mode != 1 && mode != 3) return LAE_EINVAL;
diff --git a/laenerf_amd/csrc/gridencoder.hip b/laenerf_amd/csrc/gridencoder.hip
--- a/laenerf_amd/csrc/gridencoder.hip
+++ b/laenerf_amd/csrc/gridencoder.hip
@@ -4,6 +4,7 @@
 #include <algorithm>
 #include <type_traits>
 #include "lae_common.h"
+#include "dw_reduce.h"
 #include <vector>
 #include <mutex>
 #include <utility>
@@ -329,7 +330,9 @@
 __global__ __launch_bounds__(GRID_BLOCK) void k_grid_bwd(
     const T* __restrict__ grad, const float* __restrict__ inputs, const int32_t* __restrict__ offsets,
     T* __restrict__ grad_grid, uint32_t B, uint32_t L, LevelScales sc, uint32_t gridtype, bool align_corners,
-    uint32_t interp, uint32_t nb, bool xcd_mode, uint64_t gs_b, uint64_t gs_l, bool only_unbinned) {
+    uint32_t interp, uint32_t nb, bool xcd_mode, uint64_t gs_b, uint64_t gs_l, bool only_unbinned,
+    uint32_t* __restrict__ grad_dirty = nullptr) {
+    if (grad_dirty && blockIdx.x == 0 && threadIdx.x == 0) *grad_dirty = 1u;
     uint32_t level, chunk;
     block_to_level_chunk(nb, xcd_mode, level, chunk);
     if (level >= L) return;
@@ -410,6 +413,14 @@
     uint32_t* tickets;
 };
 
+__host__ __device__ __forceinline__ lae_dw::DwTailJob* plan_tail_job(const BwdPlan& plan) {
+    static_assert((TICKET_WORDS * 4) % alignof(lae_dw::DwTailJob) == 0, "the tail job sits right behind the tickets");
+    return reinterpret_cast<lae_dw::DwTailJob*>(plan.tickets + TICKET_WORDS);
+}
+__host__ __device__ __forceinline__ uint32_t* plan_dirty_snapshot(const BwdPlan& plan) {
+    return plan.tickets + TICKET_WORDS + sizeof(lae_dw::DwTailJob) / 4;
+}
+
 __device__ __forceinline__ uint32_t pack_half2(float a, float b) {
     const half2_t h = {(half_t)a, (half_t)b};
     return __builtin_bit_cast(uint32_t, h);
@@ -420,14 +431,21 @@
     const T* __restrict__ gradT, const float* __restrict__ inputs, const int32_t* __restrict__ offsets, uint32_t B,
     uint32_t L, LevelScales sc, uint32_t gridtype_, bool align_corners_, uint32_t interp_, uint32_t U, BwdPlan plan,
     typename BVal<T>::type* __restrict__ qvals, uint16_t* __restrict__ qkeys, uint32_t* __restrict__ touched_,
-    uint32_t* __restrict__ level_full) {
+    uint32_t* __restrict__ level_full, uint32_t* __restrict__ grad_dirty = nullptr, lae_dw::DwTailJob tail = lae_dw::DwTailJob{}) {
     const uint32_t gridtype = PLAIN ? 0u : gridtype_, interp = PLAIN ? 0u : interp_;
     const bool align_corners = PLAIN ? false : align_corners_;
     using V = typename BVal<T>::type;
     if constexpr (FILL) GRID_STAMP(blockIdx.x, 0);
     const uint32_t NBLK = U / SEGS;
     const uint32_t level = blockIdx.x / NBLK, chunk = blockIdx.x % NBLK;
-    if (FILL && blockIdx.x == 0) for (uint32_t k = threadIdx.x; k < TICKET_WORDS; k += FILL_THREADS) plan.tickets[k] = 0;
+    if (FILL && blockIdx.x == 0) {
+        for (uint32_t k = threadIdx.x; k < TICKET_WORDS; k += FILL_THREADS) plan.tickets[k] = 0;
+        if (threadIdx.x == 0) {
+            *plan_dirty_snapshot(plan) = grad_dirty ? *grad_dirty : 1u;
+            if (grad_dirty) *grad_dirty = 1u;
+            *plan_tail_job(plan) = tail;
+        }
+    }
     const LevelInfo<3> li = level_info<3>(sc, offsets, level, gridtype, align_corners);
     const uint32_t P = (li.hashmap_size + PART - 1) >> PART_SHIFT;
     if (P > BK_MAX) return;
@@ -867,6 +885,7 @@
     };
 
     bool first_task = true;
+    uint32_t tail_task;
     [[maybe_unused]] uint32_t stamp_task = 0;
     GRID_STAMP(4096 + blockIdx.x, 0);
     for (;;) {
@@ -875,7 +894,7 @@
         __syncthreads();
         const uint32_t t = __builtin_amdgcn_readfirstlane(s_ticket);
         GRID_STAMP(4096 + blockIdx.x, 1 + stamp_task * 6);
-        if (t >= total_buckets) break;
+        if (t >= total_buckets) { tail_task = t - total_buckets; break; }
         GRID_NOTE(4096 + blockIdx.x, 2 + stamp_task * 6, t);
         const uint32_t item = t;
         uint32_t level = 0;
@@ -884,16 +903,19 @@
         const uint32_t bk = item - __builtin_amdgcn_readfirstlane(s_first[level]);
         const uint32_t SUB = __builtin_amdgcn_readfirstlane(s_sub[level]), p = bk / SUB, sub = bk % SUB;
         const uint32_t table_off = (uint32_t)offsets[level], hashmap_size = (uint32_t)offsets[level + 1] - table_off;
-        const uint32_t n = __builtin_amdgcn_readfirstlane(plan.totals[level * BK_MAX + p]), q0 = __builtin_amdgcn_readfirstlane(plan.offs[level * BK_MAX + p]);
+        const uint32_t n_raw = plan.totals[level * BK_MAX + p], q0_raw = plan.offs[level * BK_MAX + p], dirty_raw = *plan_dirty_snapshot(plan);
+        const uint32_t n = __builtin_amdgcn_readfirstlane(n_raw), q0 = __builtin_amdgcn_readfirstlane(q0_raw);
+        const bool grad_dirty = __builtin_amdgcn_readfirstlane(dirty_raw) != 0u;
         const uint32_t lo = (uint32_t)(((uint64_t)n * sub) / SUB), hi = (uint32_t)(((uint64_t)n * (sub + 1)) / SUB);
         if (n == 0) { __syncthreads(); continue; }
         const uint32_t part_lo = p << PART_SHIFT;
         const uint32_t n_ent = min(PART, hashmap_size - part_lo);
         T* __restrict__ dst = grad_grid + ((size_t)table_off + part_lo) * 2;
         uint32_t oldv[HALF ? PART / ACC_THREADS : 1];
+        const uint32_t n_old = grad_dirty ? n_ent : 0u;
         if constexpr (HALF) {
 #pragma unroll
-            for (int it = 0; it < (int)(PART / ACC_THREADS); it++) { const uint32_t e = tid + it * ACC_THREADS; oldv[it] = e < n_ent ? reinterpret_cast<const uint32_t*>(dst)[e] : 0u; }
+            for (int it = 0; it < (int)(PART / ACC_THREADS); it++) { const uint32_t e = tid + it * ACC_THREADS; oldv[it] = e < n_old ? reinterpret_cast<const uint32_t*>(dst)[e] : 0u; }
         }
         for (uint32_t i = tid; i < ACCW; i += ACC_THREADS) acc64[i] = 0ull;
         if (tid < PART / 32) poison[tid] = 0u;
@@ -1014,7 +1036,7 @@
                 const uint32_t e = tid + it * ACC_THREADS;
                 if (e >= n_ent) break;
                 const long long i0 = (long long)acc64[e], i1 = (long long)acc64[PART + e];
-                const bool bad = (poison[e >> 5] >> (e & 31)) & 1u;
+                const bool bad = (poison[(tid >> 5) + it * (ACC_THREADS / 32)] >> (tid & 31)) & 1u;
                 if (i0 == 0 && i1 == 0 && !bad) continue;
                 const uint32_t o = oldv[it];
                 uint32_t r0, r1;
@@ -1040,6 +1062,15 @@
         GRID_STAMP(4096 + blockIdx.x, 6 + stamp_task * 6);
         stamp_task++;
         __syncthreads();
+    }
+    static_assert(sizeof(acc64) >= lae_dw::DWR_LDS_FLOATS * sizeof(float) && ACC_THREADS == (int)lae_dw::DWR_THREADS, "tail tasks run in this workgroup");
+    const lae_dw::DwTailJob& tail = *plan_tail_job(plan);
+    const uint32_t n_tail = __builtin_amdgcn_readfirstlane(tail.n_tasks);
+    while (tail_task < n_tail) {
+        lae_dw::dw_tail_task(tail, tail_task, reinterpret_cast<float*>(acc64));
+        if (tid == 0) s_ticket = atomicAdd(&plan.tickets[0], 1u) + gridDim.x;
+        __syncthreads();
+        tail_task = __builtin_amdgcn_readfirstlane(s_ticket) - total_buckets;
     }
 }
 
@@ -1315,6 +1346,8 @@
     int32_t* nf_flag = nullptr;
     uint32_t* touched = nullptr;
     uint32_t* touched_full = nullptr;
+    uint32_t* dirty = nullptr;
+    const lae_dw::DwTailJob* tail = nullptr;
 };
 template <typename T, int D, int C>
 static void launch_bwd(const BwdArgs& a) {
@@ -1322,7 +1355,7 @@
     const bool xcd = (a.L % 8) == 0;
     k_grid_bwd<T, D, C><<<nb * a.L, GRID_BLOCK, 0, a.stream>>>(a.grad ? (const T*)a.grad : nullptr, a.inputs, a.offsets,
                                                                 (T*)a.gemb, a.B, a.L, a.sc, a.gridtype, a.align,
-                                                                a.interp, nb, xcd, a.gs_b, a.gs_l, false);
+                                                                a.interp, nb, xcd, a.gs_b, a.gs_l, false, a.dirty);
 }
 template <typename T, int D>
 static int dispatch_bwd_c(const BwdArgs& a, uint32_t C) {
@@ -1396,7 +1429,7 @@
     const size_t U = bwd_units(B);
     auto up = [](size_t v) { return (v + 255) / 256 * 256; };
     PlanLayout w;
-    w.totals_off = up((size_t)TICKET_WORDS * 4);
+    w.totals_off = up((size_t)TICKET_WORDS * 4 + sizeof(lae_dw::DwTailJob) + 4);
     w.offs_off = w.totals_off + up((size_t)L * BK_MAX * 4);
     w.cnt_off = w.offs_off + up((size_t)L * BK_MAX * 4);
     w.part_off = w.cnt_off + up((size_t)L * U * BK_MAX * 2);
@@ -1479,15 +1512,16 @@
     const T* g = (const T*)gT;
     T* ge = (T*)gemb;
     if (!caller_plan) bwd_plan<T>(inputs, offsets, B, L, a, plan);
+    const lae_dw::DwTailJob tail_job = a.tail ? *a.tail : lae_dw::DwTailJob{};
 #ifdef LAE_GRID_BWD_PHASE_PROBE
     const char* phase_env = getenv("LAE_GRID_BWD_PHASE");
     const int phase_probe = phase_env ? atoi(phase_env) : 0;
     if (phase_probe != 2)
 #endif
     if (a.gridtype == 0 && !a.align && a.interp == 0)
-        k_bwd_walk<T, true, true><<<U / SEGS * L, FILL_THREADS, 0, a.stream>>>(g, inputs, offsets, B, L, a.sc, a.gridtype, a.align, a.interp, U, plan, qvals, qkeys, nullptr, nullptr);
+        k_bwd_walk<T, true, true><<<U / SEGS * L, FILL_THREADS, 0, a.stream>>>(g, inputs, offsets, B, L, a.sc, a.gridtype, a.align, a.interp, U, plan, qvals, qkeys, nullptr, nullptr, a.dirty, tail_job);
     else
-        k_bwd_walk<T, true, false><<<U / SEGS * L, FILL_THREADS, 0, a.stream>>>(g, inputs, offsets, B, L, a.sc, a.gridtype, a.align, a.interp, U, plan, qvals, qkeys, nullptr, nullptr);
+        k_bwd_walk<T, true, false><<<U / SEGS * L, FILL_THREADS, 0, a.stream>>>(g, inputs, offsets, B, L, a.sc, a.gridtype, a.align, a.interp, U, plan, qvals, qkeys, nullptr, nullptr, a.dirty, tail_job);
 #ifdef LAE_GRID_BWD_PHASE_PROBE
     if (phase_probe == 1) return lae::check_launch("grid backward (fill-only probe)");
 #endif
@@ -1518,10 +1552,11 @@
                          const void* dy_dx, void* grad_inputs, uint32_t gridtype, int align_corners, uint32_t interp,
                          int dtype, bool blc, void* stream, float in_shift = 0.0f, float in_scale = 1.0f,
                          const int32_t* offsets_host = nullptr, const void* plan = nullptr, int32_t* nf_flag = nullptr,
-                         uint32_t* touched = nullptr) {
+                         uint32_t* touched = nullptr, uint32_t* dirty = nullptr, const lae_dw::DwTailJob* tail = nullptr) {
     (void)embeddings;
     if (B == 0) return LAE_OK;
     if (!grad || !inputs || !offsets || !grad_embeddings) return LAE_ENULL;
+    if (tail && !(D == 3 && C == 2 && L <= 32 && B <= BWD_MAX_SAMPLES && !g_force_atomic_bwd && dtype == LAE_F16)) return LAE_EINVAL;
     if (plan && !(D == 3 && C == 2 && L <= 32 && B <= BWD_MAX_SAMPLES && !blc && !g_force_atomic_bwd)) return LAE_EINVAL;
     if (gridtype > 1 || interp > 1) return LAE_EINVAL;
     if (touched && dtype != LAE_F16) return LAE_EINVAL;
@@ -1535,6 +1570,8 @@
     a.nf_flag = nf_flag;
     a.touched = touched;
     if (touched) a.touched_full = touched + touched_words(offsets_host, L);
+    a.dirty = dirty;
+    a.tail = tail;
     a.grad = grad; a.inputs = inputs; a.offsets = offsets; a.gemb = grad_embeddings; a.B = B; a.L = L;
     int rc = fill_scales(a.sc, L, S, H);
     if (rc) return rc;
@@ -1634,10 +1671,11 @@
                                 void* grad_embeddings, uint32_t B, uint32_t D, uint32_t C, uint32_t L, float S,
                                 uint32_t H, const void* dy_dx, void* grad_inputs, uint32_t gridtype,
                                 int align_corners, uint32_t interp, int dtype, int blc, float in_shift, float in_scale,
-                                const int32_t* offsets_host, int32_t* nonfinite_flag, uint32_t* touched_lines, void* stream) {
+                                const int32_t* offsets_host, int32_t* nonfinite_flag, uint32_t* touched_lines, uint32_t* grad_dirty,
+                                void* stream) {
     return grid_backward(grad, inputs, embeddings, offsets, grad_embeddings, B, D, C, L, S, H, dy_dx, grad_inputs,
                          gridtype, align_corners, interp, dtype, blc != 0, stream, in_shift, in_scale, offsets_host, nullptr,
-                         nonfinite_flag, touched_lines);
+                         nonfinite_flag, touched_lines, grad_dirty);
 }
 
 uint64_t lae_grid_backward_workspace_bytes(uint32_t B, uint32_t L, int dtype) {
@@ -1678,10 +1716,47 @@
 int lae_grid_encode_backward_planned(const void* grad, const float* inputs, const int32_t* offsets, void* grad_embeddings, uint32_t B,
                                      uint32_t D, uint32_t C, uint32_t L, float S, uint32_t H, uint32_t gridtype, int align_corners,
                                      uint32_t interp, int dtype, float in_shift, float in_scale, const int32_t* offsets_host,
-                                     const void* plan, int32_t* nonfinite_flag, void* stream) {
+                                     const void* plan, int32_t* nonfinite_flag, uint32_t* grad_dirty, void* stream) {
     if (!plan) return LAE_ENULL;
     return grid_backward(grad, inputs, nullptr, offsets, grad_embeddings, B, D, C, L, S, H, nullptr, nullptr, gridtype, align_corners,
-                         interp, dtype, false, stream, in_shift, in_scale, offsets_host, plan, nonfinite_flag, nullptr);
+                         interp, dtype, false, stream, in_shift, in_scale, offsets_host, plan, nonfinite_flag, nullptr, grad_dirty);
+}
+
+int lae_nerf_field_backward(const float* grad_sigmas, const float* grad_rgbs, const void* enc, const float* dirs, const void* h,
+                            const float* rgbs, const void* sigma_weights, const void* color_weights, uint32_t M, float density_scale,
+                            void* grad_h, void* grad_enc, void* grad_sigma_weights, void* grad_color_weights,
+                            int accumulate_weight_grads, int32_t* weights_nonfinite_flag, const float* loss_partials,
+                            uint32_t loss_n_part, uint32_t loss_n_elem, const float* loss_scale, float* loss_out,
+                            const float* inputs, const int32_t* offsets, void* grad_embeddings, uint32_t L, float S, uint32_t H,
+                            uint32_t gridtype, int align_corners, uint32_t interp, float in_shift, float in_scale,
+                            const int32_t* offsets_host, const void* plan, int32_t* table_nonfinite_flag, uint32_t* touched_lines,
+                            uint32_t* grad_dirty, void* stream) {
+    if (!grad_sigma_weights || !grad_color_weights) return LAE_ENULL;
+    if (loss_out && (!loss_partials || loss_n_elem == 0)) return LAE_EINVAL;
+    if (M > 0) {
+        if (!grad_sigmas || !grad_rgbs || !enc || !dirs || !h || !rgbs || !sigma_weights || !color_weights || !grad_h || !grad_enc ||
+            !inputs || !offsets || !grad_embeddings) return LAE_ENULL;
+        if (M % 16 != 0 || gridtype > 1 || interp > 1) return LAE_EINVAL;
+        LevelScales sc;
+        if (const int rc = fill_scales(sc, L, S, H)) return rc;
+        const bool binned = L <= 32 && M <= BWD_MAX_SAMPLES && !g_force_atomic_bwd;
+        if (plan && !binned) return LAE_EINVAL;
+        if (table_nonfinite_flag || touched_lines) {
+            if (!binned || !offsets_host) return LAE_EINVAL;
+            for (uint32_t l = 0; l < L; l++)
+                if (!level_is_binned((uint32_t)(offsets_host[l + 1] - offsets_host[l]))) return LAE_EINVAL;
+        }
+    }
+    const char* off = getenv("LAE_FIELD_NO_RIDE_ALONG");
+    const bool ride = M > 0 && L <= 32 && M <= BWD_MAX_SAMPLES && !g_force_atomic_bwd && !(off && off[0] == '1');
+    lae_dw::DwTailJob tail{};
+    int rc = lae::nerf_head_backward(grad_sigmas, grad_rgbs, enc, dirs, h, rgbs, sigma_weights, color_weights, M, density_scale, grad_h,
+                                     grad_enc, grad_sigma_weights, grad_color_weights, accumulate_weight_grads, 1, weights_nonfinite_flag,
+                                     loss_partials, loss_n_part, loss_n_elem, loss_scale, loss_out, stream, ride ? &tail : nullptr);
+    if (rc != LAE_OK) return rc;
+    return grid_backward(grad_enc, inputs, nullptr, offsets, grad_embeddings, M, 3, 2, L, S, H, nullptr, nullptr, gridtype, align_corners,
+                         interp, LAE_F16, false, stream, in_shift, in_scale, offsets_host, plan, table_nonfinite_flag,
+                         plan ? nullptr : touched_lines, grad_dirty, ride ? &tail : nullptr);
 }
 
 int lae_grid_forward_schedule(const int32_t* offsets_host, uint32_t L, float S, uint32_t H, uint32_t n_chunks, uint32_t* nseg_out,
diff --git a/laenerf_amd/csrc/lae_common.h b/laenerf_amd/csrc/lae_common.h
--- a/laenerf_amd/csrc/lae_common.h
+++ b/laenerf_amd/csrc/lae_common.h
@@ -44,6 +44,16 @@
                               hipStream_t stream);
 uint32_t frame_head_max_blocks();
 
+}
+namespace lae_dw { struct DwTailJob; }
+namespace lae {
+int nerf_head_backward(const float* grad_sigmas, const float* grad_rgbs, const void* enc, const float* dirs, const void* h,
+                       const float* rgbs, const void* sigma_weights, const void* color_weights, uint32_t M, float density_scale,
+                       void* grad_h, void* grad_enc, void* grad_sigma_weights, void* grad_color_weights,
+                       int accumulate_weight_grads, int enc_level_major, int32_t* nonfinite_flag, const float* loss_partials,
+                       uint32_t loss_n_part, uint32_t loss_n_elem, const float* loss_scale, float* loss_out, void* stream,
+                       lae_dw::DwTailJob* tail);
+
 static inline int check_launch(const char* what) {
     hipError_t e = hipGetLastError();
     if (e != hipSuccess) { set_last_error(what, e); return LAE_ELAUNCH; }
diff --git a/laenerf_amd/csrc/optimizer.hip b/laenerf_amd/csrc/optimizer.hip
--- a/laenerf_amd/csrc/optimizer.hip
+++ b/laenerf_amd/csrc/optimizer.hip
@@ -156,6 +156,7 @@
     float* p[MAX_SEGS]; float* m[MAX_SEGS]; float* v[MAX_SEGS]; void* grad[MAX_SEGS]; half_t* shadow[MAX_SEGS];
     const float* lr[MAX_SEGS]; size_t n[MAX_SEGS]; int is_half[MAX_SEGS]; int count;
     const uint32_t* touched[MAX_SEGS];
+    uint32_t* dirty[MAX_SEGS];
 };
 
 template <typename G>
@@ -243,6 +244,10 @@
     const bool skip = st->skip != 0;
     const float inv_scale = st->inv_scale, bc2_sqrt = st->bc2_sqrt;
     if (blockIdx.x == gridDim.x - 1 && threadIdx.x == 0) prepare_next_step(st, h.beta1, h.beta2);
+    if (blockIdx.x == gridDim.x / 2 && threadIdx.x == 0) {
+#pragma unroll
+        for (int s = 0; s < MAX_SEGS; s++) if (s < sg.count && sg.dirty[s]) *sg.dirty[s] = 0u;
+    }
     for (int s = 0; s < sg.count; s++) {
         const float lr_over_bc1 = (float)((double)sg.lr[s][0] * (double)st->inv_bc1);
         if (sg.is_half[s]) seg_apply(sg.p[s], sg.m[s], sg.v[s], (half_t*)sg.grad[s], sg.shadow[s], sg.n[s], skip, inv_scale, bc2_sqrt, lr_over_bc1, h, sg.touched[s]);
@@ -371,7 +376,7 @@
 
 int lae_adam_apply_multi(uint32_t n_tensors, float* const* params, float* const* exp_avgs, float* const* exp_avg_sqs, void* const* grads,
                          const int* grad_is_half, void* const* shadows_half, const uint64_t* sizes, const float* const* lrs,
-                         const void* const* touched_lines, const void* state, float beta1, float beta2, float eps, float weight_decay,
+                         const void* const* touched_lines, void* const* grad_dirty, const void* state, float beta1, float beta2, float eps, float weight_decay,
                          void* stream) {
     if (n_tensors == 0) return LAE_OK;
     if (!params || !exp_avgs || !exp_avg_sqs || !grads || !grad_is_half || !shadows_half || !sizes || !lrs || !state) return LAE_ENULL;
@@ -387,6 +392,7 @@
         sg.p[i] = params[i]; sg.m[i] = exp_avgs[i]; sg.v[i] = exp_avg_sqs[i]; sg.grad[i] = grads[i];
         sg.shadow[i] = (half_t*)shadows_half[i]; sg.lr[i] = lrs[i]; sg.n[i] = sizes[i]; sg.is_half[i] = grad_is_half[i];
         sg.touched[i] = (touched_lines && weight_decay == 0.0f) ? (const uint32_t*)touched_lines[i] : nullptr;
+        sg.dirty[i] = grad_dirty ? (uint32_t*)grad_dirty[i] : nullptr;
         biggest = std::max(biggest, (size_t)sizes[i]);
     }
     sg.count = (int)n_tensors;
diff --git a/laenerf_amd/editing/style_encoder.py b/laenerf_amd/editing/style_encoder.py
--- a/laenerf_amd/editing/style_encoder.py
+++ b/laenerf_amd/editing/style_encoder.py
@@ -151,7 +151,8 @@
             enc.shadow.mark_all_touched()
         _grid.grid_encode_backward(grad_feats, x, table, enc.offsets, grad_table, M, 3, 2, L, S, H, None, None, enc.gridtype_id,
                                    enc.align_corners, enc.interp_id, blc=False, in_map=ctx.in_map, offsets_host=enc.offsets_host,
-                                   plan=ctx.plan, nonfinite_flag=flag, touched_lines=touched)
+                                   plan=ctx.plan, nonfinite_flag=flag, touched_lines=touched,
+                                   grad_dirty=enc.shadow.dirty_for_backward() if enc.shadow is not None else None)
         return None, None, (None if enc.shadow is not None else grad_table), None, None, None, None, None
 
 
diff --git a/laenerf_amd/field.py b/laenerf_amd/field.py
--- a/laenerf_amd/field.py
+++ b/laenerf_amd/field.py
@@ -57,8 +57,6 @@
             wflag = _weights_flag(ctx.shadows)
         else:
             gws, gwc = torch.empty_like(ws), torch.empty_like(wc)
-        _mlp.nerf_head_backward(grad_sigmas, grad_rgbs, feats, dirs, h, rgbs, ws, wc, M, ctx.density_scale, grad_h, grad_feats,
-                                gws, gwc, accumulate=ctx.shadows is not None, level_major=True, nonfinite_flag=wflag)
         grad_table = enc.shadow.grad_half if enc.shadow is not None else torch.zeros_like(table)
         flag = enc.shadow.flag_for_backward(M) if enc.shadow is not None else None
         touched = enc.shadow.touched_for_backward(M) if flag is not None else None
@@ -66,9 +64,12 @@
             touched = None
         if enc.shadow is not None and touched is None:
             enc.shadow.mark_all_touched()
-        _grid.grid_encode_backward(grad_feats, x, table, enc.offsets, grad_table, M, 3, 2, L, S, H, None, None, enc.gridtype_id,
-                                   enc.align_corners, enc.interp_id, blc=False, in_map=ctx.in_map, offsets_host=enc.offsets_host, plan=ctx.plan,
-                                   nonfinite_flag=flag, touched_lines=touched)
+        dirty = enc.shadow.dirty_for_backward() if enc.shadow is not None else None
+        _mlp.nerf_field_backward(grad_sigmas, grad_rgbs, feats, dirs, h, rgbs, ws, wc, M, ctx.density_scale, grad_h, grad_feats, gws, gwc,
+                                 x, enc.offsets, grad_table, L, S, H, enc.gridtype_id, enc.align_corners, enc.interp_id,
+                                 accumulate=ctx.shadows is not None, weights_nonfinite_flag=wflag, in_map=ctx.in_map,
+                                 offsets_host=enc.offsets_host, plan=ctx.plan, table_nonfinite_flag=flag, touched_lines=touched,
+                                 grad_dirty=dirty)
         return (None, None, None if enc.shadow is not None else grad_table,
                 None if ctx.shadows is not None else gws.to(ctx.wdtypes[0]),
                 None if ctx.shadows is not None else gwc.to(ctx.wdtypes[1]), None, None, None, None, None, None)
diff --git a/laenerf_amd/gridencoder/grid.py b/laenerf_amd/gridencoder/grid.py
--- a/laenerf_amd/gridencoder/grid.py
+++ b/laenerf_amd/gridencoder/grid.py
@@ -57,7 +57,8 @@
             ctx.shadow.mark_all_touched()
         _backend.grid_encode_backward(grad, inputs, embeddings, offsets, grad_embeddings, B, D, C, L, S, H, dy_dx,
                                       grad_inputs, gridtype, ctx.align_corners, interpolation, blc=True, in_map=ctx.in_map,
-                                      offsets_host=ctx.offsets_host, nonfinite_flag=flag, touched_lines=touched)
+                                      offsets_host=ctx.offsets_host, nonfinite_flag=flag, touched_lines=touched,
+                                      grad_dirty=ctx.shadow.dirty_for_backward() if ctx.shadow is not None else None)
         if dy_dx is not None:
             grad_inputs = grad_inputs.to(inputs.dtype)
             if ctx.in_map[1] != 1.0:
@@ -75,8 +76,22 @@
         self.grad_half = self.grad_store[:n].view_as(self.half)
         self.version = embeddings._version
         self.nonfinite_flag = None
-        self.unreported = False
+        self.grad_dirty = None
+        self._unreported = False
         self.touched_lines = None
+
+    @property
+    def unreported(self):
+        return self._unreported
+
+    @unreported.setter
+    def unreported(self, value):
+        self._unreported = bool(value)
+        if value and self.grad_dirty is not None:
+            self.grad_dirty.fill_(1)
+
+    def dirty_for_backward(self):
+        return None if self.grad_dirty is None else self.grad_dirty.data_ptr()
 
     def mark_all_touched(self):
         if self.touched_lines is not None:
diff --git a/laenerf_amd/optim.py b/laenerf_amd/optim.py
--- a/laenerf_amd/optim.py
+++ b/laenerf_amd/optim.py
@@ -54,6 +54,10 @@
                         shadow.touched_lines = torch.zeros(n_words, dtype=torch.int32, device=p.device)
                 elif shadow is not None and isinstance(owner, FFMLP):
                     shadow.nonfinite_flag = self.dev_state.data_ptr() + 8
+        if not os.environ.get("LAE_GRID_NO_DIRTY_WORD"):
+            for p, _, _, shadow, _ in self.items:
+                if shadow is not None and isinstance(tables.get(id(p)), GridEncoder) and shadow.grad_dirty is None:
+                    shadow.grad_dirty = torch.ones(1, dtype=torch.int32, device=p.device)
         self._scale_view = self.dev_state.view(torch.float32)
         self._scale_view[0] = init_scale if self.use_scaler else 1.0
         self.device_lr = bool(device_lr)
@@ -134,6 +138,8 @@
         for p, _, _, shadow, _ in self.items:
             if shadow is not None:
                 shadow.grad_half.zero_()
+                if getattr(shadow, "grad_dirty", None) is not None:
+                    shadow.grad_dirty.zero_()
                 p.grad = None
             elif p.grad is not None:
                 p.grad.zero_()
@@ -155,13 +161,14 @@
 
     def _tables(self):
         grads = [self._grad(p, sh) for p, _, _, sh, _ in self.items]
-        key = tuple(g.data_ptr() for g, _ in grads)
+        dirty = [None if sh is None or getattr(sh, "grad_dirty", None) is None else sh.grad_dirty.data_ptr() for _, _, _, sh, _ in self.items]
+        key = tuple(g.data_ptr() for g, _ in grads) + tuple(dirty)
         if self._args is None or self._args["key"] != key:
             n = len(self.items)
             arr = lambda vals: (ctypes.c_void_p * n)(*vals)
             self._args = {
                 "key": key, "n": n,
-                "grads": arr(key), "is_half": (ctypes.c_int * n)(*[h for _, h in grads]),
+                "grads": arr(key[:n]), "dirty": arr(dirty), "is_half": (ctypes.c_int * n)(*[h for _, h in grads]),
                 "sizes": (ctypes.c_uint64 * n)(*[p.numel() for p, *_ in self.items]),
                 "params": arr([p.data_ptr() for p, *_ in self.items]),
                 "m": arr([m.data_ptr() for _, m, *_ in self.items]), "v": arr([v.data_ptr() for _, _, v, *_ in self.items]),
@@ -190,7 +197,7 @@
         _lib.check(lib.lae_adam_begin(st, self.betas[0], self.betas[1], self.growth_interval, self.growth_factor,
                                       self.backoff_factor, int(self.use_scaler), s), "adam_begin")
         _lib.check(lib.lae_adam_apply_multi(a["n"], a["params"], a["m"], a["v"], a["grads"], a["is_half"], a["shadows"],
-                                            a["sizes"], a["lrs"], a["touched"], st, self.betas[0], self.betas[1], self.eps,
+                                            a["sizes"], a["lrs"], a["touched"], a["dirty"], st, self.betas[0], self.betas[1], self.eps,
                                             self.weight_decay, s), "adam_apply")
         for *_, shadow, _ in self.items:
             if shadow is not None and hasattr(shadow, "unreported"):
```

New measurement: 11.44 Mrays/s (median of 6 runs). 2.3% higher.
